# CEED/Laghos

Hardware: AMD Instinct MI355X
Metric: Mdofs×steps/s on 3D Sedov -pa (Q3/Q2) (higher is better)
Workload: dtype f64; 1 GPU; 3D Sedov -p 1 -m cube01_hex -rs 4 -ok 3 -ot 2 -pa (32^3 elements, E0/2^dim = 0.125); transport=none (one rank), elements=32768, h1_dofs=2738019, l2_dofs=884736, quad_points_per_element=216, rk_stages_executed=1300, ode=RK4, parallelism=elements1x1x1, zones_per_gpu=32x32x32

## Files before the change

### include/laghos_hip.h

```cpp
#ifndef LAGHOS_HIP_H
#define LAGHOS_HIP_H

#ifdef __cplusplus
extern "C" {
#endif

#define LGH_OK 0
#define LGH_ERR_ARG 1
#define LGH_ERR_UNSUPPORTED 2
#define LGH_ERR_HIP 3
#define LGH_ERR_COMM 4

#define LGH_SPACE_H1 0
#define LGH_SPACE_L2 1

typedef struct lgh_ctx lgh_ctx;

typedef struct lgh_config
{
   int dim, NE;
   int D1D, Q1D, L1D;
   int N;
   const int *h1_map;
   const double *B_h1;
// ... 42 lines not shown
int lgh_mass_eliminate_rhs(lgh_ctx *ctx, double *b);
int lgh_mass_mult(lgh_ctx *ctx, int space, const double *x, double *y);
int lgh_mass_mult_full(lgh_ctx *ctx, int space, const double *x, double *y);

int lgh_cg_solve(lgh_ctx *ctx, int space, const double *b, double *x, double rel_tol,
                 int max_iter, int *iters);
int lgh_l2_mass_solve_local(lgh_ctx *ctx, const double *b, double *x);

int lgh_qupdate(lgh_ctx *ctx, const double *S);
int lgh_qupdate_set_tiny_grad(lgh_ctx *ctx, double tiny_grad);
int lgh_set_fused_forces(lgh_ctx *ctx, int on);
int lgh_qupdate_store_stress(lgh_ctx *ctx, int on);
int lgh_qupdate_stores_stress(lgh_ctx *ctx, int *on);
int lgh_qupdate_form(lgh_ctx *ctx, int *form);
int lgh_reset_quadrature_data(lgh_ctx *ctx);
int lgh_fused_force_mult(lgh_ctx *ctx, double *y_h1);
int lgh_fused_force_mult_transpose(lgh_ctx *ctx, double *y_l2);
int lgh_quadrature_generation(lgh_ctx *ctx, unsigned long *gen, int *f1_valid, int *ftv_valid);
int lgh_get_fused_forces(lgh_ctx *ctx, int *f1, int *ftv);

int lgh_solve_velocity(lgh_ctx *ctx, const double *S, double *dS_dt, const double *one_l2,
                       double *rhs_h1, double *work_B, double rel_tol, int max_iter,
                       int *h1_iters);
int lgh_solve_energy(lgh_ctx *ctx, const double *S, const double *v_h1, double *dS_dt,
                     double *e_rhs, const double *e_source, double rel_tol, int max_iter,
                     int *l2_iters);
int lgh_solve_energy_begin(lgh_ctx *ctx, const double *S, const double *v_h1, double *dS_dt,
                           double *e_rhs, const double *e_source, double rel_tol, int max_iter);
int lgh_solve_energy_end(lgh_ctx *ctx, int *l2_iters);
int lgh_energy_lockstep_stats(lgh_ctx *ctx, long out[4]);

int lgh_vec_set(lgh_ctx *ctx, double *y, double a, long n);
int lgh_vec_copy(lgh_ctx *ctx, double *y, const double *x, long n);
int lgh_vec_axpby_pair(lgh_ctx *ctx, double *z1, double a1, const double *x1, double b1, double *z2, double a2, const double *x2, double b2,
                       const double *y, long n);
int lgh_vec_axpby(lgh_ctx *ctx, double *z, double a, const double *x, double b,
                  const double *y, long n);
int lgh_vec_dot(lgh_ctx *ctx, const double *x, const double *y, long n, double *result);
int lgh_vec_fingerprint(lgh_ctx *ctx, const double *x, long n, unsigned long long offset, unsigned long long out[2]);
int lgh_vec_fingerprint_shape(lgh_ctx *ctx, const double *x, long n, long out[4]);
int lgh_fingerprint_host(const void *words, long n, unsigned long long offset, unsigned long long out[2]);

int lgh_set_velocity_source(lgh_ctx *ctx, const double *accel_h1);

int lgh_tg_source_2d(lgh_ctx *ctx, const double *S, double *e_source);

int lgh_internal_energy(lgh_ctx *ctx, const double *e_l2, double *result);
int lgh_kinetic_energy(lgh_ctx *ctx, const double *v_h1, double *result);

int lgh_sedov_setup(int dim, double gamma, double rho0, double blast_energy, double omega, double par[21]);
int lgh_sedov_shock(const double par[21], double t, double shock[6]);
int lgh_sedov_eval_point(const double par[21], double t, double r, double *rho, double *v, double *P);
int lgh_sedov_eval(lgh_ctx *ctx, const double par[21], double t, long n, const double *r, double *rho, double *v,
                   double *P);
int lgh_compute_density(lgh_ctx *ctx, const double *x_h1, double *rho_l2);
int lgh_sedov_density_error(lgh_ctx *ctx, const double *x_h1, const double *rho_l2, const double par[21], double t,
                            const double origin[3], int n1d, const double *weights, const double *B_h1,
                            const double *G_h1, const double *B_l2, double *err2);

int lgh_sample_fields(lgh_ctx *ctx, const double *S, const double *rho_l2 ,
                      int R1, const double *B_h1_lat ,
                      const double *B_l2_lat ,
                      double *x_out, double *v_out, double *e_out, double *rho_out, double *p_out);

int lgh_sample_derived(lgh_ctx *ctx, const double *S, int R1, const double *B_h1_lat ,
                       const double *G_h1_lat , const double *B_l2_lat ,
// ... 82 lines not shown
```

### laghos_amd/_lib.py

```python
import ctypes
import os

_HERE = os.path.dirname(os.path.abspath(__file__))
LIB_PATH = os.path.join(_HERE, "liblaghos_hip.so")

c_dp = ctypes.c_void_p
c_int_p = ctypes.POINTER(ctypes.c_int)
c_dbl_p = ctypes.POINTER(ctypes.c_double)


class LghConfig(ctypes.Structure):
    _fields_ = [
        ("dim", ctypes.c_int), ("NE", ctypes.c_int),
        ("D1D", ctypes.c_int), ("Q1D", ctypes.c_int), ("L1D", ctypes.c_int),
        ("N", ctypes.c_int),
        ("h1_map", c_int_p),
        ("B_h1", c_dbl_p), ("G_h1", c_dbl_p), ("B_l2", c_dbl_p),
        ("weights", c_dbl_p), ("gamma", c_dbl_p),
        ("ess_count", ctypes.c_int * 3),
        ("ess", c_int_p * 3),
        ("owner", c_dbl_p),
        ("use_viscosity", ctypes.c_int), ("use_vorticity", ctypes.c_int),
        ("cfl", ctypes.c_double),
        ("order_v", ctypes.c_int),
# ... 12 lines not shown
    "lgh_last_error": (ctypes.c_char_p, []),
    "lgh_version": (ctypes.c_char_p, []),
    "lgh_create": (_I, [ctypes.POINTER(LghConfig), ctypes.POINTER(_P)]),
    "lgh_destroy": (_I, [_P]),
    "lgh_sync": (_I, [_P]),
    "lgh_stream": (_P, [_P]),
    "lgh_qdata_stressJinvT": (_P, [_P]),
    "lgh_qdata_Jac0inv": (_P, [_P]),
    "lgh_qdata_rho0DetJ0w": (_P, [_P]),
    "lgh_mass_D": (_P, [_P]),
    "lgh_mass_diag": (_P, [_P]),
    "lgh_set_h0": (_I, [_P, _D]),
    "lgh_get_h0": (_I, [_P, c_dbl_p]),
    "lgh_set_dt_est": (_I, [_P, _D]),
    "lgh_get_dt_est": (_I, [_P, c_dbl_p]),
    "lgh_setup_rho0detj0": (_I, [_P, _P, _P, _P, c_dbl_p]),
    "lgh_force_mult": (_I, [_P, _P, _P]),
    "lgh_force_mult_transpose": (_I, [_P, _P, _P]),
    "lgh_mass_set_essential_tdofs": (_I, [_P, _I]),
    "lgh_mass_eliminate_rhs": (_I, [_P, _P]),
    "lgh_mass_mult": (_I, [_P, _I, _P, _P]),
    "lgh_mass_mult_full": (_I, [_P, _I, _P, _P]),
    "lgh_cg_solve": (_I, [_P, _I, _P, _P, _D, _I, c_int_p]),
    "lgh_l2_mass_solve_local": (_I, [_P, _P, _P]),
    "lgh_qupdate": (_I, [_P, _P]),
    "lgh_solve_velocity": (_I, [_P, _P, _P, _P, _P, _P, _D, _I, c_int_p]),
    "lgh_solve_energy": (_I, [_P, _P, _P, _P, _P, _P, _D, _I, c_int_p]),
    "lgh_solve_energy_begin": (_I, [_P, _P, _P, _P, _P, _P, _D, _I]),
    "lgh_tg_source_2d": (_I, [_P, _P, _P]),
    "lgh_set_velocity_source": (_I, [_P, _P]),
    "lgh_solve_energy_end": (_I, [_P, c_int_p]),
    "lgh_vec_set": (_I, [_P, _P, _D, _L]),
    "lgh_vec_copy": (_I, [_P, _P, _P, _L]),
    "lgh_vec_axpby": (_I, [_P, _P, _D, _P, _D, _P, _L]),
    "lgh_vec_axpby_pair": (_I, [_P, _P, _D, _P, _D, _P, _D, _P, _D, _P, _L]),
    "lgh_vec_dot": (_I, [_P, _P, _P, _L, c_dbl_p]),
    "lgh_vec_fingerprint": (_I, [_P, _P, _L, ctypes.c_ulonglong, ctypes.POINTER(ctypes.c_ulonglong)]),
    "lgh_vec_fingerprint_shape": (_I, [_P, _P, _L, ctypes.POINTER(ctypes.c_long)]),
    "lgh_fingerprint_host": (_I, [_P, _L, ctypes.c_ulonglong, ctypes.POINTER(ctypes.c_ulonglong)]),
    "lgh_internal_energy": (_I, [_P, _P, c_dbl_p]),
    "lgh_kinetic_energy": (_I, [_P, _P, c_dbl_p]),
    "lgh_sedov_setup": (_I, [_I, _D, _D, _D, _D, c_dbl_p]),
    "lgh_sedov_shock": (_I, [c_dbl_p, _D, c_dbl_p]),
    "lgh_sedov_eval_point": (_I, [c_dbl_p, _D, _D, c_dbl_p, c_dbl_p, c_dbl_p]),
    "lgh_sedov_eval": (_I, [_P, c_dbl_p, _D, _L, _P, _P, _P, _P]),
    "lgh_compute_density": (_I, [_P, _P, _P]),
    "lgh_sedov_density_error": (_I, [_P, _P, _P, c_dbl_p, _D, c_dbl_p, _I, c_dbl_p, c_dbl_p, c_dbl_p, c_dbl_p, c_dbl_p]),
    "lgh_sample_fields": (_I, [_P, _P, _P, _I, c_dbl_p, c_dbl_p, _P, _P, _P, _P, _P]),
    "lgh_sample_derived": (_I, [_P, _P, _I, c_dbl_p, c_dbl_p, c_dbl_p, _P, _P, _P, _P, _P]),
    "lgh_diagnostics_zones": (_I, [_P, _P, _P]),
    "lgh_diagnostics": (_I, [_P, _P, c_dbl_p]),
    "lgh_profile": (_I, [_P, _P, ctypes.POINTER(LghProfileSpec), c_dbl_p, ctypes.POINTER(ctypes.c_long)]),
    "lgh_get_timers": (_I, [_P, c_dbl_p, ctypes.POINTER(ctypes.c_long)]),
    "lgh_reset_timers": (_I, [_P]),
    "lgh_enable_timers": (_I, [_P, _I]),
    "lgh_ktime_begin": (_I, [_P, _I, _I]),
    "lgh_ktime_end": (_I, [_P, c_int_p, c_dbl_p]),
    "lgh_table_symmetry": (_I, [_P, c_int_p, c_int_p]),
    "lgh_k1_form": (_I, [_P, c_int_p]),
    "lgh_l2_mass_form": (_I, [_P, c_int_p, c_int_p]),
    "lgh_vcg_layout_stats": (_I, [_P, ctypes.POINTER(ctypes.c_long)]),
    "lgh_energy_lockstep_stats": (_I, [_P, ctypes.POINTER(ctypes.c_long)]),
    "lgh_mesh_order": (_I, [_P, ctypes.POINTER(ctypes.c_long)]),
    "lgh_mesh_order_host": (_I, [_I, _I, _I, _I, c_int_p, c_int_p, c_int_p, ctypes.POINTER(ctypes.c_long)]),
    "lgh_mass_data_form": (_I, [_P, c_int_p]),
    "lgh_jac0inv_form": (_I, [_P, c_int_p]),
# ... 73 lines not shown
```

### laghos_amd/csrc/lgh_1d.hip

```cpp
#include <algorithm>
#include <cmath>
#include <limits>
#include <type_traits>

#include "lgh_common.hpp"

namespace lgh
{

bool kernel_id_supported_1d(int kid)
{
   switch (kid)
   {
      case 0x122: case 0x134: case 0x146: case 0x158: case 0x16A: return true;
   }
   return false;
}

template <int V> using IC = std::integral_constant<int, V>;

template <class F> static int dispatch_1d(const lgh_ctx *c, F &&f)
{
   switch (c->kid)
   {
// ... 689 lines not shown
   LGH_TRY(alloc_copy(&c->B, cfg->B_h1, (size_t)Q * D));
   LGH_TRY(alloc_copy(&c->G, cfg->G_h1, (size_t)Q * D));
   LGH_TRY(alloc_copy(&c->Bl, cfg->B_l2, (size_t)Q * L));
   LGH_TRY(alloc_copy(&c->W, cfg->weights, (size_t)Q));
   LGH_TRY(alloc_copy(&c->gamma, cfg->gamma, (size_t)NE));
   const size_t nmap = (size_t)NE * D;
   LGH_TRY(alloc_copy(&c->h1map, cfg->h1_map, nmap));
   LGH_TRY(mesh_order_build(c, cfg->h1_map));
   {
      std::vector<int> off((size_t)N + 1, 0), idx(nmap);
      for (size_t i = 0; i < nmap; i++) { off[(size_t)cfg->h1_map[i] + 1]++; }
      for (int n = 0; n < N; n++) { off[(size_t)n + 1] += off[n]; }
      std::vector<int> pos(off.begin(), off.end() - 1);
      for (size_t i = 0; i < nmap; i++) { idx[pos[cfg->h1_map[i]]++] = (int)i; }
      LGH_TRY(alloc_copy(&c->t_off, off.data(), off.size()));
      LGH_TRY(alloc_copy(&c->t_idx, idx.data(), idx.size()));
   }
   {
      c->ess_count[0] = cfg->ess_count[0];
      std::vector<uint8_t> mask((size_t)N, 0);
      for (int i = 0; i < c->ess_count[0]; i++) { mask[cfg->ess[0][i]] = 1; }
      LGH_TRY(alloc_copy(&c->essmask[0], mask.data(), mask.size()));
      LGH_TRY(alloc_copy(&c->ess[0], c->ess_count[0] ? cfg->ess[0] : nullptr, (size_t)c->ess_count[0]));
   }
   const size_t nq = (size_t)NE * Q;
   LGH_TRY(alloc_zero(&c->stressJinvT, nq));
   LGH_TRY(alloc_zero(&c->Jac0inv, nq));
   LGH_TRY(alloc_zero(&c->rho0DetJ0w, nq));
   LGH_TRY(alloc_zero(&c->massD, nq));
   LGH_TRY(alloc_zero(&c->me_fac, (size_t)NE * L * L));
   LGH_TRY(alloc_zero(&c->diagV, (size_t)N));
   LGH_TRY(alloc_zero(&c->dinvV, (size_t)N));
   LGH_TRY(alloc_zero(&c->dt_est_dev, (size_t)kDtSlotStride * (1 + kDtSlots)));
   LGH_TRY(alloc_zero(&c->dev_flags, (size_t)8));
   LGH_TRY(alloc_zero(&c->YE, std::max(nmap, (size_t)c->L2V)));
   const size_t nv = std::max<size_t>((size_t)N, (size_t)c->L2V);
   LGH_TRY(alloc_zero(&c->cg_r, nv));
   LGH_TRY(alloc_zero(&c->cg_z, nv));
   LGH_TRY(alloc_zero(&c->cg_d0, nv));
   LGH_TRY(alloc_zero(&c->cg_y, nv));
   c->part_stride = (int)std::max<size_t>(std::max<size_t>((size_t)NE, (nv + 255) / 256), 2048) + (int)kShards;
   LGH_TRY(alloc_zero(&c->partials, 4 * (size_t)c->part_stride));
   LGH_TRY(alloc_zero(&c->tickets, 4 * (size_t)kTicketSlot));
   LGH_TRY(alloc_zero(&c->cgs, 1));
   LGH_TRY(alloc_zero(&c->scal, 16));
   LGH_HIP_CHECK(hipHostMalloc((void **)&c->host_pinned, 96 * sizeof(double), hipHostMallocMapped | hipHostMallocCoherent));
   memset(c->host_pinned, 0, 96 * sizeof(double));
   LGH_HIP_CHECK(hipHostGetDevicePointer((void **)&c->host_pinned_dev, c->host_pinned, 0));
   LGH_HIP_CHECK(hipEventCreate(&c->timers.ev[0]));
   LGH_HIP_CHECK(hipEventCreate(&c->timers.ev[1]));
   {
      const std::vector<double> infs((size_t)kDtSlotStride * (1 + kDtSlots), std::numeric_limits<double>::infinity());
      LGH_HIP_CHECK(hipMemcpy(c->dt_est_dev, infs.data(), infs.size() * sizeof(double), hipMemcpyHostToDevice));
   }
#undef LGH_TRY
   return LGH_OK;
}

int mass_changed_1d(lgh_ctx *c)
{
   return dispatch_1d(c, [&](auto Dc, auto Qc) {
      constexpr int D = decltype(Dc)::value, Q = decltype(Qc)::value;
      hipLaunchKernelGGL((h1_diag_e_1d_k<D, Q>), dim3(zone_grid(c)), dim3(256), 0, c->stream, c->NE, c->B, c->massD, c->YE);
      hipLaunchKernelGGL(gather_1d_k, dim3(ceil_div(c->N, 256)), dim3(256), 0, c->stream, c->N, c->t_off, c->t_idx, c->YE,
                         (const uint8_t *)nullptr, c->diagV);
      hipLaunchKernelGGL(reciprocal_1d_k, dim3(ceil_div(c->N, 256)), dim3(256), 0, c->stream, c->N, c->diagV, c->dinvV);
      hipLaunchKernelGGL((l2_factor_1d_k<D - 1, Q>), dim3(zone_grid(c)), dim3(256), 0, c->stream, c->NE, c->Bl, c->massD,
// ... 258 lines not shown
```

### laghos_amd/csrc/lgh_api.hip

```cpp
#include <cstdarg>
#include <cstdlib>
#include <cmath>
#include <algorithm>
#include <limits>

#include "lgh_common.hpp"

#include <chrono>
#include <dlfcn.h>

namespace lgh
{

static thread_local char g_err[512] = "";
void set_error(const char *fmt, ...)
{
   va_list ap;
   va_start(ap, fmt);
   vsnprintf(g_err, sizeof(g_err), fmt, ap);
   va_end(ap);
}

__global__ void __launch_bounds__(256) vec_set_k(double *y, double a, long n)
{
// ... 5 lines not shown
   for (long i = blockIdx.x * (long)blockDim.x + threadIdx.x; i < n; i += (long)gridDim.x * blockDim.x)
   {
      z[i] = fma(a, x[i], __dmul_rn(b, y[i]));
   }
}
__global__ void __launch_bounds__(256)
vec_axpby2_k(double2 *z, double a, const double2 *x, double b, const double2 *y, long n2)
{
   const long stride = (long)gridDim.x * blockDim.x;
   long i = blockIdx.x * (long)blockDim.x + threadIdx.x;
   for (; i + stride < n2; i += 2 * stride)
   {
      const double2 x0 = x[i], y0 = y[i], x1 = x[i + stride], y1 = y[i + stride];
      z[i] = make_double2(fma(a, x0.x, __dmul_rn(b, y0.x)), fma(a, x0.y, __dmul_rn(b, y0.y)));
      z[i + stride] = make_double2(fma(a, x1.x, __dmul_rn(b, y1.x)), fma(a, x1.y, __dmul_rn(b, y1.y)));
   }
   if (i < n2)
   {
      const double2 x0 = x[i], y0 = y[i];
      z[i] = make_double2(fma(a, x0.x, __dmul_rn(b, y0.x)), fma(a, x0.y, __dmul_rn(b, y0.y)));
   }
}
__global__ void __launch_bounds__(256)
vec_axpby_pair_k(double2 *z1, double a1, const double2 *x1, double b1, double2 *z2, double a2, const double2 *x2, double b2, const double2 *y, long n2)
{
   const long stride = (long)gridDim.x * blockDim.x;
   for (long i = blockIdx.x * (long)blockDim.x + threadIdx.x; i < n2; i += stride)
   {
      const double2 y0 = y[i], p = x1[i], q = x2[i];
      z1[i] = make_double2(fma(a1, p.x, __dmul_rn(b1, y0.x)), fma(a1, p.y, __dmul_rn(b1, y0.y)));
      z2[i] = make_double2(fma(a2, q.x, __dmul_rn(b2, y0.x)), fma(a2, q.y, __dmul_rn(b2, y0.y)));
   }
}
__global__ void __launch_bounds__(256) vec_neg_k(double *y, long n)
{
   for (long i = blockIdx.x * (long)blockDim.x + threadIdx.x; i < n; i += (long)gridDim.x * blockDim.x) { y[i] = -y[i]; }
}
__global__ void __launch_bounds__(256) vec_zero_list_k(double *y, const int *list, int n)
{
   const int i = blockIdx.x * blockDim.x + threadIdx.x;
   if (i < n) { y[list[i]] = 0.0; }
}
__global__ void __launch_bounds__(256)
vec_dot_k(const double *x, const double *y, const double *w, long n, double *partials,
          unsigned int *ticket, double *out)
{
   __shared__ double red[16];
   double s = 0.0;
   for (long i = blockIdx.x * (long)blockDim.x + threadIdx.x; i < n; i += (long)gridDim.x * blockDim.x)
   {
      s += (w ? w[i] : 1.0) * x[i] * y[i];
   }
   const double bsum = block_sum(s, red);
   double total;
   if (grid_sum_last_block(bsum, partials, ticket, red, total))
   {
      if (threadIdx.x == 0) { *out = total; }
   }
}
__global__ void set_double_k(double *p, double v) { *p = v; }
__global__ void __launch_bounds__(256) dt_est_set_k(double *p, double v)
{
   if (threadIdx.x == 0) { p[0] = v; }
   for (int s = threadIdx.x; s < kDtSlots; s += blockDim.x) { p[kDtSlotStride * (1 + s)] = __builtin_inf(); }
}
__global__ void __launch_bounds__(256) dt_est_fold_k(double *p, const int *err, double *host_out, const unsigned long long token)
// ... 32 lines not shown
   if (n >= 4096 && (((uintptr_t)z | (uintptr_t)x | (uintptr_t)y) & 15u) == 0)
   {
      const long n2 = n / 2;
      hipLaunchKernelGGL(vec_axpby2_k, dim3(grid_for(n2)), dim3(256), 0, c->stream, (double2 *)z, a, (const double2 *)x, b,
                         (const double2 *)y, n2);
      if (n & 1) { hipLaunchKernelGGL(vec_axpby_k, dim3(1), dim3(64), 0, c->stream, z + 2 * n2, a, x + 2 * n2, b, y + 2 * n2, 1L); }
   }
   else { hipLaunchKernelGGL(vec_axpby_k, dim3(grid_for(n)), dim3(256), 0, c->stream, z, a, x, b, y, n); }
   LGH_HIP_CHECK(hipGetLastError());
   return LGH_OK;
}
int vec_axpby_pair(lgh_ctx *c, double *z1, double a1, const double *x1, double b1, double *z2, double a2, const double *x2, double b2,
                   const double *y, long n)
{
   if (n <= 0) { return LGH_OK; }
   if (n >= 4096 && (((uintptr_t)z1 | (uintptr_t)x1 | (uintptr_t)z2 | (uintptr_t)x2 | (uintptr_t)y) & 15u) == 0)
   {
      const long n2 = n / 2;
      hipLaunchKernelGGL(vec_axpby_pair_k, dim3(grid_for(n2)), dim3(256), 0, c->stream, (double2 *)z1, a1, (const double2 *)x1, b1, (double2 *)z2, a2,
                         (const double2 *)x2, b2, (const double2 *)y, n2);
      LGH_HIP_CHECK(hipGetLastError());
      if (n & 1)
      {
         hipLaunchKernelGGL(vec_axpby_k, dim3(1), dim3(64), 0, c->stream, z1 + 2 * n2, a1, x1 + 2 * n2, b1, y + 2 * n2, 1L);
         hipLaunchKernelGGL(vec_axpby_k, dim3(1), dim3(64), 0, c->stream, z2 + 2 * n2, a2, x2 + 2 * n2, b2, y + 2 * n2, 1L);
      }
      LGH_HIP_CHECK(hipGetLastError());
      return LGH_OK;
   }
   int rc = vec_axpby(c, z1, a1, x1, b1, y, n);
   if (rc) { return rc; }
   return vec_axpby(c, z2, a2, x2, b2, y, n);
}
int vec_neg_inplace(lgh_ctx *c, double *y, long n)
{
   if (n <= 0) { return LGH_OK; }
   hipLaunchKernelGGL(vec_neg_k, dim3(grid_for(n)), dim3(256), 0, c->stream, y, n);
   LGH_HIP_CHECK(hipGetLastError());
   return LGH_OK;
}
int vec_zero_list(lgh_ctx *c, double *y, const int *list, int n)
{
   if (n <= 0) { return LGH_OK; }
   hipLaunchKernelGGL(vec_zero_list_k, dim3(ceil_div(n, 256)), dim3(256), 0, c->stream, y, list, n);
   LGH_HIP_CHECK(hipGetLastError());
   return LGH_OK;
}
int vec_dot(lgh_ctx *c, const double *x, const double *y, const double *w, long n, double *dev_out)
{
   hipLaunchKernelGGL(vec_dot_k, dim3(grid_for(n)), dim3(256), 0, c->stream, x, y, w, n,
                      c->partials + 3 * (size_t)c->part_stride, c->tickets + 3 * kTicketSlot, dev_out);
   LGH_HIP_CHECK(hipGetLastError());
   return LGH_OK;
}

void timer_start(lgh_ctx *c)
{
   if (!c->timers.enabled) { return; }
   (void)hipEventRecord(c->timers.ev[0], c->stream);
}
void timer_stop(lgh_ctx *c, int which)
{
   if (!c->timers.enabled) { return; }
   (void)hipEventRecord(c->timers.ev[1], c->stream);
   (void)hipEventSynchronize(c->timers.ev[1]);
   float ms = 0.f;
// ... 55 lines not shown
static bool kernel_id_supported(int id)
{
   switch (id)
   {
      case 0x222: case 0x234: case 0x246: case 0x258: case 0x26A:
      case 0x322: case 0x334: case 0x346: case 0x358: case 0x36A:
         return true;
   }
   return false;
}

}

namespace lgh
{
int host_wait_token(lgh_ctx *c, volatile unsigned long long *word, const unsigned long long token)
{
   const bool spin = !(getenv("LGH_SPIN") && getenv("LGH_SPIN")[0] == '0');
   if (spin)
   {
      const auto t0 = std::chrono::steady_clock::now();
      for (long i = 0;; i++)
      {
         if (__atomic_load_n((const unsigned long long *)word, __ATOMIC_ACQUIRE) == token) { return LGH_OK; }
         __builtin_ia32_pause();
         if ((i & 1023) == 1023 && std::chrono::steady_clock::now() - t0 > std::chrono::milliseconds(50)) { break; }
      }
   }
   LGH_HIP_CHECK(hipStreamSynchronize(c->stream));
   if (__atomic_load_n((const unsigned long long *)word, __ATOMIC_ACQUIRE) != token) { set_error("host look: the finishing kernel did not report"); return LGH_ERR_HIP; }
   return LGH_OK;
}

int energy_overlap_poll(lgh_ctx *c)
{
   if (c->e_async != 1 || c->e_polled) { return LGH_OK; }
   int it = 0;
   std::swap(c->stream, c->stream2);
   c->on_stream2 = 1;
   int rc = cg_l2_end(c, &it);
   if (rc == LGH_OK) { rc = (hipEventRecord(c->ev_join, c->stream) == hipSuccess) ? LGH_OK : LGH_ERR_HIP; }
   std::swap(c->stream, c->stream2);
   c->on_stream2 = 0;
   if (rc) { return rc; }
   c->e_polled = 1;
   c->e_iters = it;
   return LGH_OK;
}

}

using namespace lgh;

extern "C"
{

const char *lgh_last_error(void) { return g_err; }
const char *lgh_version(void) { return "laghos_hip 0.1 (gfx950)"; }

static int create_impl(const lgh_config *cfg, lgh_ctx *c, const int kid);

int lgh_create(const lgh_config *cfg, lgh_ctx **out)
{
   LGH_CHECK_ARG(cfg && out);
   LGH_CHECK_ARG(cfg->dim == 1 || cfg->dim == 2 || cfg->dim == 3);
   LGH_CHECK_ARG(cfg->NE > 0 && cfg->N > 0);
   LGH_CHECK_ARG(cfg->h1_map && cfg->B_h1 && cfg->G_h1 && cfg->B_l2 && cfg->weights && cfg->gamma);
   if (cfg->L1D != cfg->D1D - 1)
   {
      set_error("L1D!=D1D-1");
      return LGH_ERR_UNSUPPORTED;
   }
   const int kid = (cfg->dim << 8) | (cfg->D1D << 4) | cfg->Q1D;
   if (!(cfg->dim == 1 ? kernel_id_supported_1d(kid) : kernel_id_supported(kid)))
// ... 32 lines not shown
   memset((void *)c, 0, sizeof(lgh_ctx));
   new (&c->timers) Timers();
   c->device = cfg->device;
   const int rc_create = (cfg->dim == 1) ? create_1d(cfg, c) : create_impl(cfg, c, kid);
   if (rc_create != LGH_OK)
   {
      lgh_destroy(c);
      return rc_create;
   }
   *out = c;
   return LGH_OK;
}

static int create_impl(const lgh_config *cfg, lgh_ctx *c, const int kid)
{
   c->dim = cfg->dim; c->NE = cfg->NE; c->D1D = cfg->D1D; c->Q1D = cfg->Q1D; c->L1D = cfg->L1D;
   const int dim = c->dim;
   c->ND = dim == 2 ? c->D1D * c->D1D : c->D1D * c->D1D * c->D1D;
   c->NQ = dim == 2 ? c->Q1D * c->Q1D : c->Q1D * c->Q1D * c->Q1D;
   c->NL = dim == 2 ? c->L1D * c->L1D : c->L1D * c->L1D * c->L1D;
   c->N = cfg->N;
   c->H1V = dim * c->N;
   c->L2V = c->NE * c->NL;
   c->kid = kid;
   c->visc = cfg->use_viscosity != 0;
   c->vort = cfg->use_vorticity != 0;
   c->cfl = cfg->cfl;
   c->h1order = (double)cfg->order_v;
   {
      const char *env = getenv("LGH_Q_TINY_GRAD");
      c->q_tiny_grad = env ? atof(env) : 1e-30;
      c->stress_store = 1;
      c->stress_current = 0;
   }
   c->h0 = 0.0;
   c->device = cfg->device;
   c->cur_ess = -1;
   c->nranks = 1;
   c->rank = 0;
   if (cfg->stream) { c->stream = (hipStream_t)cfg->stream; c->own_stream = false; }
   else { LGH_HIP_CHECK(hipStreamCreateWithFlags(&c->stream, hipStreamNonBlocking)); c->own_stream = true; }

   int rc;
#define LGH_TRY(x) do { rc = (x); if (rc) { return rc; } } while (0)
   LGH_TRY(dev_alloc_copy(&c->B, cfg->B_h1, (size_t)c->Q1D * c->D1D));
   {
      const char *env = getenv("LGH_B_SYM");
      auto mirror = [&](const double *B, const int n) {
         if (env && env[0] == '0') { return 0; }
         for (int i = 0; i < n; i++)
         {
            const double u = B[i], v = B[n - 1 - i];
            if (std::fabs(u - v) > 1e-14 * std::max(1.0, std::max(std::fabs(u), std::fabs(v)))) { return 0; }
         }
         return 1;
      };
      c->b_h1_sym = mirror(cfg->B_h1, c->Q1D * c->D1D);
      c->b_l2_sym = mirror(cfg->B_l2, c->Q1D * c->L1D);
   }
   LGH_TRY(dev_alloc_copy(&c->G, cfg->G_h1, (size_t)c->Q1D * c->D1D));
   LGH_TRY(dev_alloc_copy(&c->Bl, cfg->B_l2, (size_t)c->Q1D * c->L1D));
   LGH_TRY(dev_alloc_copy(&c->W, cfg->weights, (size_t)c->NQ));
   {
      const int Q = c->Q1D, dim = c->dim;
      std::vector<double> w1((size_t)Q);
      const double w0 = (dim == 3) ? cbrt(cfg->weights[0]) : sqrt(cfg->weights[0]);
// ... 73 lines not shown
   }
   for (int k = 0; k < 3; k++)
   {
      c->ess_count[k] = (k < dim) ? cfg->ess_count[k] : 0;
      std::vector<uint8_t> mask((size_t)c->N, 0);
      for (int i = 0; i < c->ess_count[k]; i++)
      {
         const int n = cfg->ess[k][i];
         if (n < 0 || n >= c->N) { set_error("essential dof out of range"); return LGH_ERR_ARG; }
         mask[n] = 1;
      }
      LGH_TRY(dev_alloc_copy(&c->essmask[k], mask.data(), mask.size()));
      LGH_TRY(dev_alloc_copy(&c->ess[k], c->ess_count[k] ? cfg->ess[k] : nullptr, (size_t)c->ess_count[k]));
   }
   if (cfg->owner) { LGH_TRY(dev_alloc_copy(&c->owner, cfg->owner, (size_t)c->N)); }

   const size_t nq = (size_t)c->NE * c->NQ;
   LGH_TRY(dev_alloc_zero(&c->stressJinvT, nq * dim * dim));
   LGH_TRY(dev_alloc_zero(&c->Jac0inv, nq * dim * dim));
   LGH_TRY(dev_alloc_zero(&c->Jac0inv_soa, nq * dim * dim));
   LGH_TRY(dev_alloc_zero(&c->Jac0inv_e, (size_t)cfg->NE * dim * dim));
   LGH_TRY(dev_alloc_zero(&c->rho0DetJ0w, nq));
   LGH_TRY(dev_alloc_zero(&c->massD, nq + 2048));
   LGH_TRY(dev_alloc_zero(&c->diagV, (size_t)c->N));
   LGH_TRY(dev_alloc_zero(&c->dinvV, (size_t)c->N));
   LGH_TRY(dev_alloc_zero(&c->dt_est_dev, (size_t)kDtSlotStride * (1 + kDtSlots)));
   {
      const char *env = getenv("LGH_FUSED_FTV");
      if (!(env && env[0] == '0'))
      {
         LGH_TRY(dev_alloc_zero(&c->erhs_q, (size_t)c->L2V));
         LGH_TRY(dev_alloc_zero(&c->v_snap, (size_t)c->H1V));
      }
      LGH_TRY(dev_alloc_zero(&c->dev_flags, (size_t)8));
      c->mass_rank1 = -1;
      env = getenv("LGH_FUSED_F1");
      if (c->dim == 3 && !(env && env[0] == '0')) { LGH_TRY(dev_alloc_zero(&c->force_e_q, nmap * dim + (size_t)dim * c->ND)); }
   }
   const size_t ne_nd = nmap * dim;
   LGH_TRY(dev_alloc_zero(&c->XE, std::max<size_t>(ne_nd, (size_t)c->L2V)));
   LGH_TRY(dev_alloc_zero(&c->YE, ne_nd + (size_t)dim * c->ND));
   const size_t nv = std::max<size_t>((size_t)c->N, (size_t)c->L2V);
   LGH_TRY(dev_alloc_zero(&c->cg_r, nv));
   LGH_TRY(dev_alloc_zero(&c->cg_z, nv));
   LGH_TRY(dev_alloc_zero(&c->cg_d0, nv));
   LGH_TRY(dev_alloc_zero(&c->cg_d1, nv));
   LGH_TRY(dev_alloc_zero(&c->cg_y, nv));
   c->part_stride = (int)std::max<size_t>(std::max<size_t>((size_t)c->NE, (nv + 255) / 256), 2048) + (int)kShards;
   LGH_TRY(dev_alloc_zero(&c->partials, 4 * (size_t)c->part_stride));
   LGH_TRY(dev_alloc_zero(&c->tickets, 4 * (size_t)kTicketSlot));
   LGH_TRY(dev_alloc_zero(&c->cgs, 1));
   LGH_TRY(dev_alloc_zero(&c->scal, 16));
   LGH_HIP_CHECK(hipHostMalloc((void **)&c->host_pinned, 96 * sizeof(double), hipHostMallocMapped | hipHostMallocCoherent));
   memset(c->host_pinned, 0, 96 * sizeof(double));
   LGH_HIP_CHECK(hipHostGetDevicePointer((void **)&c->host_pinned_dev, c->host_pinned, 0));
   LGH_HIP_CHECK(hipEventCreate(&c->timers.ev[0]));
   LGH_HIP_CHECK(hipEventCreate(&c->timers.ev[1]));
   {
      const std::vector<double> infs((size_t)kDtSlotStride * (1 + kDtSlots), std::numeric_limits<double>::infinity());
      LGH_HIP_CHECK(hipMemcpy(c->dt_est_dev, infs.data(), infs.size() * sizeof(double), hipMemcpyHostToDevice));
   }
#undef LGH_TRY
   return LGH_OK;
}

int lgh_destroy(lgh_ctx *c)
{
   if (!c) { return LGH_OK; }
   (void)hipSetDevice(c->device);
   (void)hipStreamSynchronize(c->stream);
   void *ptrs[] = {c->B, c->G, c->Bl, c->W, c->w1d, c->M1h, c->M1l, c->gamma, c->h1map, c->t_off, c->t_idx, c->t_ell, c->essmask[0],
                   c->essmask[1], c->essmask[2], c->ess[0], c->ess[1], c->ess[2], c->owner,
                   c->stressJinvT, c->Jac0inv, c->Jac0inv_soa, c->Jac0inv_e, c->rho0DetJ0w, c->massD, c->diagV, c->dinvV,
                   c->dt_est_dev, c->erhs_q, c->v_snap, c->dev_flags, c->ones_l2, c->massS, c->ones_ne, c->force_e_q, c->XE, c->YE, c->cg_r, c->cg_z, c->cg_d0, c->cg_d1, c->cg_y,
                   c->partials, c->tickets, c->cgs, c->scal, c->vcg_s, c->vcg_vec, c->vcg_partials,
                   c->vcg_tickets, c->me_fac, c->fp_dev, c->diag_dev, c->prof_dev};
   for (void *p : ptrs) { if (p) { (void)hipFree(p); } }
   if (c->host_pinned) { (void)hipHostFree(c->host_pinned); }
   if (c->timers.ev[0]) { (void)hipEventDestroy(c->timers.ev[0]); }
   if (c->timers.ev[1]) { (void)hipEventDestroy(c->timers.ev[1]); }
   if (c->ktime)
   {
      for (hipEvent_t e : c->ktime->ev) { (void)hipEventDestroy(e); }
      delete c->ktime;
   }
   cg_l2_free(c);
   vcg_free(c);
   mesh_order_free(c);
   if (c->q_trace_dev) { (void)hipFree(c->q_trace_dev); }
   if (c->stream2)
   {
      (void)hipStreamSynchronize(c->stream2);
      (void)hipStreamDestroy(c->stream2);
      (void)hipEventDestroy(c->ev_fork);
      (void)hipEventDestroy(c->ev_join);
   }
   for (auto &ring : c->ls_ev) { for (hipEvent_t e : ring) { if (e) { (void)hipEventDestroy(e); } } }
   extern void lgh_comm_free(lgh_ctx *);
   lgh_comm_free(c);
   if (c->own_stream) { (void)hipStreamDestroy(c->stream); }
   delete c;
   return LGH_OK;
}

int lgh_sync(lgh_ctx *c)
{
   LGH_CHECK_ARG(c);
   LGH_HIP_CHECK(hipStreamSynchronize(c->stream));
   return LGH_OK;
}
void *lgh_stream(lgh_ctx *c) { return c ? (void *)c->stream : nullptr; }

static void invalidate_fused(lgh_ctx *c)
{
   c->fused_ftv_valid = 0;
   c->fused_f1_valid = 0;
   c->qgen++;
}
double *lgh_qdata_stressJinvT(lgh_ctx *c)
{
   invalidate_fused(c);
   if (c->stress_store) { c->stress_current = 1; }
   return c->stressJinvT;
}
static int stress_on_hand(lgh_ctx *c, const char *who)
{
   if (c->stress_current) { return LGH_OK; }
   set_error("%s needs stressJinvT, which the last lgh_qupdate kept in registers (lgh_qupdate_store_stress(ctx, 0)): "
             "only F.1 and F^T v of the state's own velocity are on hand; store the stress (..., 1) and update again", who);
   return LGH_ERR_ARG;
}
static int no_1d(const lgh_ctx *c, const char *who)
{
   if (c->dim != 1) { return LGH_OK; }
   set_error("%s: not available for a 1D context (lgh_1d.hip has its own kernels)", who);
   return LGH_ERR_UNSUPPORTED;
}
int lgh_qupdate_form(lgh_ctx *c, int *form)
{
   LGH_CHECK_ARG(c && form);
   *form = qupdate_form(c);
   return LGH_OK;
}
int lgh_qupdate_stores_stress(lgh_ctx *c, int *on)
{
   LGH_CHECK_ARG(c && on);
   *on = (!c->stress_store && c->erhs_q && c->force_e_q && c->v_snap && !c->fused_forces_off && c->dim == 3) ? 0 : 1;
   return LGH_OK;
}
int lgh_qupdate_store_stress(lgh_ctx *c, int on)
{
   LGH_CHECK_ARG(c);
   if ((on != 0) != (c->stress_store != 0))
   {
      c->stress_store = on ? 1 : 0;
      invalidate_fused(c);
      c->stress_current = 0;
   }
   return LGH_OK;
}
int lgh_reset_quadrature_data(lgh_ctx *c)
{
   LGH_CHECK_ARG(c);
   invalidate_fused(c);
   return LGH_OK;
}
int lgh_fused_force_mult(lgh_ctx *c, double *y_h1)
{
   LGH_CHECK_ARG(c && y_h1);
   if (!(c->force_e_q && c->fused_f1_valid)) { set_error("lgh_fused_force_mult: no fused F.1 on hand"); return LGH_ERR_ARG; }
   int rc = h1_transpose_gather(c, c->dim, c->force_e_q, y_h1);
   if (rc == LGH_OK && c->multi != 0) { rc = halo_sum(c, y_h1, c->dim); }
   return rc;
}
int lgh_fused_force_mult_transpose(lgh_ctx *c, double *y_l2)
{
   LGH_CHECK_ARG(c && y_l2);
   if (!(c->erhs_q && c->fused_ftv_valid)) { set_error("lgh_fused_force_mult_transpose: no fused F^T v on hand"); return LGH_ERR_ARG; }
   LGH_HIP_CHECK(hipMemcpyAsync(y_l2, c->erhs_q, sizeof(double) * (size_t)c->L2V, hipMemcpyDeviceToDevice, c->stream));
   return LGH_OK;
}
int lgh_quadrature_generation(lgh_ctx *c, unsigned long *gen, int *f1_valid, int *ftv_valid)
{
   LGH_CHECK_ARG(c && gen && f1_valid && ftv_valid);
   *gen = c->qgen;
   *f1_valid = c->fused_f1_valid;
   *ftv_valid = c->fused_ftv_valid;
   return LGH_OK;
}
double *lgh_qdata_Jac0inv(lgh_ctx *c) { return c->Jac0inv; }
double *lgh_qdata_rho0DetJ0w(lgh_ctx *c) { return c->rho0DetJ0w; }
double *lgh_mass_D(lgh_ctx *c)
{
   c->mass_rank1 = -1;
   c->mass_gen++;
   return c->massD;
}
int lgh_mass_data_form(lgh_ctx *c, int *form)
{
   LGH_CHECK_ARG(c && form);
   if (c->dim == 1) { *form = 0; return LGH_OK; }
   const double *Dq, *Se;
   int dqs;
   int rc = mass_data(c, &Dq, &dqs, &Se);
   if (rc) { return rc; }
   *form = (c->mass_rank1 == 1) ? 1 : 0;
   return LGH_OK;
}
int lgh_mass_data_changed(lgh_ctx *c)
{
   LGH_CHECK_ARG(c);
   c->mass_rank1 = -1;
   c->mass_gen++;
   if (c->dim == 1) { return mass_changed_1d(c); }
   return mass_assemble_diag(c);
}
double *lgh_mass_diag(lgh_ctx *c) { return c->diagV; }
int lgh_set_h0(lgh_ctx *c, double h0) { LGH_CHECK_ARG(c); c->h0 = h0; return LGH_OK; }
int lgh_get_h0(lgh_ctx *c, double *h0) { LGH_CHECK_ARG(c && h0); *h0 = c->h0; return LGH_OK; }

int lgh_set_dt_est(lgh_ctx *c, double v)
{
   LGH_CHECK_ARG(c);
   hipLaunchKernelGGL(dt_est_set_k, dim3(1), dim3(256), 0, c->stream, c->dt_est_dev, v);
   LGH_HIP_CHECK(hipGetLastError());
   return LGH_OK;
}
int lgh_get_dt_est(lgh_ctx *c, double *v)
{
   LGH_CHECK_ARG(c && v);
   const unsigned long long token = ++c->look_token;
   hipLaunchKernelGGL(dt_est_fold_k, dim3(1), dim3(256), 0, c->stream, c->dt_est_dev, c->dev_flags + 4, c->host_pinned_dev + 8, token);
   LGH_HIP_CHECK(hipGetLastError());
   {
      const int rc = host_wait_token(c, (volatile unsigned long long *)(c->host_pinned + 10), token);
      if (rc) { return rc; }
   }
   *v = c->host_pinned[8];
   if (*(const int *)(c->host_pinned + 9) != 0)
   {
      LGH_HIP_CHECK(hipMemsetAsync(c->dev_flags + 4, 0, sizeof(int), c->stream));
      set_error("lgh_solve_energy was given a velocity other than the state's while the stress was kept in registers "
                "(lgh_qupdate_store_stress(ctx, 0)): its right-hand side is NaN");
      return LGH_ERR_ARG;
   }
   return LGH_OK;
}

int lgh_setup_rho0detj0(lgh_ctx *c, const double *x0, const double *rho0_l2, const double *rho0_q,
                        double *volume)
{
   LGH_CHECK_ARG(c && x0 && rho0_l2 && rho0_q && volume);
   invalidate_fused(c);
   c->mass_rank1 = -1;
   c->mass_gen++;
   int rc = (c->dim == 1) ? setup_1d(c, x0, rho0_l2, rho0_q, volume)
                          : setup_rho0detj0(c, x0, rho0_l2, rho0_q, volume);
   if (rc) { return rc; }
   if (c->dim != 1) { rc = mass_assemble_diag(c); }
   if (rc == LGH_OK) { c->setup_done = 1; }
   return rc;
}

int lgh_force_mult(lgh_ctx *c, const double *x_l2, double *y_h1)
{
   LGH_CHECK_ARG(c && x_l2 && y_h1);
   int rc = stress_on_hand(c, "lgh_force_mult");
   if (rc) { return rc; }
   if (c->dim == 1) { return force_mult_1d(c, x_l2, y_h1); }
   kt_begin(c, LGH_KERNEL_FORCE_MULT);
   rc = force_mult_E(c, c->stressJinvT, x_l2, c->YE);
   kt_end(c, LGH_KERNEL_FORCE_MULT);
   if (rc) { return rc; }
   rc = h1_transpose_gather(c, c->dim, c->YE, y_h1);
   if (rc) { return rc; }
   if (c->multi != 0) { rc = halo_sum(c, y_h1, c->dim); }
   return rc;
}
int lgh_force_mult_transpose(lgh_ctx *c, const double *v_h1, double *y_l2)
{
   LGH_CHECK_ARG(c && v_h1 && y_l2);
   const int rc0 = stress_on_hand(c, "lgh_force_mult_transpose");
   if (rc0) { return rc0; }
   if (c->dim == 1) { return force_mult_t_1d(c, v_h1, y_l2); }
   kt_begin(c, LGH_KERNEL_FORCE_MULT_T);
   const int rc = force_mult_t_L(c, c->stressJinvT, v_h1, y_l2);
   kt_end(c, LGH_KERNEL_FORCE_MULT_T);
   return rc;
}

int lgh_mass_set_essential_tdofs(lgh_ctx *c, int comp)
{
   LGH_CHECK_ARG(c && comp >= -1 && comp < c->dim);
   c->cur_ess = comp;
   return LGH_OK;
}
int lgh_mass_eliminate_rhs(lgh_ctx *c, double *b)
{
   LGH_CHECK_ARG(c && b);
   if (c->cur_ess < 0) { return LGH_OK; }
   return vec_zero_list(c, b, c->ess[c->cur_ess], c->ess_count[c->cur_ess]);
}
int lgh_mass_mult(lgh_ctx *c, int space, const double *x, double *y)
{
   LGH_CHECK_ARG(c && x && y && (space == LGH_SPACE_H1 || space == LGH_SPACE_L2));
   if (c->dim == 1) { return mass_apply_1d(c, space, x, y, true); }
   return space == LGH_SPACE_H1 ? mass_apply_h1(c, x, y, true) : mass_apply_l2(c, x, y);
}
int lgh_mass_mult_full(lgh_ctx *c, int space, const double *x, double *y)
{
   LGH_CHECK_ARG(c && x && y && (space == LGH_SPACE_H1 || space == LGH_SPACE_L2));
   if (c->dim == 1) { return mass_apply_1d(c, space, x, y, false); }
   return space == LGH_SPACE_H1 ? mass_apply_h1(c, x, y, false) : mass_apply_l2(c, x, y);
}

int lgh_cg_solve(lgh_ctx *c, int space, const double *b, double *x, double rel_tol, int max_iter,
                 int *iters)
{
   LGH_CHECK_ARG(c && b && x && (space == LGH_SPACE_H1 || space == LGH_SPACE_L2));
   if (c->dim == 1) { return cg_1d(c, space, b, x, rel_tol, max_iter, iters, false); }
   return cg_solve(c, space, b, x, rel_tol, max_iter, iters, false);
}

int lgh_l2_mass_solve_local(lgh_ctx *c, const double *b, double *x)
{
   LGH_CHECK_ARG(c && b && x);
   if (c->dim != 1)
   {
      set_error("lgh_l2_mass_solve_local: the zone-local energy solve belongs to the 1D (full-assembly) path; 2D/3D run the energy CG");
      return LGH_ERR_UNSUPPORTED;
   }
   return l2_solve_local_1d(c, b, x);
}

int lgh_qupdate(lgh_ctx *c, const double *S)
{
   LGH_CHECK_ARG(c && S);
   RoctxRange range("QUpdate-UpdateQuadratureData");
   timer_start(c);
   kt_begin(c, LGH_KERNEL_QUPDATE);
   int rc = (c->dim == 1) ? qupdate_1d(c, S) : qupdate(c, S);
   kt_end(c, LGH_KERNEL_QUPDATE);
   timer_stop(c, 3);
   c->timers.c[2] += c->NE;
   return rc;
}

__global__ void __launch_bounds__(256) not_all_ones_k(const double *x, const long n, int *flag)
{
   const long i = (long)blockIdx.x * blockDim.x + threadIdx.x;
   if (i < n && x[i] != 1.0) { *flag = 1; }
}
static bool is_the_one_vector(lgh_ctx *c, const double *one_l2)
{
   if (!one_l2) { return true; }
   int *flag = c->dev_flags + 1;
   if (hipMemsetAsync(flag, 0, sizeof(int), c->stream) != hipSuccess) { return false; }
   hipLaunchKernelGGL(not_all_ones_k, dim3(ceil_div(c->L2V, 256)), dim3(256), 0, c->stream, one_l2, (long)c->L2V, flag);
   int h = 1;
   if (hipMemcpyAsync(&h, flag, sizeof(int), hipMemcpyDeviceToHost, c->stream) != hipSuccess) { return false; }
   if (hipStreamSynchronize(c->stream) != hipSuccess) { return false; }
   return h == 0;
}
static int one_vector(lgh_ctx *c, const double *one_l2, const double **out)
{
   if (one_l2) { *out = one_l2; return LGH_OK; }
   if (!c->ones_l2)
   {
      LGH_HIP_CHECK(hipMalloc((void **)&c->ones_l2, sizeof(double) * (size_t)c->L2V));
      const int rc = vec_set(c, c->ones_l2, 1.0, c->L2V);
      if (rc) { return rc; }
   }
   *out = c->ones_l2;
   return LGH_OK;
}

int lgh_solve_velocity(lgh_ctx *c, const double *S, double *dS_dt, const double *one_l2,
                       double *rhs_h1, double *work_B, double rel_tol, int max_iter, int *h1_iters)
{
   LGH_CHECK_ARG(c && S && dS_dt && rhs_h1 && work_B);
   const int dim = c->dim, N = c->N;
   double *dv = dS_dt + c->H1V;
   int rc;
   if (dim == 1)
   {
      LGH_CHECK_ARG(!c->accel_src);
      const double *ones = nullptr;
      rc = one_vector(c, one_l2, &ones);
      if (rc) { return rc; }
      rc = stress_on_hand(c, "lgh_solve_velocity");
      if (rc) { return rc; }
      return solve_velocity_1d(c, ones, dv, rhs_h1, rel_tol, max_iter, h1_iters);
   }
   if (!c->timers.enabled && !c->accel_src && vcg_fused_init_ok(c))
   {
      const double *force_E = c->YE;
      if (c->force_e_q && c->fused_f1_valid && is_the_one_vector(c, one_l2)) { force_E = c->force_e_q; }
      else
      {
         const double *ones = nullptr;
         rc = one_vector(c, one_l2, &ones);
         if (rc) { return rc; }
         rc = stress_on_hand(c, "lgh_solve_velocity (F.1 of a vector other than one, or of changed quadrature data)");
         if (rc) { return rc; }
         kt_begin(c, LGH_KERNEL_FORCE_MULT);
         rc = force_mult_E(c, c->stressJinvT, ones, c->YE);
         kt_end(c, LGH_KERNEL_FORCE_MULT);
         if (rc) { return rc; }
      }
      int its[3] = {0, 0, 0};
      RoctxRange range("SolveVelocity-CGVMass");
      rc = vcg_solve(c, rhs_h1, dv, rel_tol, max_iter, its, force_E);
      if (rc) { return rc; }
// ... 31 lines not shown
      for (int cc = 0; cc < dim; cc++)
      {
         rc = mass_apply_h1(c, c->accel_src + (size_t)cc * N, work_B, false);
         if (rc) { return rc; }
         rc = vec_axpby(c, rhs_h1 + (size_t)cc * N, 1.0, rhs_h1 + (size_t)cc * N, 1.0, work_B, N);
         if (rc) { return rc; }
      }
   }
   {
      for (int cc = 0; cc < dim; cc++)
      {
         rc = vec_zero_list(c, rhs_h1 + (size_t)cc * N, c->ess[cc], c->ess_count[cc]);
         if (rc) { return rc; }
      }
      int its[3] = {0, 0, 0};
      RoctxRange range("SolveVelocity-CGVMass");
      timer_start(c);
      rc = vcg_solve(c, rhs_h1, dv, rel_tol, max_iter, its);
      if (rc == LGH_OK)
      {
         timer_stop(c, 0);
         for (int cc = 0; cc < dim; cc++)
         {
            c->timers.c[0] += its[cc];
            if (h1_iters) { *h1_iters += its[cc]; }
         }
         c->cur_ess = dim - 1;
         return LGH_OK;
      }
      if (rc != LGH_ERR_UNSUPPORTED) { return rc; }
   }
   for (int cc = 0; cc < dim; cc++)
   {
      LGH_HIP_CHECK(hipMemcpyAsync(work_B, rhs_h1 + (size_t)cc * N, sizeof(double) * N,
                                   hipMemcpyDeviceToDevice, c->stream));
      rc = lgh_mass_set_essential_tdofs(c, cc);
      if (rc) { return rc; }
      rc = lgh_mass_eliminate_rhs(c, work_B);
      if (rc) { return rc; }
      int it = 0;
      timer_start(c);
      rc = cg_solve(c, LGH_SPACE_H1, work_B, dv + (size_t)cc * N, rel_tol, max_iter, &it, true);
      timer_stop(c, 0);
      if (rc) { return rc; }
      c->timers.c[0] += it;
      if (h1_iters) { *h1_iters += it; }
   }
   return LGH_OK;
}

__global__ void __launch_bounds__(256) vec_differs_k(const double *__restrict__ a, const double *__restrict__ b, const long n, int *flag)
{
   const long stride = (long)gridDim.x * blockDim.x, t = (long)blockIdx.x * blockDim.x + threadIdx.x;
   bool diff = false;
   if (((((uintptr_t)a) | ((uintptr_t)b)) & 15u) == 0)
   {
      const longlong2 *a2 = (const longlong2 *)a, *b2 = (const longlong2 *)b;
      for (long i = t; i < n / 2; i += stride)
      {
         const longlong2 p = a2[i], q = b2[i];
         diff = diff || p.x != q.x || p.y != q.y;
      }
      if ((n & 1) && t == 0) { diff = diff || __double_as_longlong(a[n - 1]) != __double_as_longlong(b[n - 1]); }
   }
   else
   {
      for (long i = t; i < n; i += stride) { diff = diff || __double_as_longlong(a[i]) != __double_as_longlong(b[i]); }
   }
   if (diff) { *flag = 1; }
}
__global__ void __launch_bounds__(256) erhs_take_or_poison_k(double *__restrict__ y, const double *__restrict__ x, const long n, const int *__restrict__ flag, int *err)
{
   const long i = (long)blockIdx.x * blockDim.x + threadIdx.x;
   if (*flag != 0)
   {
      if (i < n) { y[i] = __builtin_nan(""); }
      if (i == 0) { *err = 1; }
      return;
   }
   if (i < n) { y[i] = x[i]; }
}
__global__ void __launch_bounds__(256) copy_unless_k(double *__restrict__ y, const double *__restrict__ x, const long n, const int *__restrict__ flag)
{
   if (*flag != 0) { return; }
   const long i = (long)blockIdx.x * blockDim.x + threadIdx.x;
   if (i < n) { y[i] = x[i]; }
}
static int energy_rhs(lgh_ctx *c, const double *v_h1, double *e_rhs)
{
   RoctxRange range("SolveEnergy-ForcePA");
   if (c->erhs_q && c->fused_ftv_valid)
   {
      int *flag = c->dev_flags + (c->on_stream2 ? 2 : 0);
      LGH_HIP_CHECK(hipMemsetAsync(flag, 0, sizeof(int), c->stream));
      hipLaunchKernelGGL(vec_differs_k, dim3(grid_for((c->H1V + 1) / 2)), dim3(256), 0, c->stream, v_h1, c->v_snap, (long)c->H1V, flag);
      LGH_HIP_CHECK(hipGetLastError());
      if (c->stress_current)
      {
         const int rc = force_mult_t_L(c, c->stressJinvT, v_h1, e_rhs, flag);
         if (rc) { return rc; }
         hipLaunchKernelGGL(copy_unless_k, dim3(ceil_div(c->L2V, 256)), dim3(256), 0, c->stream, e_rhs, c->erhs_q, (long)c->L2V, flag);
      }
      else
      {
         hipLaunchKernelGGL(erhs_take_or_poison_k, dim3(ceil_div(c->L2V, 256)), dim3(256), 0, c->stream, e_rhs, c->erhs_q, (long)c->L2V, flag, c->dev_flags + 4);
      }
      LGH_HIP_CHECK(hipGetLastError());
      return LGH_OK;
   }
   return lgh_force_mult_transpose(c, v_h1, e_rhs);
}

int lgh_solve_energy(lgh_ctx *c, const double *S, const double *v_h1, double *dS_dt, double *e_rhs,
                     const double *e_source, double rel_tol, int max_iter, int *l2_iters)
{
   LGH_CHECK_ARG(c && S && v_h1 && dS_dt && e_rhs);
   (void)S;
   double *de = dS_dt + 2 * (size_t)c->H1V;
   if (c->dim == 1)
   {
      const int rc1 = stress_on_hand(c, "lgh_solve_energy");
      if (rc1) { return rc1; }
      return solve_energy_1d(c, v_h1, de, e_rhs, e_source, l2_iters);
   }
   timer_start(c);
   int rc = energy_rhs(c, v_h1, e_rhs);
   timer_stop(c, 2);
   if (rc) { return rc; }
   if (e_source)
   {
      rc = vec_axpby(c, e_rhs, 1.0, e_rhs, 1.0, e_source, c->L2V);
      if (rc) { return rc; }
   }
   int it = 0;
   RoctxRange range("SolveEnergy-CGEMass");
   timer_start(c);
   rc = cg_solve(c, LGH_SPACE_L2, e_rhs, de, rel_tol, max_iter, &it, true);
   timer_stop(c, 1);
   if (rc) { return rc; }
   const int counted = (it == 0) ? 1 : it;
   c->timers.c[1] += counted;
   if (l2_iters) { *l2_iters += counted; }
   return LGH_OK;
}

static int create_stream2(lgh_ctx *c)
{
   const char *penv = getenv("LGH_STREAM2_PRIORITY");
   const char want = (penv && (penv[0] == 'd' || penv[0] == 'h')) ? penv[0] : 'l';
   int least = 0, greatest = 0;
   if (want != 'd' && hipDeviceGetStreamPriorityRange(&least, &greatest) == hipSuccess && least != greatest)
   {
      LGH_HIP_CHECK(hipStreamCreateWithPriority(&c->stream2, hipStreamNonBlocking, want == 'h' ? greatest : least));
   }
   else { LGH_HIP_CHECK(hipStreamCreateWithFlags(&c->stream2, hipStreamNonBlocking)); }
   LGH_HIP_CHECK(hipEventCreateWithFlags(&c->ev_fork, hipEventDisableTiming));
   LGH_HIP_CHECK(hipEventCreateWithFlags(&c->ev_join, hipEventDisableTiming));
   return LGH_OK;
}
static bool energy_overlap_ok(const lgh_ctx *c)
{
   const bool on = !(getenv("LGH_OVERLAP") && getenv("LGH_OVERLAP")[0] == '0');
   return on && (c->multi == 0 || comm_second_channel(c)) && !c->timers.enabled && !(c->ktime && c->ktime->which >= 0) && vcg_available(c);
}
int lgh_solve_energy_begin(lgh_ctx *c, const double *S, const double *v_h1, double *dS_dt, double *e_rhs,
                           const double *e_source, double rel_tol, int max_iter)
{
   LGH_CHECK_ARG(c && S && v_h1 && dS_dt && e_rhs);
   c->e_args = {S, v_h1, dS_dt, e_rhs, e_source, rel_tol, max_iter};
   c->e_lockstep = 0;
   if (c->dim == 1)
   {
      c->e_async = 2;
      return LGH_OK;
   }
   if (!energy_overlap_ok(c))
   {
      const bool ls_on = !(getenv("LGH_ENERGY_LOCKSTEP") && getenv("LGH_ENERGY_LOCKSTEP")[0] == '0');
      const bool overlap_wanted = !(getenv("LGH_OVERLAP") && getenv("LGH_OVERLAP")[0] == '0');
      if (ls_on && overlap_wanted && c->multi != 0 && !comm_second_channel(c) && !c->timers.enabled && !(c->ktime && c->ktime->which >= 0) && vcg_available(c) &&
          l2_lockstep_possible(c) && vcg_lockstep_ready(c))
      {
         int rc = energy_rhs(c, v_h1, e_rhs);
         if (rc == LGH_OK && e_source) { rc = vec_axpby(c, e_rhs, 1.0, e_rhs, 1.0, e_source, c->L2V); }
         if (rc == LGH_OK) { rc = cg_l2_begin_lockstep(c, e_rhs, dS_dt + 2 * (size_t)c->H1V, rel_tol, max_iter); }
         if (rc) { return rc; }
         c->ls_side = (getenv("LGH_LOCKSTEP_STREAM2") && getenv("LGH_LOCKSTEP_STREAM2")[0] == '1') ? 1 : 0;
         if (c->ls_side)
         {
            if (!c->stream2)
            {
               const int rc2 = create_stream2(c);
               if (rc2) { return rc2; }
            }
            for (auto &ring : c->ls_ev) { for (hipEvent_t &e : ring) { if (!e) { LGH_HIP_CHECK(hipEventCreateWithFlags(&e, hipEventDisableTiming)); } } }
         }
         c->e_async = 3;
// ... 23 lines not shown
   c->on_stream2 = 0;
   if (rc) { return rc; }
   c->e_async = 1;
   c->e_polled = 0;
   return LGH_OK;
}
int lgh_energy_lockstep_stats(lgh_ctx *c, long out[4])
{
   LGH_CHECK_ARG(c && out);
   out[0] = c->ls_stats[0]; out[1] = c->ls_stats[1]; out[2] = c->ls_stats[2];
   out[3] = (c->dim != 1 && c->multi != 0 && !comm_second_channel(c) && vcg_available(c) && l2_lockstep_possible(c) && vcg_lockstep_ready(c)) ? 1 : 0;
   return LGH_OK;
}
int lgh_solve_energy_end(lgh_ctx *c, int *l2_iters)
{
   LGH_CHECK_ARG(c && (c->e_async == 1 || c->e_async == 2 || c->e_async == 3));
   const int mode = c->e_async;
   c->e_async = 0;
   if (mode == 3)
   {
      c->e_lockstep = 0;
      int it = 0;
      const int rc = cg_l2_end_lockstep(c, &it);
      if (rc) { return rc; }
      const int counted = (it == 0) ? 1 : it;
      c->timers.c[1] += counted;
      if (l2_iters) { *l2_iters += counted; }
      return LGH_OK;
   }
   if (mode == 1 && c->e_polled)
   {
      c->e_polled = 0;
      LGH_HIP_CHECK(hipStreamWaitEvent(c->stream, c->ev_join, 0));
      const int counted = (c->e_iters == 0) ? 1 : c->e_iters;
      c->timers.c[1] += counted;
      if (l2_iters) { *l2_iters += counted; }
      return LGH_OK;
   }
   if (mode == 2)
   {
      return lgh_solve_energy(c, c->e_args.S, c->e_args.v, c->e_args.dS, c->e_args.e_rhs, c->e_args.src,
                              c->e_args.tol, c->e_args.maxit, l2_iters);
   }
   int it = 0;
   std::swap(c->stream, c->stream2);
   c->on_stream2 = 1;
   int rc = cg_l2_end(c, &it);
   if (rc == LGH_OK) { rc = (hipEventRecord(c->ev_join, c->stream) == hipSuccess) ? LGH_OK : LGH_ERR_HIP; }
   std::swap(c->stream, c->stream2);
   c->on_stream2 = 0;
   if (rc) { return rc; }
   LGH_HIP_CHECK(hipStreamWaitEvent(c->stream, c->ev_join, 0));
   const int counted = (it == 0) ? 1 : it;
   c->timers.c[1] += counted;
   if (l2_iters) { *l2_iters += counted; }
   return LGH_OK;
}

int lgh_vec_set(lgh_ctx *c, double *y, double a, long n) { LGH_CHECK_ARG(c && y); return vec_set(c, y, a, n); }
int lgh_vec_copy(lgh_ctx *c, double *y, const double *x, long n)
{
   LGH_CHECK_ARG(c && y && x);
   LGH_HIP_CHECK(hipMemcpyAsync(y, x, sizeof(double) * n, hipMemcpyDeviceToDevice, c->stream));
   return LGH_OK;
}
int lgh_vec_axpby(lgh_ctx *c, double *z, double a, const double *x, double b, const double *y, long n)
{
   LGH_CHECK_ARG(c && z && x && y);
   return vec_axpby(c, z, a, x, b, y, n);
}
int lgh_vec_axpby_pair(lgh_ctx *c, double *z1, double a1, const double *x1, double b1, double *z2, double a2, const double *x2, double b2,
                       const double *y, long n)
{
   LGH_CHECK_ARG(c && z1 && x1 && z2 && x2 && y && n >= 0);
   {
      auto overlap = [n](const double *p, const double *q) { return p < q + n && q < p + n; };
      LGH_CHECK_ARG(!overlap(z1, z2) && !overlap(z1, x2) && !overlap(z1, y));
      LGH_CHECK_ARG(!overlap(z2, y) && !overlap(z2, x1) && (z2 == x2 || !overlap(z2, x2)) && (z1 == x1 || !overlap(z1, x1)));
   }
   return vec_axpby_pair(c, z1, a1, x1, b1, z2, a2, x2, b2, y, n);
}
int lgh_vec_dot(lgh_ctx *c, const double *x, const double *y, long n, double *result)
{
   LGH_CHECK_ARG(c && x && y && result);
   int rc = vec_dot(c, x, y, nullptr, n, c->scal + 1);
   if (rc) { return rc; }
   LGH_HIP_CHECK(hipMemcpyAsync(c->host_pinned + 1, c->scal + 1, sizeof(double), hipMemcpyDeviceToHost, c->stream));
   LGH_HIP_CHECK(hipStreamSynchronize(c->stream));
   *result = c->host_pinned[1];
   return LGH_OK;
}

int lgh_set_velocity_source(lgh_ctx *c, const double *accel_h1)
{
   LGH_CHECK_ARG(c);
   if (accel_h1)
   {
      const int rc = no_1d(c, "lgh_set_velocity_source");
      if (rc) { return rc; }
   }
   c->accel_src = accel_h1;
   return LGH_OK;
}

int lgh_tg_source_2d(lgh_ctx *c, const double *S, double *e_source)
{
   LGH_CHECK_ARG(c && S && e_source);
   const int rc = no_1d(c, "lgh_tg_source_2d");
   if (rc) { return rc; }
   return tg_source_2d(c, S, e_source);
}

int lgh_internal_energy(lgh_ctx *c, const double *e_l2, double *result)
{
   LGH_CHECK_ARG(c && e_l2 && result);
   if (c->dim == 1) { return energy_1d(c, 0, e_l2, result); }
   return interp_energy(c, 0, e_l2, result);
}
int lgh_kinetic_energy(lgh_ctx *c, const double *v_h1, double *result)
{
   LGH_CHECK_ARG(c && v_h1 && result);
   if (c->dim == 1) { return energy_1d(c, 1, v_h1, result); }
   return interp_energy(c, 1, v_h1, result);
}

int lgh_get_timers(lgh_ctx *c, double t[4], long n[3])
{
   LGH_CHECK_ARG(c && t && n);
   for (int i = 0; i < 4; i++) { t[i] = c->timers.t[i]; }
   for (int i = 0; i < 3; i++) { n[i] = c->timers.c[i]; }
   return LGH_OK;
}
int lgh_reset_timers(lgh_ctx *c)
{
   LGH_CHECK_ARG(c);
   for (int i = 0; i < 4; i++) { c->timers.t[i] = 0; }
   for (int i = 0; i < 3; i++) { c->timers.c[i] = 0; }
   return LGH_OK;
}
int lgh_enable_timers(lgh_ctx *c, int on)
{
   LGH_CHECK_ARG(c);
   c->timers.enabled = on != 0;
   return LGH_OK;
}

int lgh_ktime_begin(lgh_ctx *c, int which, int max_samples)
{
   LGH_CHECK_ARG(c && which >= 0 && max_samples > 0);
   if (!c->ktime) { c->ktime = new KTime(); }
   KTime *k = c->ktime;
   while ((int)k->ev.size() < 2 * max_samples)
   {
      hipEvent_t e;
// ... 27 lines not shown
{
   LGH_CHECK_ARG(c);
   if (c->fused_forces_off == (on ? 0 : 1)) { return LGH_OK; }
   c->fused_forces_off = on ? 0 : 1;
   invalidate_fused(c);
   return LGH_OK;
}

int lgh_get_fused_forces(lgh_ctx *c, int *f1, int *ftv)
{
   LGH_CHECK_ARG(c && f1 && ftv);
   *f1 = (c->force_e_q && !c->fused_forces_off) ? 1 : 0;
   *ftv = (c->erhs_q && !c->fused_forces_off) ? 1 : 0;
   return LGH_OK;
}

int lgh_qupdate_set_tiny_grad(lgh_ctx *c, double tiny_grad)
{
   LGH_CHECK_ARG(c);
   c->q_tiny_grad = tiny_grad;
   return LGH_OK;
}

int lgh_table_symmetry(lgh_ctx *c, int *h1, int *l2)
{
   LGH_CHECK_ARG(c && h1 && l2);
   *h1 = c->b_h1_sym;
   *l2 = c->b_l2_sym;
   return LGH_OK;
}
int lgh_l2_mass_form(lgh_ctx *c, int *form, int *compact)
{
   LGH_CHECK_ARG(c && form && compact);
   if (c->dim == 1) { *form = 0; *compact = 0; return LGH_OK; }
   return l2_mass_form(c, form, compact);
}
int lgh_k1_form(lgh_ctx *c, int *form)
{
   LGH_CHECK_ARG(c && form);
   *form = (c->dim == 1) ? -1 : vcg_k1_form(c);
   return LGH_OK;
}

int lgh_test_vcg_k1(lgh_ctx *c, const double *r, const double *d_old, const double rz[3], const double rz_prev[3], int first,
                    double *y_E, double den[3])
{
   LGH_CHECK_ARG(c && r && (first || d_old) && rz && rz_prev && y_E && den);
   const int rc = no_1d(c, "lgh_test_vcg_k1");
   if (rc) { return rc; }
   return vcg_test_k1(c, r, d_old, rz, rz_prev, first, y_E, den);
}
int lgh_jac0inv_form(lgh_ctx *c, int *compact)
{
   LGH_CHECK_ARG(c && compact);
   *compact = (c->jac0_compact == 1) ? 1 : 0;
   return LGH_OK;
}
int lgh_vcg_layout_stats(lgh_ctx *c, long out[4])
{
   LGH_CHECK_ARG(c && out);
   const int rc = no_1d(c, "lgh_vcg_layout_stats");
   if (rc) { return rc; }
   return vcg_layout_stats(c, out);
}
int lgh_test_vcg_merged_faces(lgh_ctx *c, unsigned char *mask, long *n_merged)
{
   LGH_CHECK_ARG(c && mask && n_merged);
   const int rc = no_1d(c, "lgh_test_vcg_merged_faces");
   if (rc) { return rc; }
   return vcg_test_merged_faces(c, mask, n_merged);
}
int lgh_test_vcg_k2(lgh_ctx *c, int it, const double *y_E, double *r, double *d, double *x, const double den[3], const double rz[3],
                    const double rz_prev[3], const double alpha_prev[3], double rz_out[3], int *deferred_x)
{
   LGH_CHECK_ARG(c && it >= 1 && y_E && r && d && x && den && rz && rz_prev && alpha_prev && rz_out && deferred_x);
   const int rc = no_1d(c, "lgh_test_vcg_k2");
   if (rc) { return rc; }
   return vcg_test_k2(c, it, y_E, r, d, x, den, rz, rz_prev, alpha_prev, rz_out, deferred_x);
}
int lgh_test_exact_sum(lgh_ctx *c, int mode, long n, int G, int E, const double *scale, const double *v, const long long *w_in,
                       long long *w_out, double *d_out, int *i_out)
{
   LGH_CHECK_ARG(c && mode >= 0 && mode <= 4 && n >= 1 && n <= (1L << 24) && E >= -1000 && E <= 1000);
   LGH_CHECK_ARG(mode != 0 || (v && w_out && i_out));
   LGH_CHECK_ARG(mode != 1 || (w_in && d_out && !scale));
   LGH_CHECK_ARG(mode != 2 || (v && w_out && d_out && G >= 1 && G <= 1024));
   LGH_CHECK_ARG(mode != 3 || (w_in && w_out && n % 64 == 0));
   LGH_CHECK_ARG(mode != 4 || (v && i_out));
   return vcg_test_exact_sum(c, mode, n, G, E, scale, v, w_in, w_out, d_out, i_out);
}
int lgh_force_mult_E(lgh_ctx *c, const double *sJit, const double *x_E, double *y_E)
{
   LGH_CHECK_ARG(c && sJit && x_E && y_E);
   const int rc = no_1d(c, "lgh_force_mult_E");
   if (rc) { return rc; }
   return force_mult_E(c, sJit, x_E, y_E);
}
int lgh_force_mult_transpose_E(lgh_ctx *c, const double *sJit, const double *v_E, double *y_E)
{
   LGH_CHECK_ARG(c && sJit && v_E && y_E);
   const int rc = no_1d(c, "lgh_force_mult_transpose_E");
   if (rc) { return rc; }
   return force_mult_t_E(c, sJit, v_E, y_E);
}
int lgh_mass_apply_E(lgh_ctx *c, int space, const double *x_E, double *y_E)
{
   LGH_CHECK_ARG(c && x_E && y_E);
   const int rc = no_1d(c, "lgh_mass_apply_E");
   if (rc) { return rc; }
   return mass_apply_E(c, space, x_E, y_E);
}
int lgh_test_eig(lgh_ctx *c, int dim, int n, const double *A, double *lambda, double *vec)
{
   LGH_CHECK_ARG(c && A && lambda && vec && (dim == 2 || dim == 3));
   return test_eig(c, dim, n, A, lambda, vec);
}
int lgh_test_sqrt(lgh_ctx *c, int n, const double *x, double *y)
{
   LGH_CHECK_ARG(c && x && y && n >= 0);
   return test_sqrt(c, n, x, y);
}
int lgh_test_singular(lgh_ctx *c, int dim, int n, const double *A, double *sv)
{
   LGH_CHECK_ARG(c && A && sv && (dim == 2 || dim == 3));
   return test_singular(c, dim, n, A, sv);
}

}
```

### laghos_amd/csrc/lgh_comm.hip

```cpp
#include <dlfcn.h>
#include <fcntl.h>
#include <sys/mman.h>
#include <sys/stat.h>
#include <unistd.h>
#include <cstdlib>
#include <cmath>

#include <algorithm>
#include <atomic>
#include <chrono>
#include <condition_variable>
#include <map>
#include <memory>
#include <mutex>
#include <string>
#include <utility>

#include "lgh_common.hpp"

namespace lgh
{

typedef struct ncclComm *ncclComm_t;
typedef struct { char internal[128]; } ncclUniqueId;
// ... 881 lines not shown
      if (rc) { return rc; }
      if (flag < 0.0)
      {
         if (!rc_local) { set_error("lgh_comm_set_neighbors failed on another rank"); }
         return rc_local ? rc_local : LGH_ERR_COMM;
      }
      cm->allpairs = (flag > 0.5);
   }
   else if (rc_local) { return rc_local; }
   {
      LGH_HIP_CHECK(hipMalloc((void **)&cm->d_base, std::max<size_t>(n_nbr, 1) * sizeof(int)));
      LGH_HIP_CHECK(hipMalloc((void **)&cm->d_cnt, std::max<size_t>(n_nbr, 1) * sizeof(int)));
      LGH_HIP_CHECK(hipMalloc((void **)&cm->rank_src, rs.size() * sizeof(int)));
      if (n_nbr)
      {
         LGH_HIP_CHECK(hipMemcpy(cm->d_base, cm->nbr_base.data(), n_nbr * sizeof(int), hipMemcpyHostToDevice));
         LGH_HIP_CHECK(hipMemcpy(cm->d_cnt, cm->nbr_count.data(), n_nbr * sizeof(int), hipMemcpyHostToDevice));
      }
      LGH_HIP_CHECK(hipMemcpy(cm->rank_src, rs.data(), rs.size() * sizeof(int), hipMemcpyHostToDevice));
   }
   return LGH_OK;
}

int lgh_test_set_rank(lgh_ctx *c, int nranks, int rank)
{
   LGH_CHECK_ARG(c && nranks >= 1 && rank >= 0 && rank < nranks);
   c->nranks = nranks;
   c->rank = rank;
   return LGH_OK;
}
int lgh_test_word_peers(lgh_ctx *c, int nwords, long *capacity_words)
{
   LGH_CHECK_ARG(c && nwords > 0 && capacity_words);
   const long long *peers = nullptr;
   int n_peers = 0;
   const int rc = comm_word_peers(c, nwords, &peers, &n_peers);
   if (rc) { return rc; }
   const Comm *cm = c->comm;
   *capacity_words = (cm && cm->wordbuf) ? (long)cm->wordnbr * cm->wordcap : 0;
   if (peers) { LGH_HIP_CHECK(hipMemset((void *)peers, 0, (size_t)n_peers * nwords * sizeof(long long))); }
   return (cm && cm->wordbuf && cm->wordnbr == n_peers && cm->wordcap == nwords) || n_peers == 0 ? LGH_OK : LGH_ERR_COMM;
}
int lgh_test_halo_pack(lgh_ctx *c, const double *v, int ncomp, double *out)
{
   LGH_CHECK_ARG(c && v && out && c->comm && ncomp >= 1 && ncomp <= 3);
   Comm *cm = c->comm;
   if (cm->total == 0) { return LGH_OK; }
   hipLaunchKernelGGL(halo_pack_k, dim3(ceil_div((long)cm->total * ncomp, 256)), dim3(256), 0, c->stream,
                      cm->total, ncomp, c->N, cm->nodes, cm->pos, cm->cnt, v, cm->sendbuf, 0, 0, nullptr, nullptr, nullptr);
   LGH_HIP_CHECK(hipGetLastError());
   LGH_HIP_CHECK(hipMemcpyAsync(out, cm->sendbuf, (size_t)cm->bufsize * sizeof(double), hipMemcpyDeviceToDevice, c->stream));
   return LGH_OK;
}
int lgh_test_halo_combine(lgh_ctx *c, const double *in, double *v, int ncomp)
{
   LGH_CHECK_ARG(c && v && in && c->comm && ncomp >= 1 && ncomp <= 3);
   Comm *cm = c->comm;
   if (cm->total == 0) { return LGH_OK; }
   LGH_HIP_CHECK(hipMemcpyAsync(cm->recvbuf, in, (size_t)cm->bufsize * sizeof(double), hipMemcpyDeviceToDevice, c->stream));
   hipLaunchKernelGGL(halo_combine_k, dim3(ceil_div((long)cm->n_shared * ncomp, 256)), dim3(256), 0, c->stream,
                      cm->n_shared, ncomp, c->N, cm->sh_node, cm->sh_off, cm->sh_src, cm->pos, cm->cnt,
                      cm->recvbuf, v, c->nranks, 0, nullptr, nullptr, nullptr, nullptr);
   LGH_HIP_CHECK(hipGetLastError());
   return LGH_OK;
}

int lgh_test_rccl_self_sendrecv(lgh_ctx *c, int n, double *max_abs_diff)
{
   LGH_CHECK_ARG(c && c->comm && c->comm->comm && !c->comm->local && n > 0 && max_abs_diff);
   double *buf = nullptr;
   LGH_HIP_CHECK(hipMalloc((void **)&buf, 2 * (size_t)n * sizeof(double)));
   std::vector<double> h(2 * (size_t)n, 0.0);
   for (int i = 0; i < n; i++) { h[i] = 1.0 + 0.5 * i; }
   LGH_HIP_CHECK(hipMemcpy(buf, h.data(), h.size() * sizeof(double), hipMemcpyHostToDevice));
   int rc = LGH_OK;
   if (g_nccl.GroupStart() != ncclSuccess || g_nccl.Send(buf, (size_t)n, ncclFloat64, c->rank, c->comm->comm, c->stream) != ncclSuccess ||
       g_nccl.Recv(buf + n, (size_t)n, ncclFloat64, c->rank, c->comm->comm, c->stream) != ncclSuccess ||
       g_nccl.GroupEnd() != ncclSuccess)
   {
      set_error("RCCL self send/recv failed");
      rc = LGH_ERR_COMM;
   }
   if (rc == LGH_OK && hipStreamSynchronize(c->stream) != hipSuccess) { rc = LGH_ERR_HIP; }
   if (rc == LGH_OK && hipMemcpy(h.data(), buf, h.size() * sizeof(double), hipMemcpyDeviceToHost) != hipSuccess) { rc = LGH_ERR_HIP; }
   (void)hipFree(buf);
   if (rc) { return rc; }
   double d = 0.0;
   for (int i = 0; i < n; i++) { d = std::max(d, std::fabs(h[(size_t)n + i] - h[i])); }
   *max_abs_diff = d;
   return LGH_OK;
}

int lgh_groups_to_neighbors(int my_rank, int N, int n_groups, const int *group_off, const int *group_ranks,
                            const int *group_master, const int *ldof_off, const int *ldofs, double *owner,
                            int *n_nbr, int *nbr_rank, int *nbr_count, int cap_nbr, int *nbr_nodes, long cap_nodes)
{
   LGH_CHECK_ARG(my_rank >= 0 && N >= 0 && n_groups >= 0 && owner && n_nbr);
   LGH_CHECK_ARG(n_groups == 0 || (group_off && group_ranks && ldof_off && ldofs));
   for (int i = 0; i < N; i++) { owner[i] = 1.0; }
   std::vector<std::vector<int>> sets((size_t)n_groups);
   std::vector<int> order((size_t)n_groups);
   for (int g = 0; g < n_groups; g++)
// ... 21 lines not shown
   {
      if (sets[order[i]] == sets[order[i + 1]]) { set_error("lgh_groups_to_neighbors: two groups with the same rank set"); return LGH_ERR_ARG; }
   }
   std::vector<int> peers;
   for (int g = 0; g < n_groups; g++) { for (int r : sets[g]) { if (r != my_rank) { peers.push_back(r); } } }
   std::sort(peers.begin(), peers.end());
   peers.erase(std::unique(peers.begin(), peers.end()), peers.end());
   if ((int)peers.size() > cap_nbr) { set_error("lgh_groups_to_neighbors: %d peers, room for %d", (int)peers.size(), cap_nbr); return LGH_ERR_ARG; }
   LGH_CHECK_ARG(peers.empty() || (nbr_rank && nbr_count && nbr_nodes));
   long pos = 0;
   for (size_t k = 0; k < peers.size(); k++)
   {
      nbr_rank[k] = peers[k];
      int cnt = 0;
      for (int i = 0; i < n_groups; i++)
      {
         const int g = order[i];
         if (!std::binary_search(sets[g].begin(), sets[g].end(), peers[k])) { continue; }
         const int nd = ldof_off[g + 1] - ldof_off[g];
         if (pos + nd > cap_nodes) { set_error("lgh_groups_to_neighbors: node list capacity %ld too small", cap_nodes); return LGH_ERR_ARG; }
         for (int j = 0; j < nd; j++) { nbr_nodes[pos + j] = ldofs[ldof_off[g] + j]; }
         pos += nd;
         cnt += nd;
      }
      nbr_count[k] = cnt;
   }
   *n_nbr = (int)peers.size();
   return LGH_OK;
}

int lgh_halo_sum(lgh_ctx *c, double *v_h1, int ncomp)
{
   LGH_CHECK_ARG(c && v_h1 && ncomp >= 1 && ncomp <= 3);
   return halo_sum(c, v_h1, ncomp, nullptr, 0);
}

int lgh_allreduce(lgh_ctx *c, double *value, int op)
{
   LGH_CHECK_ARG(c && value);
   if (!c->multi || !c->comm) { return LGH_OK; }
   c->host_pinned[3] = *value;
   LGH_HIP_CHECK(hipMemcpyAsync(c->scal + 2, c->host_pinned + 3, sizeof(double), hipMemcpyHostToDevice, c->stream));
   int rc = allreduce_dev(c, c->scal + 2, 1, op);
   if (rc) { return rc; }
   LGH_HIP_CHECK(hipMemcpyAsync(c->host_pinned + 2, c->scal + 2, sizeof(double), hipMemcpyDeviceToHost, c->stream));
   LGH_HIP_CHECK(hipStreamSynchronize(c->stream));
   *value = c->host_pinned[2];
   return LGH_OK;
}

}
```

### laghos_amd/csrc/lgh_common.hpp

```cpp
#pragma once
#include <hip/hip_runtime.h>

#include <cstdint>
#include <cstdio>
#include <cstring>
#include <string>
#include <vector>

#include "../../include/laghos_hip.h"

namespace lgh
{

void set_error(const char *fmt, ...);

#define LGH_HIP_CHECK(expr)                                                              \
   do                                                                                    \
   {                                                                                     \
      hipError_t e_ = (expr);                                                            \
      if (e_ != hipSuccess)                                                              \
      {                                                                                  \
         lgh::set_error("HIP error %s at %s:%d: %s", hipGetErrorName(e_), __FILE__,      \
                        __LINE__, #expr);                                                \
         return LGH_ERR_HIP;                                                             \
      }                                                                                  \
   } while (0)

#define LGH_CHECK_ARG(cond)                                                              \
   do                                                                                    \
   {                                                                                     \
      if (!(cond))                                                                       \
      {                                                                                  \
         lgh::set_error("bad argument: %s (%s:%d)", #cond, __FILE__, __LINE__);          \
         return LGH_ERR_ARG;                                                             \
      }                                                                                  \
   } while (0)

constexpr int kWave = 64;

struct CgScalars
{
   double rz;
   double rz_prev;
   double den;
   double r0;
   double nom0;
   double rel_tol2;
   int done;
   int iters;
   int first;
   int pad;
};

struct Timers
{
   bool enabled = true;
   hipEvent_t ev[2] = {nullptr, nullptr};
   double t[4] = {0, 0, 0, 0};
   long c[3] = {0, 0, 0};
};

struct KTime
{
   int which = -1, max = 0, n = 0;
   std::vector<hipEvent_t> ev;
};

struct Comm;

struct MeshOrder
{
   bool structured = false, identity = true;
   int components = 0, extent[3] = {0, 0, 0};
   std::vector<int> zorder;
   std::vector<int> nnum;
   std::vector<int> ncaller;
   int *zorder_d = nullptr, *ncaller_d = nullptr, *nnum_d = nullptr;
};

}

struct lgh_ctx
{
   int dim, NE, D1D, Q1D, L1D, ND, NQ, NL, N, H1V, L2V;
   int kid;
   bool visc, vort;
   double cfl, h0, h1order;
   double q_tiny_grad;
   int device;
   hipStream_t stream;
   hipStream_t stream2;
   int on_stream2;
   hipEvent_t ev_fork, ev_join;
   void *l2run;
   const double *accel_src;
   int e_async;
   int e_lockstep;
   int ls_side = 0;
   hipEvent_t ls_ev[4][4] = {};
   long ls_stats[3] = {0, 0, 0};
   int e_polled, e_iters;
   struct { const double *S, *v; double *dS, *e_rhs; const double *src; double tol; int maxit; } e_args;
   bool own_stream;

   double *B, *G, *Bl, *W, *gamma;
   int *h1map;
   int *t_off;
   int *t_idx;
   int *t_ell;
   int t_deg;
   uint8_t *essmask[3];
   int *ess[3];
   int ess_count[3];
   double *owner;
   int cur_ess;

   double *stressJinvT, *Jac0inv, *rho0DetJ0w, *massD, *diagV, *dinvV;
   double *Jac0inv_soa;
   double *Jac0inv_e;
   int jac0_compact;
   double *massS, *ones_ne;
   double *M1h = nullptr, *M1l = nullptr;
   double *w1d = nullptr;
   int mass_rank1;
   double *dt_est_dev;
   double *erhs_q;
// ... 254 lines not shown

int force_mult_E(lgh_ctx *c, const double *sJit, const double *xE, double *yE);
int force_mult_t_L(lgh_ctx *c, const double *sJit, const double *v_h1, double *y_l2, const int *guard = nullptr);
int force_mult_t_E(lgh_ctx *c, const double *sJit, const double *vE, double *y_l2);
int h1_transpose_gather(lgh_ctx *c, int ncomp, const double *YE, double *yL);
int mass_apply_h1(lgh_ctx *c, const double *x, double *y, bool eliminate);
int mass_apply_l2(lgh_ctx *c, const double *x, double *y);
int mass_apply_E(lgh_ctx *c, int space, const double *xE, double *yE);
int mass_assemble_diag(lgh_ctx *c);
int qupdate_form(lgh_ctx *c);
int mass_data(lgh_ctx *c, const double **Dq, int *dqs, const double **Se);
int l2_mass_form(lgh_ctx *c, int *form, int *compact);
int vcg_solve(lgh_ctx *c, double *B, double *X, double rel_tol, int max_iter, int iters[3],
              const double *force_E = nullptr);
bool vcg_fused_init_ok(const lgh_ctx *c);
int partition_nodes_by_cost(lgh_ctx *c, int W, int **out, const std::vector<int> *valence = nullptr);
int make_ellz(lgh_ctx *c, unsigned **out, const int *ell = nullptr, int deg = 0);
int vcg_test_merged_faces(lgh_ctx *c, unsigned char *mask, long *n_merged);
int vcg_layout_stats(lgh_ctx *c, long out[4]);
int make_essbits(lgh_ctx *c, uint8_t **out);
void vcg_free(lgh_ctx *c);
constexpr int kDtSlots = 256, kDtSlotStride = 16;
constexpr int kYePad = 16;
bool vcg_available(const lgh_ctx *c);
int vcg_test_k1(lgh_ctx *c, const double *r, const double *d_old, const double rz[3], const double rz_prev[3], int first,
                double *YE_out, double den_out[3]);
int vcg_test_k2(lgh_ctx *c, int it, const double *YE_in, double *r, double *d, double *x, const double den[3], const double rz[3],
                const double rz_prev[3], const double alpha_prev[3], double rz_out[3], int *deferred_x);
int vcg_test_exact_sum(lgh_ctx *c, int mode, long n, int G, int E, const double *scale, const double *v, const long long *w_in,
                       long long *w_out, double *d_out, int *i_out);
int vcg_k1_form(lgh_ctx *c);
void comm_shared_nodes(const lgh_ctx *c, const uint8_t **hmask, const int **sh_node, int *n_shared);
int energy_overlap_poll(lgh_ctx *c);
int host_wait_token(lgh_ctx *c, volatile unsigned long long *word, unsigned long long token);
constexpr int kLsWord = 50;
constexpr int kLsWordsPerSet = 56;
struct LockstepWords { const long long *own; const long long *peers; int n_peers, before; };
bool l2_lockstep_possible(lgh_ctx *c);
int cg_l2_begin_lockstep(lgh_ctx *c, const double *b, double *x, double rel_tol, int max_iter);
int l2_lockstep_limit(lgh_ctx *c);
int l2_lockstep_apply(lgh_ctx *c, int it, const LockstepWords &prev, double *den_mirror);
int l2_lockstep_update(lgh_ctx *c, int it, const double *den_src, long long *word_out);
int l2_lockstep_fold(lgh_ctx *c, int it, const LockstepWords &last);
int cg_l2_end_lockstep(lgh_ctx *c, int *iters);
int comm_ranks_before(const lgh_ctx *c);
bool vcg_lockstep_ready(const lgh_ctx *c);
int cg_l2_begin(lgh_ctx *c, const double *b, double *x, double rel_tol, int max_iter);
int cg_l2_end(lgh_ctx *c, int *iters);
void cg_l2_free(lgh_ctx *c);
int cg_solve(lgh_ctx *c, int space, const double *b, double *x, double rel_tol, int max_iter,
             int *iters, bool x_is_zero);
int qupdate(lgh_ctx *c, const double *S);
int setup_rho0detj0(lgh_ctx *c, const double *x0, const double *rho0_l2, const double *rho0_q,
                    double *volume);
int interp_energy(lgh_ctx *c, int which, const double *vec, double *result);
int tg_source_2d(lgh_ctx *c, const double *S, double *out);
int test_eig(lgh_ctx *c, int dim, int n, const double *A, double *lambda, double *vec);
int test_singular(lgh_ctx *c, int dim, int n, const double *A, double *sv);
int test_sqrt(lgh_ctx *c, int n, const double *x, double *y);
int vec_set(lgh_ctx *c, double *y, double a, long n);
int vec_axpby(lgh_ctx *c, double *z, double a, const double *x, double b, const double *y, long n);
int vec_axpby_pair(lgh_ctx *c, double *z1, double a1, const double *x1, double b1, double *z2, double a2, const double *x2, double b2,
                   const double *y, long n);
int vec_neg_inplace(lgh_ctx *c, double *y, long n);
int vec_zero_list(lgh_ctx *c, double *y, const int *list, int n);
int vec_dot(lgh_ctx *c, const double *x, const double *y, const double *w, long n, double *dev_out);
// ... 71 lines not shown
```

### laghos_amd/csrc/lgh_derived.hip

```cpp
#include "lgh_common.hpp"
#include "lgh_sample.hpp"

#include <algorithm>

namespace lgh
{

struct DerivedArgs
{
   double Th[kSampleMaxTab];
   double Gh[kSampleMaxTab];
   double Tl[kSampleMaxTab];
   const double *x, *v, *e;
   double *detj, *gradv, *div, *vort, *cs;
   const int *map;
   const double *gamma;
   long N, NP;
   int NE, D, L, R1, ZPB;
   int stride;
   int need_x, need_v, need_e;
};

template <int DIM, int KMAX>
__device__ __forceinline__ void derived_component(const DerivedArgs &a, const double *__restrict__ src, const long e0, const int nz,
// ... 206 lines not shown
         }
      }
      if (a.div)
      {
         double s = Lm[0][0];
#pragma unroll
         for (int m = 1; m < DIM; m++) { s += Lm[m][m]; }
         a.div[pt] = s;
      }
      if (a.vort)
      {
         if constexpr (DIM == 2) { a.vort[pt] = Lm[1][0] - Lm[0][1]; }
         if constexpr (DIM == 3)
         {
            a.vort[pt] = Lm[2][1] - Lm[1][2];
            a.vort[NP + pt] = Lm[0][2] - Lm[2][0];
            a.vort[2 * NP + pt] = Lm[1][0] - Lm[0][1];
         }
      }
   }
}

}

using namespace lgh;

extern "C"
{

int lgh_sample_derived(lgh_ctx *c, const double *S, int R1, const double *B_h1_lat, const double *G_h1_lat, const double *B_l2_lat,
                       double *detj_out, double *gradv_out, double *div_out, double *vort_out, double *cs_out)
{
   LGH_CHECK_ARG(c && S);
   if (!B_h1_lat || !G_h1_lat || !B_l2_lat)
   {
      set_error("lgh_sample_derived: %s is NULL", !B_h1_lat ? "B_h1_lat" : (!G_h1_lat ? "G_h1_lat" : "B_l2_lat"));
      return LGH_ERR_ARG;
   }
   if (R1 < 2 || R1 > 9)
   {
      set_error("lgh_sample_derived: R1 = %d lattice points per direction is out of range (2 <= R1 <= 9)", R1);
      return LGH_ERR_ARG;
   }
   const int dim = c->dim, D = c->D1D, L = c->L1D;
   if (dim == 1 && vort_out)
   {
      set_error("lgh_sample_derived: vort_out: there is no vorticity in 1D");
      return LGH_ERR_ARG;
   }
   if (R1 * D > kSampleMaxTab || R1 * L > kSampleMaxTab)
   {
      set_error("lgh_sample_derived: lattice tables of R1 * D1D = %d entries (at most %d)", R1 * D, kSampleMaxTab);
      return LGH_ERR_UNSUPPORTED;
   }
   if (!detj_out && !gradv_out && !div_out && !vort_out && !cs_out) { return LGH_OK; }
   DerivedArgs a;
   memset(&a, 0, sizeof(a));
   std::copy(B_h1_lat, B_h1_lat + (size_t)R1 * D, a.Th);
   std::copy(G_h1_lat, G_h1_lat + (size_t)R1 * D, a.Gh);
   std::copy(B_l2_lat, B_l2_lat + (size_t)R1 * L, a.Tl);
   const int NPZ = ipow(R1, dim);
   a.x = S; a.v = S + (size_t)c->H1V; a.e = S + 2 * (size_t)c->H1V;
   a.detj = detj_out; a.gradv = gradv_out; a.div = div_out; a.vort = vort_out; a.cs = cs_out;
   a.need_v = (gradv_out || div_out || vort_out) ? 1 : 0;
   a.need_x = (a.need_v || detj_out) ? 1 : 0;
   a.need_e = cs_out ? 1 : 0;
// ... 26 lines not shown
```

### laghos_amd/csrc/lgh_diag.hip

```cpp
#include "lgh_common.hpp"
#include "lgh_diag.hpp"

#include <algorithm>
#include <climits>
#include <cmath>

namespace lgh
{

constexpr int kDiagZone = LGH_DIAG_ZONE_COUNT;
constexpr int kDiagFoldThreads = 1024;

struct DiagArgs
{
   const double *S, *B, *G, *Bl, *W, *gamma, *m;
   const int *map, *zorder;
   double *out;
   int NE, N, D, Q, L, TC;
};

__host__ __device__ constexpr int diag_kind(const int k)
{
   return (k <= 6 || k >= 14) ? 0 : ((k == 7 || k == 8 || k == 10) ? 1 : 2);
}
// ... 241 lines not shown
   const size_t S1 = (dim == 3) ? (size_t)D * D * Q : 0, S2 = (dim == 1) ? 0 : (size_t)D * (c->NQ / Q);
   const size_t fixed = (size_t)Q * (2 * D + L) + c->NQ + kDiagZone * 4 + (size_t)dim * dim * S2;
   size_t lds = 0;
   for (a.TC = dim + 1; a.TC >= 1; a.TC--)
   {
      lds = (fixed + (size_t)a.TC * (c->ND + 2 * S1)) * sizeof(double);
      if (lds <= 64 * 1024 || dim == 1) { break; }
   }
   if (a.TC < 1 || lds > 64 * 1024)
   {
      set_error("lgh_diagnostics: one zone of D1D = %d, Q1D = %d needs %zu bytes of LDS", D, Q, lds);
      return LGH_ERR_UNSUPPORTED;
   }
   const unsigned threads = (unsigned)std::min(256, 64 * ceil_div(c->NQ, 64));
   const unsigned grid = (unsigned)std::min(c->NE, 1 << 16);
   KtScope kt(c, LGH_KERNEL_DIAG);
   if (dim == 3) { hipLaunchKernelGGL(diag_zones_k<3>, dim3(grid), dim3(threads), lds, c->stream, a); }
   else if (dim == 2) { hipLaunchKernelGGL(diag_zones_k<2>, dim3(grid), dim3(threads), lds, c->stream, a); }
   else { hipLaunchKernelGGL(diag_zones_k<1>, dim3(grid), dim3(threads), lds, c->stream, a); }
   LGH_HIP_CHECK(hipGetLastError());
   return LGH_OK;
}

}

using namespace lgh;

extern "C"
{

int lgh_diagnostics_zones(lgh_ctx *c, const double *S, double *zone_out)
{
   LGH_CHECK_ARG(c && S && zone_out);
   const int rc = diag_ready(c, "lgh_diagnostics_zones");
   if (rc) { return rc; }
   return diag_zones(c, S, zone_out);
}

int lgh_diagnostics(lgh_ctx *c, const double *S, double out[LGH_DIAG_COUNT])
{
   LGH_CHECK_ARG(c && S && out);
   int rc = diag_ready(c, "lgh_diagnostics");
   if (rc) { return rc; }
   if (!c->diag_dev)
   {
      LGH_HIP_CHECK(hipMalloc((void **)&c->diag_dev, ((size_t)kDiagZone * c->NE + 32) * sizeof(double)));
   }
   double *g = c->diag_dev, *zone = g + 32;
   rc = diag_zones(c, S, zone);
   if (rc) { return rc; }
   hipLaunchKernelGGL(diag_fold_k, dim3(kDiagZone), dim3(kDiagFoldThreads), 0, c->stream, c->NE, (const double *)zone, g);
   LGH_HIP_CHECK(hipGetLastError());
   double h[18];
   LGH_HIP_CHECK(hipStreamSynchronize(c->stream));
   LGH_HIP_CHECK(hipMemcpy(h, g, sizeof(h), hipMemcpyDeviceToHost));
   double rank = (double)c->rank, zid = h[17];
   if (c->multi != 0 && c->comm)
   {
      const double own_min = h[10], own_zone = h[17];
      for (int i = 0; i < 10; i += 3)
      {
         rc = allreduce_dev(c, g + i, std::min(3, 10 - i), 0);
         if (rc) { return rc; }
      }
      rc = allreduce_dev(c, g + 10, 7, 1);
      if (rc) { return rc; }
      LGH_HIP_CHECK(hipStreamSynchronize(c->stream));
      LGH_HIP_CHECK(hipMemcpy(h, g, 17 * sizeof(double), hipMemcpyDeviceToHost));
      rank = (own_min == h[10]) ? (double)c->rank : INFINITY;
      rc = lgh_allreduce(c, &rank, 1);
      if (rc) { return rc; }
      zid = (rank == (double)c->rank) ? own_zone : INFINITY;
      rc = lgh_allreduce(c, &zid, 1);
      if (rc) { return rc; }
// ... 10 lines not shown
```

### laghos_amd/csrc/lgh_fingerprint.hip

```cpp
#include "lgh_common.hpp"

#include <algorithm>

#include "../../include/lgh_fingerprint.h"

namespace lgh
{

constexpr int kFpThreads = 256;
constexpr int kFpWaves = kFpThreads / kWave;

__device__ __forceinline__ void fp_take(const ulonglong2 w, const unsigned long long pos, unsigned long long &s, unsigned long long &x)
{
   const unsigned long long h0 = lgh_fp_word(w.x, pos), h1 = lgh_fp_word(w.y, pos + 1ULL);
   s += h0 + h1;
   x ^= h0 ^ h1;
}

__device__ __forceinline__ void fp_fold(unsigned long long &s, unsigned long long &x, unsigned long long *red)
{
   for (int d = kWave / 2; d > 0; d >>= 1)
   {
      s += __shfl_down(s, d, kWave);
      x ^= __shfl_down(x, d, kWave);
// ... 85 lines not shown
   *cap = 8L * c->ncu;
   *head = (n > 0 && ((uintptr_t)x & 15u) != 0) ? 1 : 0;
   const long np = (n - *head) >> 1;
   *blocks = std::max(1L, std::min(*cap, (np + kFpThreads - 1) / kFpThreads));
}

}

using namespace lgh;

extern "C"
{

int lgh_fingerprint_host(const void *words, long n, unsigned long long offset, unsigned long long out[2])
{
   if (!out || n < 0 || (n > 0 && !words))
   {
      set_error("lgh_fingerprint_host: bad argument (n = %ld, words %s, out %s)", n, words ? "given" : "NULL", out ? "given" : "NULL");
      return LGH_ERR_ARG;
   }
   if (((uintptr_t)words & 7u) != 0)
   {
      set_error("lgh_fingerprint_host: the words must be 8-byte aligned");
      return LGH_ERR_ARG;
   }
   out[0] = out[1] = 0ULL;
   lgh_fp_accumulate((const unsigned long long *)words, n, offset, out);
   return LGH_OK;
}

int lgh_vec_fingerprint(lgh_ctx *c, const double *x, long n, unsigned long long offset, unsigned long long out[2])
{
   LGH_CHECK_ARG(c && out && n >= 0 && (x || n == 0));
   LGH_CHECK_ARG(((uintptr_t)x & 7u) == 0);
   if (n == 0)
   {
      out[0] = out[1] = 0ULL;
      return LGH_OK;
   }
   long blocks, cap;
   int head;
   fp_shape(c, x, n, &blocks, &head, &cap);
   if (!c->fp_dev) { LGH_HIP_CHECK(hipMalloc((void **)&c->fp_dev, (2 + 2 * (size_t)cap) * sizeof(unsigned long long))); }
   {
      KtScope kt(c, LGH_KERNEL_FINGERPRINT);
      hipLaunchKernelGGL(fingerprint_k, dim3((unsigned)blocks), dim3(kFpThreads), 0, c->stream, (const unsigned long long *)x, n, head,
                         offset, c->fp_dev + 2);
      hipLaunchKernelGGL(fingerprint_fold_k, dim3(1), dim3(kFpThreads), 0, c->stream, c->fp_dev + 2, (int)blocks, c->fp_dev);
   }
   LGH_HIP_CHECK(hipGetLastError());
   unsigned long long h[2] = {0ULL, 0ULL};
   LGH_HIP_CHECK(hipMemcpyAsync(h, c->fp_dev, sizeof(h), hipMemcpyDeviceToHost, c->stream));
   LGH_HIP_CHECK(hipStreamSynchronize(c->stream));
   out[0] = h[0];
   out[1] = h[1];
   return LGH_OK;
}

int lgh_vec_fingerprint_shape(lgh_ctx *c, const double *x, long n, long out[4])
{
   LGH_CHECK_ARG(c && out && n >= 0);
   long blocks, cap;
   int head;
   fp_shape(c, x, n, &blocks, &head, &cap);
   out[0] = n > 0 ? blocks : 0;
   out[1] = kFpThreads;
   out[2] = head;
   out[3] = 2L * kFpThreads * cap;
   return LGH_OK;
}
}
```

### laghos_amd/csrc/lgh_mass.hip

```cpp
#include "lgh_common.hpp"

namespace lgh
{

struct MassArgs
{
   int NE;
   const double *B;
   const double *Dq;
   const double *Se;
   int dqs;
   const double *M1;
   const double *w1;
   const double *x;
   const int *map;
   double *y;
   double *d;
   CgScalars *cgs;
   double *partials;
   unsigned int *ticket;
   int multi;
   int iter;
   int no_y;
   double *ux, *ur;
// ... 1233 lines not shown
   s->first = 1;
   s->iters = 0;
}

static int launch_l2_update(lgh_ctx *c, const MassArgs &m, const CgVecArgs &v)
{
   MassArgs a = m;
   const int rc = mass_data(c, &a.Dq, &a.dqs, &a.Se);
   if (rc) { return rc; }
   a.M1 = c->M1l;
   a.ux = v.x;
   a.ur = v.r;
   a.partials = v.partials;
   a.ticket = v.ticket;
   a.iter = v.iter;
#define LGH_L2U(L_, NEB_) hipLaunchKernelGGL((mass_apply_l2_kron<L_, NEB_, 4>), dim3(ceil_div(c->NE, NEB_)), dim3(256), 0, c->stream, a)
   if (l2_one_round(c)) { LGH_L2U(5, 10); }
   else
   {
      switch (c->L1D)
      {
         case 1: LGH_L2U(1, 256); break;
         case 2: LGH_L2U(2, 128); break;
         case 3: LGH_L2U(3, 64); break;
         case 4: LGH_L2U(4, 32); break;
         default: LGH_L2U(5, 16); break;
      }
   }
#undef LGH_L2U
   LGH_HIP_CHECK(hipGetLastError());
   return LGH_OK;
}

int cg_solve(lgh_ctx *c, int space, const double *b, double *x, double rel_tol, int max_iter,
             int *iters, bool x_is_zero)
{
   const bool h1 = (space == LGH_SPACE_H1);
   const int n = h1 ? c->N : c->L2V;
   const bool multi = (c->multi != 0);
   int rc;
   hipLaunchKernelGGL(cg_set_tol_k, dim3(1), dim3(1), 0, c->stream, c->cgs, rel_tol * rel_tol);

   CgVecArgs v;
   memset(&v, 0, sizeof(v));
   v.n = n;
   v.b = b;
   v.x = x;
   v.r = c->cg_r;
   v.z = h1 ? c->cg_z : c->cg_r;
   v.dinv = h1 ? c->dinvV : nullptr;
   v.owner = (h1 && multi) ? c->owner : nullptr;
   v.cgs = c->cgs;
   v.partials = c->partials;
   v.ticket = c->tickets;
   v.allreduce_pending = multi ? 1 : 0;
   const uint8_t *ess = (h1 && c->cur_ess >= 0) ? c->essmask[c->cur_ess] : nullptr;
   const int nb = ceil_div(n, 256);
   const int nbu = ceil_div(n, 256 * kUpdU);

   if (!h1) { rc = vec_set(c, x, 0.0, n); if (rc) { return rc; } x_is_zero = true; }
   if (!x_is_zero)
   {
      rc = mass_apply_h1(c, x, c->cg_y, true);
      if (rc) { return rc; }
      v.yL = c->cg_y;
      hipLaunchKernelGGL(cg_init_k<true>, dim3(nb), dim3(256), 0, c->stream, v);
   }
   else { hipLaunchKernelGGL(cg_init_k<false>, dim3(nb), dim3(256), 0, c->stream, v); }
   LGH_HIP_CHECK(hipGetLastError());
   if (multi)
   {
      rc = allreduce_dev(c, &c->cgs->rz, 1, 0);
      if (rc) { return rc; }
      hipLaunchKernelGGL(cg_init_finish_k, dim3(1), dim3(1), 0, c->stream, c->cgs);
   }

   MassArgs m = base_args(c, space);
   m.x = h1 ? c->cg_z : c->cg_r;
   m.map = h1 ? c->h1map : nullptr;
   m.y = h1 ? c->YE : c->cg_y;
   m.cgs = c->cgs;
   m.partials = c->partials + c->part_stride;
   m.ticket = c->tickets + 1 * kTicketSlot;
   m.multi = multi ? 1 : 0;

   m.d = c->cg_d0;
   v.d = c->cg_d0;
   v.d_in_place = h1 ? 0 : 1;
   m.no_y = (!h1 && l2_fused_update(c)) ? 1 : 0;
   int it = 0;
   CgScalars *hs = (CgScalars *)c->host_pinned;
   int &last = c->cg_last_iters[h1 ? 0 : 1][(h1 && c->cur_ess >= 0) ? c->cur_ess : 0];
   int chunk = last > 0 ? last : 8;
   bool done = false;
   bool first_look = true;
   int looks = 0;
   while (!done)
   {
      if (multi && it > 0) { hipLaunchKernelGGL(cg_update_finish_k, dim3(1), dim3(1), 0, c->stream, c->cgs, it); }
      LGH_HIP_CHECK(hipMemcpyAsync(hs, c->cgs, sizeof(CgScalars), hipMemcpyDeviceToHost, c->stream));
      LGH_HIP_CHECK(hipStreamSynchronize(c->stream));
      if (hs->done || it >= max_iter) { break; }
      if (!first_look) { chunk = (++looks <= 2) ? 2 : std::min(64, 2 * chunk); }
      first_look = false;
      const int upto = std::min(max_iter, it + chunk);
      for (; it < upto;)
      {
         ++it;
         m.iter = it;
         kt_begin(c, h1 ? LGH_KERNEL_MASS_CG_H1 : LGH_KERNEL_MASS_CG_L2);
         rc = h1 ? launch_mass<2>(c, space, m) : launch_mass<3>(c, space, m);
         kt_end(c, h1 ? LGH_KERNEL_MASS_CG_H1 : LGH_KERNEL_MASS_CG_L2);
         if (rc) { return rc; }
         v.iter = it;
         v.ess = ess;
         if (h1 && !multi)
         {
            v.ell = c->t_ell;
            v.deg = c->t_deg;
            v.YE = c->YE;
            kt_begin(c, LGH_KERNEL_CG_UPDATE_H1);
            if (c->t_deg <= 4) { hipLaunchKernelGGL((cg_update_k<true, 4>), dim3(nbu), dim3(256), 0, c->stream, v); }
            else if (c->t_deg <= 8) { hipLaunchKernelGGL((cg_update_k<true, 8>), dim3(nbu), dim3(256), 0, c->stream, v); }
            else
            {
               hipLaunchKernelGGL(mass_gather_k, dim3(nb), dim3(256), 0, c->stream, c->N, c->t_deg,
                                  c->t_ell, c->YE, (const uint8_t *)nullptr, c->cg_y);
               v.yL = c->cg_y;
               hipLaunchKernelGGL((cg_update_k<false, 0>), dim3(nbu), dim3(256), 0, c->stream, v);
            }
            kt_end(c, LGH_KERNEL_CG_UPDATE_H1);
         }
         else
// ... 145 lines not shown
}
int l2_lockstep_fold(lgh_ctx *c, int it, const LockstepWords &last)
{
   L2Run *r = (L2Run *)c->l2run;
   if (!r || !r->active || it != r->it) { set_error("l2_lockstep_fold: iteration %d is not the last one enqueued", it); return LGH_ERR_ARG; }
   hipLaunchKernelGGL(l2_lockstep_fold_k, dim3(1), dim3(1), 0, c->stream, c->cgs, it, last);
   LGH_HIP_CHECK(hipGetLastError());
   return LGH_OK;
}
int cg_l2_end(lgh_ctx *c, int *iters);
int cg_l2_end_lockstep(lgh_ctx *c, int *iters)
{
   L2Run *r = (L2Run *)c->l2run;
   if (!r || !r->active) { return LGH_ERR_ARG; }
   r->m.ls_on = 0;
   r->m.ls_den_mirror = nullptr;
   const int inside = r->it;
   const int rc = cg_l2_end(c, iters);
   c->ls_stats[0] += 1;
   c->ls_stats[1] += inside;
   c->ls_stats[2] += r->it - inside;
   return rc;
}

int cg_l2_end(lgh_ctx *c, int *iters)
{
   L2Run *r = (L2Run *)c->l2run;
   if (!r || !r->active) { return LGH_ERR_ARG; }
   CgScalars *hs = (CgScalars *)c->host_pinned;
   int looks = 0, chunk = 2;
   while (true)
   {
      if (r->m.multi && r->it > 0) { hipLaunchKernelGGL(cg_update_finish_k, dim3(1), dim3(1), 0, c->stream, c->cgs, r->it); }
      LGH_HIP_CHECK(hipMemcpyAsync(hs, c->cgs, sizeof(CgScalars), hipMemcpyDeviceToHost, c->stream));
      LGH_HIP_CHECK(hipStreamSynchronize(c->stream));
      if (hs->done || r->it >= r->max_iter) { break; }
      chunk = (++looks <= 2) ? 2 : std::min(64, 2 * chunk);
      const int rc = l2_enqueue(c, r, std::min(r->max_iter, r->it + chunk));
      if (rc) { return rc; }
   }
   int fin = hs->iters;
   if (!hs->done && r->it >= r->max_iter) { fin = r->max_iter; }
   c->cg_last_iters[1][0] = fin;
   if (iters) { *iters = fin; }
   r->active = false;
   return LGH_OK;
}
void cg_l2_free(lgh_ctx *c)
{
   delete (L2Run *)c->l2run;
   c->l2run = nullptr;
}


}
```

### laghos_amd/csrc/lgh_profile.hip

```cpp
#include "lgh_common.hpp"
#include "lgh_diag.hpp"
#include "lgh_vcg.hpp"

#include <algorithm>
#include <cmath>
#include <cstdlib>

namespace lgh
{

constexpr int kProfSums = 7;
constexpr int kProfWords = 2 * kLimbs;
constexpr int kProfGranule = 128;
constexpr int kProfLoShift = 96;
constexpr int kProfMinE = -760;
constexpr int kProfShards = 16, kProfShardStride = 16;
constexpr int kProfPack = 2 * (kLimbs + 1);
constexpr int kProfMaxGrid = 2048;

struct ProfScratch
{
   long long *words;
   unsigned long long *flags;
   unsigned long long *count;
// ... 433 lines not shown
      c[0] += (long long)p[0] * 4294967296LL;
      c[kLimbs - 1] += (long long)p[kLimbs + 2] + (long long)p[kLimbs + 1] * 4294967296LL;
      for (int j = 1; j < kLimbs; j++) { c[kLimbs - 1 + j] = (long long)p[kLimbs + 2 + j]; }
      bool neg = false;
      for (int pass = 0; pass < 2; pass++)
      {
         for (int j = 2 * kLimbs - 2; j > 0; j--)
         {
            const long long carry = c[j] >> 32;
            c[j] -= carry * 4294967296LL;
            c[j - 1] += carry;
         }
         if (pass == 1 || c[0] >= 0) { break; }
         neg = true;
         for (int j = 0; j < 2 * kLimbs - 1; j++) { c[j] = -c[j]; }
      }
      long long top[kLimbs], bot[kLimbs];
      for (int j = 0; j < kLimbs; j++) { top[j] = c[j]; bot[j] = (j < kLimbs - 1) ? c[kLimbs + j] : 0; }
      const double val = exact_value(bot, E - 32 * kLimbs) + exact_value(top, E);
      o[1 + k] = (flags[i] != 0.0) ? __builtin_nan("") : (neg ? -val : val);
   }
   o[8] = rmin[r];
   o[9] = -rmax[r];
   if (r == 0) { s.out[(size_t)R * LGH_PROFILE_COLS] = excl[0]; }
}

}

using namespace lgh;

extern "C" int lgh_profile(lgh_ctx *c, const double *S, const lgh_profile_spec *spec, double *out, long *n_excluded)
{
   LGH_CHECK_ARG(c && S && spec && out && n_excluded);
   if (!c->setup_done)
   {
      set_error("lgh_profile: lgh_setup_rho0detj0 has not been called (rho0DetJ0w is not set)");
      return LGH_ERR_ARG;
   }
   const int dim = c->dim, D = c->D1D, Q = c->Q1D, L = c->L1D;
   LGH_CHECK_ARG(spec->axis >= 0 && spec->axis <= 3 && (spec->axis == 3 || spec->axis < dim));
   LGH_CHECK_ARG(spec->nbins >= 1 && spec->nbins <= LGH_PROFILE_MAX_BINS);
   LGH_CHECK_ARG(std::isfinite(spec->lo) && std::isfinite(spec->hi) && spec->lo < spec->hi && std::isfinite(spec->hi - spec->lo));
   if (spec->axis == 3)
   {
      for (int k = 0; k < dim; k++) { LGH_CHECK_ARG(std::isfinite(spec->origin[k])); }
   }
   const int R = spec->nbins + 2;
   if (R > c->prof_rows)
   {
      if (c->prof_dev) { LGH_HIP_CHECK(hipFree(c->prof_dev)); c->prof_dev = nullptr; c->prof_rows = 0; }
      LGH_HIP_CHECK(hipMalloc(&c->prof_dev, prof_layout(nullptr, R).bytes));
      c->prof_rows = R;
   }
   ProfArgs a;
   a.s = prof_layout(c->prof_dev, c->prof_rows);
   a.S = S; a.B = c->B; a.G = c->G; a.Bl = c->Bl; a.W = c->W; a.gamma = c->gamma; a.m = c->rho0DetJ0w;
   a.map = c->h1map;
   const MeshOrder *o = mesh_order(c);
   a.zorder = o ? o->zorder_d : nullptr;
   a.NE = c->NE; a.N = c->N; a.D = D; a.Q = Q; a.L = L;
   a.axis = spec->axis; a.nbins = spec->nbins;
   a.lo = spec->lo;
   a.inv_w = (double)spec->nbins / (spec->hi - spec->lo);
   for (int k = 0; k < 3; k++) { a.origin[k] = (spec->axis == 3 && k < dim) ? spec->origin[k] : 0.0; }
   const char *fenv = getenv("LGH_PROFILE_FOLD");
   a.fold = fenv ? std::max(0, atoi(fenv)) : 8;
// ... 59 lines not shown
```

### laghos_amd/csrc/lgh_qupdate.hip

```cpp
#include "lgh_qpoint.hpp"
#include "lgh_qrows.hpp"

namespace lgh
{

int qupdate_form(lgh_ctx *c);
int qupdate(lgh_ctx *c, const double *S)
{
   QArgs a = q_base(c);
   a.x = S;
   a.v = S + c->H1V;
   a.e = S + 2 * (size_t)c->H1V;
   a.result = c->dt_est_dev;
   a.Jac0inv_e = (c->jac0_compact == 1) ? c->Jac0inv_e : nullptr;
   const bool keep = !c->stress_store && a.erhs_q && a.force_e && c->v_snap;
   if (keep) { a.stressJinvT = nullptr; }
   const int form = qupdate_form(c);
   const int rc = (form == 1) ? launch_qrows(c, a) : launch_q<QMODE_UPDATE>(c, a);
   c->qgen++;
   c->stress_current = (rc == LGH_OK && !keep) ? 1 : 0;
   c->fused_ftv_valid = (rc == LGH_OK && a.erhs_q && c->v_snap) ? 1 : 0;
   c->fused_f1_valid = (rc == LGH_OK && a.force_e) ? 1 : 0;
   if (c->fused_ftv_valid)
   {
      LGH_HIP_CHECK(hipMemcpyAsync(c->v_snap, S + c->H1V, sizeof(double) * (size_t)c->H1V, hipMemcpyDeviceToDevice, c->stream));
   }
   return rc;
}

int qupdate_form(lgh_ctx *c)
{
   const char *fenv = getenv("LGH_Q_FORM");
   return (qrows_available(c) && !(fenv && fenv[0] == '0')) ? 1 : 0;
}

int interp_energy(lgh_ctx *c, int which, const double *vec, double *result)
{
   QArgs a = q_base(c);
   a.result = c->scal;
   int rc;
   if (which == 0)
   {
      a.e = vec;
      rc = launch_q<QMODE_IE>(c, a);
   }
   else
   {
      a.v = vec;
      rc = launch_q<QMODE_KE>(c, a);
   }
   if (rc) { return rc; }
   if (c->multi != 0)
   {
      rc = allreduce_dev(c, c->scal, 1, 0);
      if (rc) { return rc; }
   }
   LGH_HIP_CHECK(hipMemcpyAsync(c->host_pinned, c->scal, sizeof(double), hipMemcpyDeviceToHost, c->stream));
   LGH_HIP_CHECK(hipStreamSynchronize(c->stream));
// ... 112 lines not shown
```

### laghos_amd/csrc/lgh_sample.hip

```cpp
#include "lgh_common.hpp"
#include "lgh_sample.hpp"

#include <algorithm>

namespace lgh
{

struct SampleArgs
{
   double Th[kSampleMaxTab];
   double Tl[kSampleMaxTab];
   const double *h1src[6];
   double *h1out[6];
   const double *l2src[2];
   double *e_out, *rho_out, *p_out;
   const int *map;
   const double *gamma;
   int nh, nl;
   int NE, D, L, R1, ZPB;
   int strideA, strideB;
};

template <int DIM>
__global__ void __launch_bounds__(kSampleThreads) sample_fields_k(const SampleArgs a)
// ... 48 lines not shown
   for (int i = t; i < nh * npts; i += kSampleThreads)
   {
      const int f = i / npts, zp = i - f * npts, z = zp / NPZ, p = zp - z * NPZ;
      a.h1out[f][p0 + zp] = sample_last(D, R1, preH, p, Th, in + (size_t)(z * NF + f) * sin);
   }
   if (nl > 0)
   {
      for (int zp = t; zp < npts; zp += kSampleThreads)
      {
         const int z = zp / NPZ, p = zp - z * NPZ;
         const double ev = sample_last(L, R1, preH, p, Tl, in + (size_t)(z * NF + nh) * sin);
         if (a.e_out) { a.e_out[p0 + zp] = ev; }
         if (nl > 1)
         {
            const double rv = sample_last(L, R1, preH, p, Tl, in + (size_t)(z * NF + nh + 1) * sin);
            if (a.rho_out) { a.rho_out[p0 + zp] = rv; }
            if (a.p_out) { a.p_out[p0 + zp] = (a.gamma[e0 + z] - 1.0) * rv * fmax(ev, 0.0); }
         }
      }
   }
}

}

using namespace lgh;

extern "C"
{

int lgh_sample_fields(lgh_ctx *c, const double *S, const double *rho_l2, int R1, const double *B_h1_lat, const double *B_l2_lat,
                      double *x_out, double *v_out, double *e_out, double *rho_out, double *p_out)
{
   LGH_CHECK_ARG(c && S && B_h1_lat && B_l2_lat);
   if (R1 < 2 || R1 > 9)
   {
      set_error("lgh_sample_fields: R1 = %d lattice points per direction is out of range (2 <= R1 <= 9)", R1);
      return LGH_ERR_ARG;
   }
   if (!rho_l2 && (rho_out || p_out))
   {
      set_error("lgh_sample_fields: %s needs the density dofs, but rho_l2 is NULL", rho_out ? "rho_out" : "p_out");
      return LGH_ERR_ARG;
   }
   const int dim = c->dim, D = c->D1D, L = c->L1D;
   if (R1 * D > kSampleMaxTab || R1 * L > kSampleMaxTab)
   {
      set_error("lgh_sample_fields: lattice tables of R1 * D1D = %d entries (at most %d)", R1 * D, kSampleMaxTab);
      return LGH_ERR_UNSUPPORTED;
   }
   if (!x_out && !v_out && !e_out && !rho_out && !p_out) { return LGH_OK; }
   SampleArgs a;
   memset(&a, 0, sizeof(a));
   std::copy(B_h1_lat, B_h1_lat + (size_t)R1 * D, a.Th);
   std::copy(B_l2_lat, B_l2_lat + (size_t)R1 * L, a.Tl);
   const int NPZ = ipow(R1, dim);
   const size_t NP = (size_t)c->NE * NPZ;
   for (int k = 0; k < dim; k++)
   {
      if (x_out) { a.h1src[a.nh] = S + (size_t)k * c->N; a.h1out[a.nh++] = x_out + k * NP; }
   }
   for (int k = 0; k < dim; k++)
   {
      if (v_out) { a.h1src[a.nh] = S + (size_t)(dim + k) * c->N; a.h1out[a.nh++] = v_out + k * NP; }
   }
   if (e_out || rho_out || p_out)
   {
// ... 30 lines not shown
```

### laghos_amd/csrc/lgh_sedov.hip

```cpp
#include "lgh_common.hpp"

#include <algorithm>
#include <cmath>
#include <vector>

namespace lgh
{

struct SedovPar
{
   double dim, gamma, rho0, E, omega;
   double a, b, c, d, e;
   double al0, al1, al2, al3, al4, al5;
   double V0, Vv, V2, Vs;
   double alpha;
};
static_assert(sizeof(SedovPar) == 21 * sizeof(double), "SedovPar is the flat parameter block");
struct SedovShock { double r2, U, rho1, rho2, v2, p2; };


static const double kGx[5] = {1.488743389816312108848260011297200e-01, 4.333953941292471907992659431657842e-01,
                              6.794095682990244062343273651148736e-01, 8.650633666889845107320966884234930e-01,
                              9.739065285171717200779640120844521e-01};
static const double kGw[5] = {2.955242247147528701738929946513383e-01, 2.692667193099963550912269215694694e-01,
// ... 408 lines not shown
{
   LGH_CHECK_ARG(par && dim >= 1 && dim <= 3 && gamma > 1.0 && rho0 > 0.0 && blast_energy > 0.0);
   if (omega != 0.0)
   {
      set_error("lgh_sedov_setup: only omega = 0 (uniform initial density) is supported");
      return LGH_ERR_UNSUPPORTED;
   }
   SedovPar s;
   s.dim = dim; s.gamma = gamma; s.rho0 = rho0; s.E = blast_energy; s.omega = omega;
   sedov_setup(s);
   std::copy(reinterpret_cast<double *>(&s), reinterpret_cast<double *>(&s) + 21, par);
   return LGH_OK;
}

int lgh_sedov_shock(const double par[21], double t, double shock[6])
{
   LGH_CHECK_ARG(par && shock && t > 0.0);
   const SedovShock k = sedov_shock(par_from(par), t);
   shock[0] = k.r2; shock[1] = k.U; shock[2] = k.rho1; shock[3] = k.rho2; shock[4] = k.v2; shock[5] = k.p2;
   return LGH_OK;
}

int lgh_sedov_eval_point(const double par[21], double t, double r, double *rho, double *v, double *P)
{
   LGH_CHECK_ARG(par && rho && v && P && t > 0.0);
   const SedovPar s = par_from(par);
   sedov_point(s, sedov_shock(s, t), r, *rho, *v, *P);
   return LGH_OK;
}

int lgh_sedov_eval(lgh_ctx *c, const double par[21], double t, long n, const double *r, double *rho, double *v, double *P)
{
   LGH_CHECK_ARG(c && par && t > 0.0 && n >= 0 && (n == 0 || (r && rho && v && P)));
   if (n == 0) { return LGH_OK; }
   const SedovPar s = par_from(par);
   hipLaunchKernelGGL(sedov_eval_k, dim3((unsigned)((n + 255) / 256)), dim3(256), 0, c->stream, s, sedov_shock(s, t), n, r,
                      rho, v, P);
   LGH_HIP_CHECK(hipGetLastError());
   return LGH_OK;
}

int lgh_compute_density(lgh_ctx *c, const double *x_h1, double *rho_l2)
{
   LGH_CHECK_ARG(c && x_h1 && rho_l2);
   if (c->dim == 1) { return density_1d(c, x_h1, rho_l2); }
   const int grid = std::min(c->NE, 2048);
   DevBuf scratch;
   if (scratch.alloc((size_t)grid * c->NL * (c->NL + 1) * sizeof(double))) { set_error("lgh_compute_density: hipMalloc failed"); return LGH_ERR_HIP; }
   const size_t lds = ((size_t)c->dim * c->ND + c->NQ + c->NL) * sizeof(double);
   if (c->dim == 3)
   {
      hipLaunchKernelGGL(density_project_k<3>, dim3(grid), dim3(256), lds, c->stream, c->NE, c->N, c->D1D, c->Q1D, c->L1D,
                         c->h1map, c->B, c->G, c->Bl, c->W, x_h1, c->rho0DetJ0w, (double *)scratch.p, rho_l2);
   }
   else if (c->dim == 2)
   {
      hipLaunchKernelGGL(density_project_k<2>, dim3(grid), dim3(256), lds, c->stream, c->NE, c->N, c->D1D, c->Q1D, c->L1D,
                         c->h1map, c->B, c->G, c->Bl, c->W, x_h1, c->rho0DetJ0w, (double *)scratch.p, rho_l2);
   }
   LGH_HIP_CHECK(hipGetLastError());
   LGH_HIP_CHECK(hipStreamSynchronize(c->stream));
   return LGH_OK;
}

int lgh_sedov_density_error(lgh_ctx *c, const double *x_h1, const double *rho_l2, const double par[21], double t,
                            const double origin[3], int n1d, const double *weights, const double *B_h1,
                            const double *G_h1, const double *B_l2, double *err2)
{
   LGH_CHECK_ARG(c && x_h1 && rho_l2 && par && origin && weights && B_h1 && G_h1 && B_l2 && err2 && t > 0.0 &&
                 n1d >= 1 && n1d <= 64);
   if (c->dim == 1) { return sedov_density_error_1d(c, x_h1, rho_l2, par, t, origin, n1d, weights, B_h1, G_h1, B_l2, err2); }
   const int D = c->D1D, L = c->L1D;
   std::vector<double> tab;
   tab.insert(tab.end(), weights, weights + n1d);
   tab.insert(tab.end(), B_h1, B_h1 + (size_t)n1d * D);
   tab.insert(tab.end(), G_h1, G_h1 + (size_t)n1d * D);
   tab.insert(tab.end(), B_l2, B_l2 + (size_t)n1d * L);
   DevBuf dtab, part;
   if (dtab.alloc(tab.size() * sizeof(double)) || part.alloc((size_t)c->NE * sizeof(double)))
   {
      set_error("lgh_sedov_density_error: hipMalloc failed");
      return LGH_ERR_HIP;
   }
   LGH_HIP_CHECK(hipMemcpy(dtab.p, tab.data(), tab.size() * sizeof(double), hipMemcpyHostToDevice));
   const double *dw = (const double *)dtab.p, *dB = dw + n1d, *dG = dB + (size_t)n1d * D, *dBl = dG + (size_t)n1d * D;
   const SedovPar s = par_from(par);
   const SedovShock k = sedov_shock(s, t);
   const size_t lds = ((size_t)c->dim * c->ND + c->NL + 256) * sizeof(double);
   const int grid = std::min(c->NE, 1 << 16);
   if (c->dim == 3)
   {
      hipLaunchKernelGGL(sedov_density_error_k<3>, dim3(grid), dim3(256), lds, c->stream, c->NE, c->N, D, L, n1d, c->h1map,
                         dB, dG, dBl, dw, x_h1, rho_l2, s, k, origin[0], origin[1], origin[2], (double *)part.p);
   }
   else if (c->dim == 2)
   {
      hipLaunchKernelGGL(sedov_density_error_k<2>, dim3(grid), dim3(256), lds, c->stream, c->NE, c->N, D, L, n1d, c->h1map,
                         dB, dG, dBl, dw, x_h1, rho_l2, s, k, origin[0], origin[1], 0.0, (double *)part.p);
   }
   LGH_HIP_CHECK(hipGetLastError());
   hipLaunchKernelGGL(sum_ordered_k, dim3(1), dim3(1024), 0, c->stream, c->NE, (const double *)part.p, c->scal);
   LGH_HIP_CHECK(hipGetLastError());
   if (c->multi != 0)
// ... 11 lines not shown
```

### laghos_amd/csrc/lgh_vcg.hip

```cpp
#include "lgh_vcg.hpp"

namespace lgh
{
typedef unsigned v4u_ __attribute__((ext_vector_type(4)));


template <int D, int Q, int NEB>
__global__ void __launch_bounds__(Q *Q *NEB, (Q >= 8) ? 1 : 2)
vcg_apply_3d(const VcgArgs a, const int nbatch)
{
   constexpr int NQ = Q * Q * Q, ND = D * D * D;
   constexpr int SX = (ND > D * Q * Q) ? ND : D * Q * Q;
   constexpr int SA = D * D * Q;
   constexpr int SAE = (SA > D * Q * D) ? SA : D * Q * D;
   constexpr int OFF_A = kVC * SX, OFF_IN = OFF_A + kVC * SAE;
   constexpr int PER = OFF_IN + kVC * ND + 1;
   constexpr int NT = Q * Q * NEB;
   constexpr int GPT = (NEB * ND + NT - 1) / NT;
   __shared__ double smem[NEB * PER];
   __shared__ double red[48];

   if (a.s->all_done) { return; }
   const int tid = threadIdx.x;
   const int tx = tid % Q, ty = (tid / Q) % Q, eb = tid / (Q * Q);
// ... 2301 lines not shown
   else { if (u2) { LGH_K2P_LAUNCH(true, 2, 2); } else if (occ3) { LGH_K2P_LAUNCH(true, 1, 6); } else { LGH_K2P_LAUNCH(true, 1, 4); } }
#undef LGH_K2P_LAUNCH
   kt_end(c, LGH_KERNEL_CG_UPDATE_H1);
}

int vcg_solve(lgh_ctx *c, double *B, double *X, double rel_tol, int max_iter, int iters[3], const double *force_E)
{
   if (!vcg_supported(c)) { return LGH_ERR_UNSUPPORTED; }
   VcgPlan plan;
   int rc = vcg_prepare(c, B, X, rel_tol, plan, true);
   if (rc) { return rc; }
   VcgArgs &a = plan.a;
   VcgAux *aux = plan.aux;
   const bool k2p = plan.k2p;
   const bool multi = c->multi != 0;
   const size_t N = (size_t)c->N;
   VcgScalars *ds = (VcgScalars *)c->vcg_s;
   const int nb = ceil_div((long)N, 256);
   const HaloNodeAlias *alias = (aux->ord && aux->o_alias.nodes) ? &aux->o_alias : nullptr;

   a.partials = c->vcg_partials;
   a.ticket = c->vcg_tickets;
   if (force_E)
   {
      if (multi || c->t_deg > 8) { set_error("vcg_solve: fused init is single-rank, degree <= 8"); return LGH_ERR_ARG; }
      if (aux->ellf && aux->essbits)
      {
         hipLaunchKernelGGL(vcg_init_force_z_k, dim3(nb), dim3(256), 0, c->stream, a, force_E, 8u * (unsigned)c->ND, aux->ellf, B);
      }
      else { hipLaunchKernelGGL(vcg_init_force_k<8>, dim3(nb), dim3(256), 0, c->stream, a, force_E, c->ND, B, aux->o_ellc ? aux->o_ellc : c->t_ell, c->t_deg); }
   }
   else
   {
      if (aux->ord) { LGH_HIP_CHECK(hipMemsetAsync(a.x, 0, kVC * N * sizeof(double), c->stream)); }
      hipLaunchKernelGGL(vcg_init_k, dim3(nb), dim3(256), 0, c->stream, a);
   }
   LGH_HIP_CHECK(hipGetLastError());
   if (multi)
   {
      rc = allreduce_dev(c, ds->rz, kVC, 0);
      if (rc) { return rc; }
      hipLaunchKernelGGL(vcg_init_finish_k, dim3(1), dim3(1), 0, c->stream, ds);
   }

   VcgScalars *hs = (VcgScalars *)(c->host_pinned + 32);
   static_assert(sizeof(VcgScalars) <= 64 * sizeof(double), "pinned staging too small");
   int it = 0, looks = 0;
   bool energy_polled = false;
   const bool ls = c->e_lockstep == 1 && multi && a.rzl && aux->ls_ready && (a.n_shared == 0 || a.nx_den == kVC + 1);
   const int ls_limit = ls ? std::min(l2_lockstep_limit(c), max_iter) : 0;
   const int ls_before = ls ? comm_ranks_before(c) : 0;
   auto ls_words = [&](const int set_it) { return LockstepWords{a.rzl + (set_it % 3) * kLimbWords, a.rzl_peers, a.n_rz_peers, ls_before}; };
   const bool ls_side = ls && c->ls_side != 0 && c->stream2 != nullptr;
   auto side = [&](auto &&f) -> int {
      if (!ls_side) { return f(); }
      std::swap(c->stream, c->stream2);
      const int r = f();
      std::swap(c->stream, c->stream2);
      return r;
   };
   auto hand_over = [&](hipEvent_t ev, const bool from_side) -> int {
      if (!ls_side) { return LGH_OK; }
      LGH_HIP_CHECK(hipEventRecord(ev, from_side ? c->stream2 : c->stream));
      LGH_HIP_CHECK(hipStreamWaitEvent(from_side ? c->stream : c->stream2, ev, 0));
      return LGH_OK;
   };
   if (ls_side) { rc = hand_over(c->ev_fork, false); if (rc) { return rc; } }
// ... 567 lines not shown
```

### laghos_amd/host/laghos.cpp

```cpp
#include <algorithm>
#include <cerrno>
#include <chrono>
#include <cmath>
#include <cstdlib>
#include <cstring>
#include <fstream>
#include <sys/stat.h>
#include <iomanip>
#include <iostream>
#include <limits>
#include <memory>
#include <sstream>
#include <string>

#include "laghos_solver.hpp"
#include "sedov_exact.hpp"
#include "vtk_output.hpp"
#include "checkpoint.hpp"
#include "history.hpp"
#include "profile.hpp"

using namespace laghos;

namespace
// ... 876 lines not shown
      s->prof_last = h.ti;
      if (s->t >= o.t_final || (o.max_tsteps >= 0 && s->steps > o.max_tsteps)) { s->last_step = true; }
      return s.release();
   }
   s->S.FromHost(S0);
   s->S_old.SetSize(s->S.Size());
   s->ode->Init(*s->hydro);
   s->energy_init = s->hydro->InternalEnergy(s->S) + s->hydro->KineticEnergy(s->S);
   s->hydro->ResetTimeStepEstimate();
   s->t = 0.0;
   s->dt = s->hydro->GetTimeStepEstimate(s->S);
   if (o.paraview && !DumpParaview(s.get(), 0)) { return nullptr; }
   if (o.hist_steps > 0 && !(HistoryOpen(s.get(), -1) && HistoryRecord(s.get(), 0))) { return nullptr; }
   if (o.prof_steps > 0 && !ProfileRecord(s.get(), 0)) { return nullptr; }
   return s.release();
}

void laghos_sim_destroy(laghos_sim *s) { delete s; }

int laghos_sim_step(laghos_sim *s)
{
   Options &o = s->opt;
   auto &hydro = *s->hydro;
   const bool root = (o.rank == 0) && !o.quiet;
   while (true)
   {
      if (s->last_step) { return 0; }
      if (s->t + s->dt >= o.t_final)
      {
         s->dt = o.t_final - s->t;
         s->last_step = true;
      }
      if (s->steps == o.max_tsteps) { s->last_step = true; }
      hydro.Copy(s->S_old, s->S);
      s->t_old = s->t;
      hydro.ResetTimeStepEstimate();
      s->ode->Step(s->S, s->t, s->dt);
      s->steps++;
      const double dt_est = hydro.GetTimeStepEstimate(s->S);
      if (dt_est < s->dt)
      {
         s->dt *= 0.85;
         if (s->dt < std::numeric_limits<double>::epsilon())
         {
            s->error = "The time step crashed!";
            std::fprintf(stderr, "%s\n", s->error.c_str());
            return -1;
         }
         s->t = s->t_old;
         hydro.Copy(s->S, s->S_old);
         hydro.ResetQuadratureData();
         s->repeats++;
         if (root) { std::cout << "Repeating step " << s->ti << std::endl; }
         if (s->steps < o.max_tsteps) { s->last_step = false; }
         if (s->last_step && o.ckpt_steps > 0 && s->ti > 1 && !PeriodicCheckpoint(s, s->ti - 1)) { return -1; }
         if (s->last_step && o.hist_steps > 0 && s->ti - 1 > s->hist_last && !HistoryRecord(s, s->ti - 1)) { return -1; }
         if (s->last_step && o.prof_steps > 0 && s->ti - 1 > s->prof_last && !ProfileRecord(s, s->ti - 1)) { return -1; }
         continue;
      }
      else if (dt_est > 1.25 * s->dt) { s->dt *= 1.02; }

      if (s->last_step || (s->ti % o.vis_steps) == 0)
      {
         const double sqrt_norm = hydro.ENorm(s->S);
         if (root)
         {
            std::cout << std::fixed;
            std::cout << "step " << std::setw(5) << s->ti << ",\tt = " << std::setw(5) << std::setprecision(4)
                      << s->t << ",\tdt = " << std::setw(5) << std::setprecision(6) << s->dt
// ... 417 lines not shown
```

### laghos_amd/host/laghos_solver.cpp

```cpp
#include "laghos_solver.hpp"

#include <cmath>
#include <cstdlib>
#include <cstring>
#include <iomanip>
#include <iostream>
#include <limits>

namespace laghos
{
namespace hydrodynamics
{

void AbortWithLghError(const char *where)
{
   std::fprintf(stderr, "%s failed: %s\n", where, lgh_last_error());
   std::abort();
}

LagrangianHydroOperator::LagrangianHydroOperator(const Discretization &d, const std::vector<double> &S0,
                                                 const std::vector<double> &rho0_l2,
                                                 const std::vector<double> &gamma,
                                                 const std::vector<double> &rho0_q, double cfl,
                                                 double cgt, int cgiter, int device, const char *nccl_id)
// ... 64 lines not shown
   LGH_VERIFY(lgh_setup_rho0detj0(ctx, x0.Read(), r_l2.Read(), r_q.Read(), &vol));
   double ne = (double)NE;
   if (multi)
   {
      LGH_VERIFY(lgh_allreduce(ctx, &vol, 0));
      LGH_VERIFY(lgh_allreduce(ctx, &ne, 0));
   }
   volume = vol;
   qdata->h0 = std::pow(vol / ne, 1.0 / dim) / (double)d.tab.order_v;
   LGH_VERIFY(lgh_set_h0(ctx, qdata->h0));

   one.SetSize(L2Vsize);
   LGH_VERIFY(lgh_vec_set(ctx, one.Write(), 1.0, L2Vsize));
   rhs.SetSize(H1Vsize);
   e_rhs.SetSize(L2Vsize);
   source_type = d.SourceType();
   if (source_type == 1) { e_source.SetSize(L2Vsize); }
   if (source_type == 2)
   {
      std::vector<double> acc((size_t)H1Vsize, 0.0);
      for (long i = H1Vsize / dim; i < 2 * (H1Vsize / dim); i++) { acc[i] = -1.0; }
      accel_src.FromHost(acc);
      LGH_VERIFY(lgh_set_velocity_source(ctx, accel_src.Read()));
   }
   B.SetSize(d.N);
   LGH_VERIFY(lgh_sync(ctx));
}

LagrangianHydroOperator::~LagrangianHydroOperator() { lgh_destroy(ctx); }

void LagrangianHydroOperator::Mult(const Vector &S, Vector &dS_dt) const
{
   UpdateMesh(S);
   LGH_VERIFY(lgh_vec_copy(ctx, dS_dt.Write(), S.Read() + H1Vsize, H1Vsize));
   UpdateQuadratureData(S);
   if (source_type == 1) { LGH_VERIFY(lgh_tg_source_2d(ctx, S.Read(), e_source.Write())); }
   LGH_VERIFY(lgh_solve_energy_begin(ctx, S.Read(), S.Read() + H1Vsize, dS_dt.Write(), e_rhs.Write(),
                                     source_type == 1 ? e_source.Read() : nullptr, cg_rel_tol, cg_max_iter));
   SolveVelocity(S, dS_dt);
   int it = 0;
   LGH_VERIFY(lgh_solve_energy_end(ctx, &it));
   qdata_is_current = false;
}

void LagrangianHydroOperator::SolveVelocity(const Vector &S, Vector &dS_dt) const
{
   UpdateQuadratureData(S);
   int it = 0;
   LGH_VERIFY(lgh_solve_velocity(ctx, S.Read(), dS_dt.Write(), nullptr, rhs.Write(), B.Write(),
                                 cg_rel_tol, cg_max_iter, &it));
}

void LagrangianHydroOperator::SolveEnergy(const Vector &S, const Vector &v, Vector &dS_dt) const
{
   UpdateQuadratureData(S);
   int it = 0;
   if (source_type == 1) { LGH_VERIFY(lgh_tg_source_2d(ctx, S.Read(), e_source.Write())); }
   LGH_VERIFY(lgh_solve_energy(ctx, S.Read(), v.Read(), dS_dt.Write(), e_rhs.Write(),
                               source_type == 1 ? e_source.Read() : nullptr,
                               cg_rel_tol, cg_max_iter, &it));
}

void LagrangianHydroOperator::UpdateQuadratureData(const Vector &S) const
{
   unsigned long gen = 0;
   int f1 = 0, ftv = 0;
   LGH_VERIFY(lgh_quadrature_generation(ctx, &gen, &f1, &ftv));
   if (qdata_is_current && gen == qdata_gen) { return; }
// ... 111 lines not shown
                                        std::vector<double> &v, std::vector<double> &p) const
{
   const long n = (long)r.size();
   Vector dev(4 * n);
   std::vector<double> h(4 * n, 0.0);
   std::copy(r.begin(), r.end(), h.begin());
   dev.FromHost(h);
   double *d = dev.Write();
   LGH_VERIFY(lgh_sedov_eval(ctx, par, t, n, d, d + n, d + 2 * n, d + 3 * n));
   Sync();
   dev.ToHost(h);
   rho.assign(h.begin() + n, h.begin() + 2 * n);
   v.assign(h.begin() + 2 * n, h.begin() + 3 * n);
   p.assign(h.begin() + 3 * n, h.end());
}

double LagrangianHydroOperator::AllReduce(double v, int op) const
{
   if (disc.part.nranks > 1) { LGH_VERIFY(lgh_allreduce(ctx, &v, op)); }
   return v;
}
void LagrangianHydroOperator::Add(Vector &z, double a, const Vector &x, double b, const Vector &y) const
{
   LGH_VERIFY(lgh_vec_axpby(ctx, z.Write(), a, x.Read(), b, y.Read(), z.Size()));
}
void LagrangianHydroOperator::Add2(Vector &z1, double a1, const Vector &x1, double b1, Vector &z2, double a2, const Vector &x2, double b2,
                                   const Vector &y) const
{
   LGH_VERIFY(lgh_vec_axpby_pair(ctx, z1.Write(), a1, x1.Read(), b1, z2.Write(), a2, x2.Read(), b2, y.Read(), z1.Size()));
}
void LagrangianHydroOperator::Copy(Vector &y, const Vector &x) const
{
   LGH_VERIFY(lgh_vec_copy(ctx, y.Write(), x.Read(), y.Size()));
}
void LagrangianHydroOperator::Sync() const { LGH_VERIFY(lgh_sync(ctx)); }

const TimingData &LagrangianHydroOperator::Timing() const
{
   double t[4];
   long c[3];
   LGH_VERIFY(lgh_get_timers(ctx, t, c));
   timer.sw_cgH1 = t[0];
   timer.sw_cgL2 = t[1];
   timer.sw_force = t[2];
   timer.sw_qdata = t[3];
   timer.H1iter = c[0];
   timer.L2iter = c[1];
   timer.quad_tstep = c[2];
   return timer;
}
void LagrangianHydroOperator::ResetTiming() { LGH_VERIFY(lgh_reset_timers(ctx)); }
void LagrangianHydroOperator::EnableTimers(bool on) { LGH_VERIFY(lgh_enable_timers(ctx, on ? 1 : 0)); }

void LagrangianHydroOperator::PrintTimingData(bool IamRoot, int steps, bool fom) const
{
   const TimingData &tm = Timing();
   double T[5] = {tm.sw_cgH1, tm.sw_cgL2, tm.sw_force, tm.sw_qdata, 0.0};
   T[4] = T[0] + T[2] + T[3];
   for (int i = 0; i < 5; i++) { T[i] = -AllReduce(-T[i], 1); }
   double l2work = (double)tm.L2dof * (double)tm.L2iter, quads = (double)tm.quad_tstep, zones = (double)NE;
   l2work = AllReduce(l2work, 0);
   quads = AllReduce(quads, 0);
   zones = AllReduce(zones, 0);
   if (!IamRoot) { return; }
   using namespace std;
   const long H1iter = tm.H1iter / dim;
// ... 70 lines not shown
   t += dt;
}

void RK3SSPSolver::Init(hydrodynamics::LagrangianHydroOperator &op)
{
   ODESolver::Init(op);
   k.SetSize(op.Size());
   y.SetSize(op.Size());
}
void RK3SSPSolver::Step(Vector &S, double &t, double &dt)
{
   f->Mult(S, k);
   f->Add(y, 1.0, S, dt, k);
   f->Mult(y, k);
   f->Add(y, 1.0, y, dt, k);
   f->Add(y, 3. / 4, S, 1. / 4, y);
   f->Mult(y, k);
   f->Add(y, 1.0, y, dt, k);
   f->Add(S, 1. / 3, S, 2. / 3, y);
   t += dt;
}

void RK4Solver::Init(hydrodynamics::LagrangianHydroOperator &op)
{
   ODESolver::Init(op);
   k.SetSize(op.Size());
   y.SetSize(op.Size());
   z.SetSize(op.Size());
}

void RK4Solver::Step(Vector &S, double &t, double &dt)
{
   f->Mult(S, k);
   f->Add2(y, 1.0, S, dt / 2, z, 1.0, S, dt / 6, k);
   f->Mult(y, k);
   f->Add2(y, 1.0, S, dt / 2, z, 1.0, z, dt / 3, k);
   f->Mult(y, k);
   f->Add2(y, 1.0, S, dt, z, 1.0, z, dt / 3, k);
   f->Mult(y, k);
   f->Add(S, 1.0, z, dt / 6, k);
   t += dt;
}

void ExplicitRKSolver::Init(hydrodynamics::LagrangianHydroOperator &op)
{
   ODESolver::Init(op);
   y.SetSize(op.Size());
   k.resize(s);
   for (int i = 0; i < s; i++) { k[i].SetSize(op.Size()); }
}
void ExplicitRKSolver::Step(Vector &S, double &t, double &dt)
{
   f->Mult(S, k[0]);
   for (int l = 0, i = 1; i < s; i++)
   {
      f->Add(y, 1.0, S, a[l++] * dt, k[0]);
      for (int j = 1; j < i; j++) { f->Add(y, 1.0, y, a[l++] * dt, k[j]); }
      f->Mult(y, k[i]);
   }
   for (int i = 0; i < s; i++) { f->Add(S, 1.0, S, b[i] * dt, k[i]); }
   t += dt;
}
const double RK6Solver::a[] = {
   .6e-1,
   .1923996296296296296296296296296296296296e-1,
   .7669337037037037037037037037037037037037e-1,
   .35975e-1,
   0.,
   .107925,
   1.318683415233148260919747276431735612861,
   0.,
// ... 73 lines not shown
```

### laghos_amd/host/laghos_solver.hpp

```cpp
#pragma once
#include <memory>

#include "fem.hpp"
#include "laghos_assembly.hpp"

namespace laghos
{
namespace hydrodynamics
{

struct TimingData
{
   double sw_cgH1 = 0, sw_cgL2 = 0, sw_force = 0, sw_qdata = 0;
   long L2dof = 0, H1iter = 0, L2iter = 0, quad_tstep = 0;
};

class QUpdate
{
   lgh_ctx *ctx;

public:
   explicit QUpdate(lgh_ctx *c) : ctx(c) {}
   void UpdateQuadratureData(const Vector &S, QuadratureData &) { LGH_VERIFY(lgh_qupdate(ctx, S.Read())); }
};
// ... 37 lines not shown
   void UpdateMesh(const Vector &) const {}
   void UpdateQuadratureData(const Vector &S) const;
   double GetTimeStepEstimate(const Vector &S) const;
   void ResetTimeStepEstimate() const;
   void ResetQuadratureData() const { qdata_is_current = false; LGH_VERIFY(lgh_reset_quadrature_data(ctx)); }
   double InternalEnergy(const Vector &S) const;
   double KineticEnergy(const Vector &S) const;
   double ENorm(const Vector &S) const;
   void ComputeDensity(const Vector &S, Vector &rho) const;
   double SedovDensityError(const Vector &S, const Vector &rho, const double par[21], double t,
                            const double origin[3], int err_order) const;
   void SampleFields(const Vector &S, const Vector &rho, int R, Vector &out) const;
   long SamplePoints(int R) const;
   enum { DERIVED_DIV = 1, DERIVED_VORT = 2, DERIVED_GRAD = 4, DERIVED_DETJ = 8, DERIVED_CS = 16, DERIVED_ALL = 31 };
   void SampleDerived(const Vector &S, int R, unsigned mask, Vector &out, long offset = 0) const;
   long DerivedSize(int R) const;
   void Diagnostics(const Vector &S, double out[LGH_DIAG_COUNT]) const;
   void Profile(const Vector &S, const lgh_profile_spec &spec, double *rows, long *n_excluded) const;
   void SedovEval(const double par[21], double t, const std::vector<double> &r, std::vector<double> &rho, std::vector<double> &v,
                  std::vector<double> &p) const;
   void PrintTimingData(bool IamRoot, int steps, bool fom) const;
   const TimingData &Timing() const;
   void ResetTiming();
   void EnableTimers(bool on);
   lgh_ctx *Context() const { return ctx; }
   long GlobalH1Size() const { return H1GTVSize; }
   long GlobalL2Size() const { return L2GTVSize; }
   int Rank() const { return disc.part.rank; }
   int NRanks() const { return disc.part.nranks; }
   double AllReduce(double v, int op) const;
   void Add(Vector &z, double a, const Vector &x, double b, const Vector &y) const;
   void Add2(Vector &z1, double a1, const Vector &x1, double b1, Vector &z2, double a2, const Vector &x2, double b2, const Vector &y) const;
   void Copy(Vector &y, const Vector &x) const;
   void Sync() const;
};

}

class ODESolver
{
protected:
   hydrodynamics::LagrangianHydroOperator *f = nullptr;

public:
   virtual ~ODESolver() {}
   virtual void Init(hydrodynamics::LagrangianHydroOperator &op) { f = &op; }
   virtual void Step(Vector &S, double &t, double &dt) = 0;
   virtual int Stages() const = 0;
};

class ForwardEulerSolver : public ODESolver
{
   Vector k;

public:
   void Init(hydrodynamics::LagrangianHydroOperator &op) override;
   void Step(Vector &S, double &t, double &dt) override;
   int Stages() const override { return 1; }
};
class RK2Solver : public ODESolver
{
   Vector k, x1;
   double a;

public:
   explicit RK2Solver(double a_ = 0.5) : a(a_) {}
// ... 57 lines not shown
```

Before: 1612 Mdofs*steps/s.

## Defer independent vector updates onto a side stream overlapping quadrature update

```diff
diff --git a/include/laghos_hip.h b/include/laghos_hip.h
--- a/include/laghos_hip.h
+++ b/include/laghos_hip.h
@@ -98,6 +98,8 @@
 
 int lgh_vec_set(lgh_ctx *ctx, double *y, double a, long n);
 int lgh_vec_copy(lgh_ctx *ctx, double *y, const double *x, long n);
+int lgh_vec_copy_deferred(lgh_ctx *ctx, double *y, const double *x, long n);
+int lgh_vec_axpby_deferred(lgh_ctx *ctx, double *z, double a, const double *x, double b, const double *y, long n);
 int lgh_vec_axpby_pair(lgh_ctx *ctx, double *z1, double a1, const double *x1, double b1, double *z2, double a2, const double *x2, double b2,
                        const double *y, long n);
 int lgh_vec_axpby(lgh_ctx *ctx, double *z, double a, const double *x, double b,
diff --git a/laghos_amd/_lib.py b/laghos_amd/_lib.py
--- a/laghos_amd/_lib.py
+++ b/laghos_amd/_lib.py
@@ -68,6 +68,8 @@
     "lgh_solve_energy_end": (_I, [_P, c_int_p]),
     "lgh_vec_set": (_I, [_P, _P, _D, _L]),
     "lgh_vec_copy": (_I, [_P, _P, _P, _L]),
+    "lgh_vec_copy_deferred": (_I, [_P, _P, _P, _L]),
+    "lgh_vec_axpby_deferred": (_I, [_P, _P, _D, _P, _D, _P, _L]),
     "lgh_vec_axpby": (_I, [_P, _P, _D, _P, _D, _P, _L]),
     "lgh_vec_axpby_pair": (_I, [_P, _P, _D, _P, _D, _P, _D, _P, _D, _P, _L]),
     "lgh_vec_dot": (_I, [_P, _P, _P, _L, c_dbl_p]),
diff --git a/laghos_amd/csrc/lgh_1d.hip b/laghos_amd/csrc/lgh_1d.hip
--- a/laghos_amd/csrc/lgh_1d.hip
+++ b/laghos_amd/csrc/lgh_1d.hip
@@ -745,7 +745,7 @@
    LGH_TRY(alloc_zero(&c->diagV, (size_t)N));
    LGH_TRY(alloc_zero(&c->dinvV, (size_t)N));
    LGH_TRY(alloc_zero(&c->dt_est_dev, (size_t)kDtSlotStride * (1 + kDtSlots)));
-   LGH_TRY(alloc_zero(&c->dev_flags, (size_t)8));
+   LGH_TRY(alloc_zero(&c->dev_flags, (size_t)16));
    LGH_TRY(alloc_zero(&c->YE, std::max(nmap, (size_t)c->L2V)));
    const size_t nv = std::max<size_t>((size_t)N, (size_t)c->L2V);
    LGH_TRY(alloc_zero(&c->cg_r, nv));
diff --git a/laghos_amd/csrc/lgh_api.hip b/laghos_amd/csrc/lgh_api.hip
--- a/laghos_amd/csrc/lgh_api.hip
+++ b/laghos_amd/csrc/lgh_api.hip
@@ -61,6 +61,25 @@
       z2[i] = make_double2(fma(a2, q.x, __dmul_rn(b2, y0.x)), fma(a2, q.y, __dmul_rn(b2, y0.y)));
    }
 }
+__global__ void __launch_bounds__(256) vec_copy_k(double *__restrict__ y, const double *__restrict__ x, long n)
+{
+   for (long i = blockIdx.x * (long)blockDim.x + threadIdx.x; i < n; i += (long)gridDim.x * blockDim.x) { y[i] = x[i]; }
+}
+template <bool XA>
+__global__ void __launch_bounds__(256) vec_copy2_k(double2 *__restrict__ y, const double *__restrict__ x, long n2)
+{
+   const long stride = (long)gridDim.x * blockDim.x;
+   long i = blockIdx.x * (long)blockDim.x + threadIdx.x;
+   auto ld = [&](const long j) { return XA ? ((const double2 *)x)[j] : make_double2(x[2 * j], x[2 * j + 1]); };
+   for (; i + stride < n2; i += 2 * stride)
+   {
+      const double2 x0 = ld(i), x1 = ld(i + stride);
+      y[i] = x0;
+      y[i + stride] = x1;
+   }
+   if (i < n2) { y[i] = ld(i); }
+}
+__global__ void set_int_k(int *p, int v) { *p = v; }
 __global__ void __launch_bounds__(256) vec_neg_k(double *y, long n)
 {
    for (long i = blockIdx.x * (long)blockDim.x + threadIdx.x; i < n; i += (long)gridDim.x * blockDim.x) { y[i] = -y[i]; }
@@ -159,6 +178,21 @@
    if (rc) { return rc; }
    return vec_axpby(c, z2, a2, x2, b2, y, n);
 }
+int vec_copy(lgh_ctx *c, double *y, const double *x, long n)
+{
+   if (n <= 0 || y == x) { return LGH_OK; }
+   if (n >= 4096 && (((uintptr_t)y | (uintptr_t)x) & 7u) == 0)
+   {
+      const long head = ((uintptr_t)y & 15u) ? 1 : 0, n2 = (n - head) / 2, tail = n - head - 2 * n2;
+      if (head) { hipLaunchKernelGGL(vec_copy_k, dim3(1), dim3(64), 0, c->stream, y, x, 1L); }
+      if (((uintptr_t)(x + head) & 15u) == 0) { hipLaunchKernelGGL(vec_copy2_k<true>, dim3(grid_for(n2)), dim3(256), 0, c->stream, (double2 *)(y + head), x + head, n2); }
+      else { hipLaunchKernelGGL(vec_copy2_k<false>, dim3(grid_for(n2)), dim3(256), 0, c->stream, (double2 *)(y + head), x + head, n2); }
+      if (tail) { hipLaunchKernelGGL(vec_copy_k, dim3(1), dim3(64), 0, c->stream, y + n - 1, x + n - 1, 1L); }
+   }
+   else { hipLaunchKernelGGL(vec_copy_k, dim3(grid_for(n)), dim3(256), 0, c->stream, y, x, n); }
+   LGH_HIP_CHECK(hipGetLastError());
+   return LGH_OK;
+}
 int vec_neg_inplace(lgh_ctx *c, double *y, long n)
 {
    if (n <= 0) { return LGH_OK; }
@@ -280,6 +314,103 @@
    return LGH_OK;
 }
 
+static int create_stream2(lgh_ctx *c)
+{
+   const char *penv = getenv("LGH_STREAM2_PRIORITY");
+   const char want = (penv && (penv[0] == 'd' || penv[0] == 'h')) ? penv[0] : 'l';
+   int least = 0, greatest = 0;
+   if (want != 'd' && hipDeviceGetStreamPriorityRange(&least, &greatest) == hipSuccess && least != greatest)
+   {
+      LGH_HIP_CHECK(hipStreamCreateWithPriority(&c->stream2, hipStreamNonBlocking, want == 'h' ? greatest : least));
+   }
+   else { LGH_HIP_CHECK(hipStreamCreateWithFlags(&c->stream2, hipStreamNonBlocking)); }
+   LGH_HIP_CHECK(hipEventCreateWithFlags(&c->ev_fork, hipEventDisableTiming));
+   LGH_HIP_CHECK(hipEventCreateWithFlags(&c->ev_join, hipEventDisableTiming));
+   LGH_HIP_CHECK(hipEventCreateWithFlags(&c->ev_side, hipEventDisableTiming));
+   LGH_HIP_CHECK(hipEventCreateWithFlags(&c->ev_side_in, hipEventDisableTiming));
+   return LGH_OK;
+}
+static bool energy_overlap_ok(const lgh_ctx *c)
+{
+   const bool on = !(getenv("LGH_OVERLAP") && getenv("LGH_OVERLAP")[0] == '0');
+   return on && (c->multi == 0 || comm_second_channel(c)) && !c->timers.enabled && !(c->ktime && c->ktime->which >= 0) && vcg_available(c);
+}
+bool side_ok(const lgh_ctx *c)
+{
+   return c->side_on && c->dim != 1 && c->multi == 0 && c->own_stream && !c->on_stream2 && energy_overlap_ok(c);
+}
+int side_begin(lgh_ctx *c)
+{
+   if (!c->stream2)
+   {
+      const int rc = create_stream2(c);
+      if (rc) { return rc; }
+   }
+   if (!c->side_fork_valid) { LGH_HIP_CHECK(hipEventRecord(c->ev_side_in, c->stream)); }
+   c->side_fork_valid = 1;
+   LGH_HIP_CHECK(hipStreamWaitEvent(c->stream2, c->ev_side_in, 0));
+   std::swap(c->stream, c->stream2);
+   c->on_stream2 = 1;
+   return LGH_OK;
+}
+void side_dst(lgh_ctx *c, const void *dst, size_t bytes)
+{
+   const char *lo = (const char *)dst, *hi = lo + bytes;
+   if (c->side_fork_valid && c->side_q.lo && lo < c->side_q.hi && c->side_q.lo < hi) { c->side_fork_valid = 0; }
+}
+int side_fork(lgh_ctx *c)
+{
+   if (!c->stream2)
+   {
+      const int rc = create_stream2(c);
+      if (rc) { return rc; }
+   }
+   LGH_HIP_CHECK(hipEventRecord(c->ev_side_in, c->stream));
+   c->side_fork_valid = 1;
+   c->side_q = {nullptr, nullptr};
+   return LGH_OK;
+}
+int side_end(lgh_ctx *c, const void *dst, size_t bytes)
+{
+   const hipError_t e = hipEventRecord(c->ev_side, c->stream);
+   std::swap(c->stream, c->stream2);
+   c->on_stream2 = 0;
+   c->side_pending = 1;
+   c->side_seq++;
+   if (dst && bytes)
+   {
+      if (c->side_nrng < 8) { c->side_rng[c->side_nrng] = {(const char *)dst, (const char *)dst + bytes}; }
+      c->side_nrng++;
+   }
+   LGH_HIP_CHECK(e);
+   return LGH_OK;
+}
+static void side_joined(lgh_ctx *c)
+{
+   c->side_pending = 0;
+   c->side_nrng = 0;
+}
+int side_join(lgh_ctx *c)
+{
+   if (!c->side_pending) { return LGH_OK; }
+   LGH_HIP_CHECK(hipStreamWaitEvent(c->stream, c->ev_side, 0));
+   side_joined(c);
+   return LGH_OK;
+}
+bool side_writes(const lgh_ctx *c, const void *p, size_t bytes)
+{
+   if (!c->side_pending) { return false; }
+   if (c->side_nrng > 8) { return true; }
+   const char *lo = (const char *)p, *hi = lo + bytes;
+   for (int i = 0; i < c->side_nrng; i++) { if (lo < c->side_rng[i].hi && c->side_rng[i].lo < hi) { return true; } }
+   return false;
+}
+static int record_join(lgh_ctx *c)
+{
+   c->side_seq_join = c->side_seq;
+   return (hipEventRecord(c->ev_join, c->stream) == hipSuccess) ? LGH_OK : LGH_ERR_HIP;
+}
+
 int energy_overlap_poll(lgh_ctx *c)
 {
    if (c->e_async != 1 || c->e_polled) { return LGH_OK; }
@@ -287,7 +418,7 @@
    std::swap(c->stream, c->stream2);
    c->on_stream2 = 1;
    int rc = cg_l2_end(c, &it);
-   if (rc == LGH_OK) { rc = (hipEventRecord(c->ev_join, c->stream) == hipSuccess) ? LGH_OK : LGH_ERR_HIP; }
+   if (rc == LGH_OK) { rc = record_join(c); }
    std::swap(c->stream, c->stream2);
    c->on_stream2 = 0;
    if (rc) { return rc; }
@@ -386,6 +517,10 @@
       c->q_tiny_grad = env ? atof(env) : 1e-30;
       c->stress_store = 1;
       c->stress_current = 0;
+   }
+   {
+      const char *env = getenv("LGH_SIDE");
+      c->side_on = (env && env[0] == '0') ? 0 : 1;
    }
    c->h0 = 0.0;
    c->device = cfg->device;
@@ -525,7 +660,7 @@
          LGH_TRY(dev_alloc_zero(&c->erhs_q, (size_t)c->L2V));
          LGH_TRY(dev_alloc_zero(&c->v_snap, (size_t)c->H1V));
       }
-      LGH_TRY(dev_alloc_zero(&c->dev_flags, (size_t)8));
+      LGH_TRY(dev_alloc_zero(&c->dev_flags, (size_t)16));
       c->mass_rank1 = -1;
       env = getenv("LGH_FUSED_F1");
       if (c->dim == 3 && !(env && env[0] == '0')) { LGH_TRY(dev_alloc_zero(&c->force_e_q, nmap * dim + (size_t)dim * c->ND)); }
@@ -587,6 +722,8 @@
       (void)hipStreamDestroy(c->stream2);
       (void)hipEventDestroy(c->ev_fork);
       (void)hipEventDestroy(c->ev_join);
+      if (c->ev_side) { (void)hipEventDestroy(c->ev_side); }
+      if (c->ev_side_in) { (void)hipEventDestroy(c->ev_side_in); }
    }
    for (auto &ring : c->ls_ev) { for (hipEvent_t e : ring) { if (e) { (void)hipEventDestroy(e); } } }
    extern void lgh_comm_free(lgh_ctx *);
@@ -599,6 +736,11 @@
 int lgh_sync(lgh_ctx *c)
 {
    LGH_CHECK_ARG(c);
+   if (c->side_pending)
+   {
+      LGH_HIP_CHECK(hipStreamSynchronize(c->stream2));
+      side_joined(c);
+   }
    LGH_HIP_CHECK(hipStreamSynchronize(c->stream));
    return LGH_OK;
 }
@@ -661,6 +803,7 @@
 int lgh_fused_force_mult(lgh_ctx *c, double *y_h1)
 {
    LGH_CHECK_ARG(c && y_h1);
+   LGH_ENTRY(c);
    if (!(c->force_e_q && c->fused_f1_valid)) { set_error("lgh_fused_force_mult: no fused F.1 on hand"); return LGH_ERR_ARG; }
    int rc = h1_transpose_gather(c, c->dim, c->force_e_q, y_h1);
    if (rc == LGH_OK && c->multi != 0) { rc = halo_sum(c, y_h1, c->dim); }
@@ -669,9 +812,9 @@
 int lgh_fused_force_mult_transpose(lgh_ctx *c, double *y_l2)
 {
    LGH_CHECK_ARG(c && y_l2);
+   LGH_ENTRY(c);
    if (!(c->erhs_q && c->fused_ftv_valid)) { set_error("lgh_fused_force_mult_transpose: no fused F^T v on hand"); return LGH_ERR_ARG; }
-   LGH_HIP_CHECK(hipMemcpyAsync(y_l2, c->erhs_q, sizeof(double) * (size_t)c->L2V, hipMemcpyDeviceToDevice, c->stream));
-   return LGH_OK;
+   return vec_copy(c, y_l2, c->erhs_q, c->L2V);
 }
 int lgh_quadrature_generation(lgh_ctx *c, unsigned long *gen, int *f1_valid, int *ftv_valid)
 {
@@ -692,6 +835,7 @@
 int lgh_mass_data_form(lgh_ctx *c, int *form)
 {
    LGH_CHECK_ARG(c && form);
+   LGH_ENTRY(c);
    if (c->dim == 1) { *form = 0; return LGH_OK; }
    const double *Dq, *Se;
    int dqs;
@@ -703,6 +847,7 @@
 int lgh_mass_data_changed(lgh_ctx *c)
 {
    LGH_CHECK_ARG(c);
+   LGH_ENTRY(c);
    c->mass_rank1 = -1;
    c->mass_gen++;
    if (c->dim == 1) { return mass_changed_1d(c); }
@@ -715,6 +860,7 @@
 int lgh_set_dt_est(lgh_ctx *c, double v)
 {
    LGH_CHECK_ARG(c);
+   LGH_ENTRY(c);
    hipLaunchKernelGGL(dt_est_set_k, dim3(1), dim3(256), 0, c->stream, c->dt_est_dev, v);
    LGH_HIP_CHECK(hipGetLastError());
    return LGH_OK;
@@ -722,6 +868,7 @@
 int lgh_get_dt_est(lgh_ctx *c, double *v)
 {
    LGH_CHECK_ARG(c && v);
+   LGH_ENTRY(c);
    const unsigned long long token = ++c->look_token;
    hipLaunchKernelGGL(dt_est_fold_k, dim3(1), dim3(256), 0, c->stream, c->dt_est_dev, c->dev_flags + 4, c->host_pinned_dev + 8, token);
    LGH_HIP_CHECK(hipGetLastError());
@@ -732,7 +879,7 @@
    *v = c->host_pinned[8];
    if (*(const int *)(c->host_pinned + 9) != 0)
    {
-      LGH_HIP_CHECK(hipMemsetAsync(c->dev_flags + 4, 0, sizeof(int), c->stream));
+      hipLaunchKernelGGL(set_int_k, dim3(1), dim3(1), 0, c->stream, c->dev_flags + 4, 0);
       set_error("lgh_solve_energy was given a velocity other than the state's while the stress was kept in registers "
                 "(lgh_qupdate_store_stress(ctx, 0)): its right-hand side is NaN");
       return LGH_ERR_ARG;
@@ -744,6 +891,7 @@
                         double *volume)
 {
    LGH_CHECK_ARG(c && x0 && rho0_l2 && rho0_q && volume);
+   LGH_ENTRY(c);
    invalidate_fused(c);
    c->mass_rank1 = -1;
    c->mass_gen++;
@@ -758,6 +906,7 @@
 int lgh_force_mult(lgh_ctx *c, const double *x_l2, double *y_h1)
 {
    LGH_CHECK_ARG(c && x_l2 && y_h1);
+   LGH_ENTRY(c);
    int rc = stress_on_hand(c, "lgh_force_mult");
    if (rc) { return rc; }
    if (c->dim == 1) { return force_mult_1d(c, x_l2, y_h1); }
@@ -773,6 +922,7 @@
 int lgh_force_mult_transpose(lgh_ctx *c, const double *v_h1, double *y_l2)
 {
    LGH_CHECK_ARG(c && v_h1 && y_l2);
+   LGH_ENTRY(c);
    const int rc0 = stress_on_hand(c, "lgh_force_mult_transpose");
    if (rc0) { return rc0; }
    if (c->dim == 1) { return force_mult_t_1d(c, v_h1, y_l2); }
@@ -791,18 +941,21 @@
 int lgh_mass_eliminate_rhs(lgh_ctx *c, double *b)
 {
    LGH_CHECK_ARG(c && b);
+   LGH_ENTRY(c);
    if (c->cur_ess < 0) { return LGH_OK; }
    return vec_zero_list(c, b, c->ess[c->cur_ess], c->ess_count[c->cur_ess]);
 }
 int lgh_mass_mult(lgh_ctx *c, int space, const double *x, double *y)
 {
    LGH_CHECK_ARG(c && x && y && (space == LGH_SPACE_H1 || space == LGH_SPACE_L2));
+   LGH_ENTRY(c);
    if (c->dim == 1) { return mass_apply_1d(c, space, x, y, true); }
    return space == LGH_SPACE_H1 ? mass_apply_h1(c, x, y, true) : mass_apply_l2(c, x, y);
 }
 int lgh_mass_mult_full(lgh_ctx *c, int space, const double *x, double *y)
 {
    LGH_CHECK_ARG(c && x && y && (space == LGH_SPACE_H1 || space == LGH_SPACE_L2));
+   LGH_ENTRY(c);
    if (c->dim == 1) { return mass_apply_1d(c, space, x, y, false); }
    return space == LGH_SPACE_H1 ? mass_apply_h1(c, x, y, false) : mass_apply_l2(c, x, y);
 }
@@ -811,6 +964,7 @@
                  int *iters)
 {
    LGH_CHECK_ARG(c && b && x && (space == LGH_SPACE_H1 || space == LGH_SPACE_L2));
+   LGH_ENTRY(c);
    if (c->dim == 1) { return cg_1d(c, space, b, x, rel_tol, max_iter, iters, false); }
    return cg_solve(c, space, b, x, rel_tol, max_iter, iters, false);
 }
@@ -818,6 +972,7 @@
 int lgh_l2_mass_solve_local(lgh_ctx *c, const double *b, double *x)
 {
    LGH_CHECK_ARG(c && b && x);
+   LGH_ENTRY(c);
    if (c->dim != 1)
    {
       set_error("lgh_l2_mass_solve_local: the zone-local energy solve belongs to the 1D (full-assembly) path; 2D/3D run the energy CG");
@@ -829,6 +984,7 @@
 int lgh_qupdate(lgh_ctx *c, const double *S)
 {
    LGH_CHECK_ARG(c && S);
+   if (side_writes(c, S, sizeof(double) * (2 * (size_t)c->H1V + (size_t)c->L2V))) { LGH_ENTRY(c); }
    RoctxRange range("QUpdate-UpdateQuadratureData");
    timer_start(c);
    kt_begin(c, LGH_KERNEL_QUPDATE);
@@ -848,7 +1004,7 @@
 {
    if (!one_l2) { return true; }
    int *flag = c->dev_flags + 1;
-   if (hipMemsetAsync(flag, 0, sizeof(int), c->stream) != hipSuccess) { return false; }
+   hipLaunchKernelGGL(set_int_k, dim3(1), dim3(1), 0, c->stream, flag, 0);
    hipLaunchKernelGGL(not_all_ones_k, dim3(ceil_div(c->L2V, 256)), dim3(256), 0, c->stream, one_l2, (long)c->L2V, flag);
    int h = 1;
    if (hipMemcpyAsync(&h, flag, sizeof(int), hipMemcpyDeviceToHost, c->stream) != hipSuccess) { return false; }
@@ -872,6 +1028,7 @@
                        double *rhs_h1, double *work_B, double rel_tol, int max_iter, int *h1_iters)
 {
    LGH_CHECK_ARG(c && S && dS_dt && rhs_h1 && work_B);
+   LGH_ENTRY(c);
    const int dim = c->dim, N = c->N;
    double *dv = dS_dt + c->H1V;
    int rc;
@@ -969,8 +1126,8 @@
    }
    for (int cc = 0; cc < dim; cc++)
    {
-      LGH_HIP_CHECK(hipMemcpyAsync(work_B, rhs_h1 + (size_t)cc * N, sizeof(double) * N,
-                                   hipMemcpyDeviceToDevice, c->stream));
+      rc = vec_copy(c, work_B, rhs_h1 + (size_t)cc * N, N);
+      if (rc) { return rc; }
       rc = lgh_mass_set_essential_tdofs(c, cc);
       if (rc) { return rc; }
       rc = lgh_mass_eliminate_rhs(c, work_B);
@@ -986,7 +1143,7 @@
    return LGH_OK;
 }
 
-__global__ void __launch_bounds__(256) vec_differs_k(const double *__restrict__ a, const double *__restrict__ b, const long n, int *flag)
+__global__ void __launch_bounds__(256) vec_differs_k(const double *__restrict__ a, const double *__restrict__ b, const long n, int *flag, int *next)
 {
    const long stride = (long)gridDim.x * blockDim.x, t = (long)blockIdx.x * blockDim.x + threadIdx.x;
    bool diff = false;
@@ -1005,6 +1162,7 @@
       for (long i = t; i < n; i += stride) { diff = diff || __double_as_longlong(a[i]) != __double_as_longlong(b[i]); }
    }
    if (diff) { *flag = 1; }
+   if (t == 0) { *next = 0; }
 }
 __global__ void __launch_bounds__(256) erhs_take_or_poison_k(double *__restrict__ y, const double *__restrict__ x, const long n, const int *__restrict__ flag, int *err)
 {
@@ -1028,9 +1186,9 @@
    RoctxRange range("SolveEnergy-ForcePA");
    if (c->erhs_q && c->fused_ftv_valid)
    {
-      int *flag = c->dev_flags + (c->on_stream2 ? 2 : 0);
-      LGH_HIP_CHECK(hipMemsetAsync(flag, 0, sizeof(int), c->stream));
-      hipLaunchKernelGGL(vec_differs_k, dim3(grid_for((c->H1V + 1) / 2)), dim3(256), 0, c->stream, v_h1, c->v_snap, (long)c->H1V, flag);
+      const int s2 = c->on_stream2 ? 1 : 0, odd = (int)(c->differs_calls[s2]++ & 1u);
+      int *flag = c->dev_flags + (s2 ? 2 : 0) + (odd ? 8 : 0), *next = c->dev_flags + (s2 ? 2 : 0) + (odd ? 0 : 8);
+      hipLaunchKernelGGL(vec_differs_k, dim3(grid_for((c->H1V + 1) / 2)), dim3(256), 0, c->stream, v_h1, c->v_snap, (long)c->H1V, flag, next);
       LGH_HIP_CHECK(hipGetLastError());
       if (c->stress_current)
       {
@@ -1052,6 +1210,7 @@
                      const double *e_source, double rel_tol, int max_iter, int *l2_iters)
 {
    LGH_CHECK_ARG(c && S && v_h1 && dS_dt && e_rhs);
+   LGH_ENTRY(c);
    (void)S;
    double *de = dS_dt + 2 * (size_t)c->H1V;
    if (c->dim == 1)
@@ -1081,25 +1240,6 @@
    return LGH_OK;
 }
 
-static int create_stream2(lgh_ctx *c)
-{
-   const char *penv = getenv("LGH_STREAM2_PRIORITY");
-   const char want = (penv && (penv[0] == 'd' || penv[0] == 'h')) ? penv[0] : 'l';
-   int least = 0, greatest = 0;
-   if (want != 'd' && hipDeviceGetStreamPriorityRange(&least, &greatest) == hipSuccess && least != greatest)
-   {
-      LGH_HIP_CHECK(hipStreamCreateWithPriority(&c->stream2, hipStreamNonBlocking, want == 'h' ? greatest : least));
-   }
-   else { LGH_HIP_CHECK(hipStreamCreateWithFlags(&c->stream2, hipStreamNonBlocking)); }
-   LGH_HIP_CHECK(hipEventCreateWithFlags(&c->ev_fork, hipEventDisableTiming));
-   LGH_HIP_CHECK(hipEventCreateWithFlags(&c->ev_join, hipEventDisableTiming));
-   return LGH_OK;
-}
-static bool energy_overlap_ok(const lgh_ctx *c)
-{
-   const bool on = !(getenv("LGH_OVERLAP") && getenv("LGH_OVERLAP")[0] == '0');
-   return on && (c->multi == 0 || comm_second_channel(c)) && !c->timers.enabled && !(c->ktime && c->ktime->which >= 0) && vcg_available(c);
-}
 int lgh_solve_energy_begin(lgh_ctx *c, const double *S, const double *v_h1, double *dS_dt, double *e_rhs,
                            const double *e_source, double rel_tol, int max_iter)
 {
@@ -1189,6 +1329,7 @@
    {
       c->e_polled = 0;
       LGH_HIP_CHECK(hipStreamWaitEvent(c->stream, c->ev_join, 0));
+      if (c->side_seq_join == c->side_seq) { side_joined(c); }
       const int counted = (c->e_iters == 0) ? 1 : c->e_iters;
       c->timers.c[1] += counted;
       if (l2_iters) { *l2_iters += counted; }
@@ -1203,33 +1344,65 @@
    std::swap(c->stream, c->stream2);
    c->on_stream2 = 1;
    int rc = cg_l2_end(c, &it);
-   if (rc == LGH_OK) { rc = (hipEventRecord(c->ev_join, c->stream) == hipSuccess) ? LGH_OK : LGH_ERR_HIP; }
+   if (rc == LGH_OK) { rc = record_join(c); }
    std::swap(c->stream, c->stream2);
    c->on_stream2 = 0;
    if (rc) { return rc; }
    LGH_HIP_CHECK(hipStreamWaitEvent(c->stream, c->ev_join, 0));
+   if (c->side_seq_join == c->side_seq) { side_joined(c); }
    const int counted = (it == 0) ? 1 : it;
    c->timers.c[1] += counted;
    if (l2_iters) { *l2_iters += counted; }
    return LGH_OK;
 }
 
-int lgh_vec_set(lgh_ctx *c, double *y, double a, long n) { LGH_CHECK_ARG(c && y); return vec_set(c, y, a, n); }
+int lgh_vec_set(lgh_ctx *c, double *y, double a, long n)
+{
+   LGH_CHECK_ARG(c && y);
+   LGH_ENTRY(c);
+   return vec_set(c, y, a, n);
+}
 int lgh_vec_copy(lgh_ctx *c, double *y, const double *x, long n)
 {
    LGH_CHECK_ARG(c && y && x);
-   LGH_HIP_CHECK(hipMemcpyAsync(y, x, sizeof(double) * n, hipMemcpyDeviceToDevice, c->stream));
-   return LGH_OK;
+   LGH_ENTRY(c);
+   return vec_copy(c, y, x, n);
+}
+int lgh_vec_copy_deferred(lgh_ctx *c, double *y, const double *x, long n)
+{
+   LGH_CHECK_ARG(c && y && x);
+   if (n <= 0) { return LGH_OK; }
+   if (!side_ok(c)) { return lgh_vec_copy(c, y, x, n); }
+   side_dst(c, y, sizeof(double) * (size_t)n);
+   int rc = side_begin(c);
+   if (rc) { return rc; }
+   rc = vec_copy(c, y, x, n);
+   const int rc2 = side_end(c, y, sizeof(double) * (size_t)n);
+   return rc ? rc : rc2;
+}
+int lgh_vec_axpby_deferred(lgh_ctx *c, double *z, double a, const double *x, double b, const double *y, long n)
+{
+   LGH_CHECK_ARG(c && z && x && y);
+   if (n <= 0) { return LGH_OK; }
+   if (!side_ok(c)) { return lgh_vec_axpby(c, z, a, x, b, y, n); }
+   side_dst(c, z, sizeof(double) * (size_t)n);
+   int rc = side_begin(c);
+   if (rc) { return rc; }
+   rc = vec_axpby(c, z, a, x, b, y, n);
+   const int rc2 = side_end(c, z, sizeof(double) * (size_t)n);
+   return rc ? rc : rc2;
 }
 int lgh_vec_axpby(lgh_ctx *c, double *z, double a, const double *x, double b, const double *y, long n)
 {
    LGH_CHECK_ARG(c && z && x && y);
+   LGH_ENTRY(c);
    return vec_axpby(c, z, a, x, b, y, n);
 }
 int lgh_vec_axpby_pair(lgh_ctx *c, double *z1, double a1, const double *x1, double b1, double *z2, double a2, const double *x2, double b2,
                        const double *y, long n)
 {
    LGH_CHECK_ARG(c && z1 && x1 && z2 && x2 && y && n >= 0);
+   LGH_ENTRY(c);
    {
       auto overlap = [n](const double *p, const double *q) { return p < q + n && q < p + n; };
       LGH_CHECK_ARG(!overlap(z1, z2) && !overlap(z1, x2) && !overlap(z1, y));
@@ -1240,6 +1413,7 @@
 int lgh_vec_dot(lgh_ctx *c, const double *x, const double *y, long n, double *result)
 {
    LGH_CHECK_ARG(c && x && y && result);
+   LGH_ENTRY(c);
    int rc = vec_dot(c, x, y, nullptr, n, c->scal + 1);
    if (rc) { return rc; }
    LGH_HIP_CHECK(hipMemcpyAsync(c->host_pinned + 1, c->scal + 1, sizeof(double), hipMemcpyDeviceToHost, c->stream));
@@ -1263,6 +1437,7 @@
 int lgh_tg_source_2d(lgh_ctx *c, const double *S, double *e_source)
 {
    LGH_CHECK_ARG(c && S && e_source);
+   LGH_ENTRY(c);
    const int rc = no_1d(c, "lgh_tg_source_2d");
    if (rc) { return rc; }
    return tg_source_2d(c, S, e_source);
@@ -1271,12 +1446,14 @@
 int lgh_internal_energy(lgh_ctx *c, const double *e_l2, double *result)
 {
    LGH_CHECK_ARG(c && e_l2 && result);
+   LGH_ENTRY(c);
    if (c->dim == 1) { return energy_1d(c, 0, e_l2, result); }
    return interp_energy(c, 0, e_l2, result);
 }
 int lgh_kinetic_energy(lgh_ctx *c, const double *v_h1, double *result)
 {
    LGH_CHECK_ARG(c && v_h1 && result);
+   LGH_ENTRY(c);
    if (c->dim == 1) { return energy_1d(c, 1, v_h1, result); }
    return interp_energy(c, 1, v_h1, result);
 }
@@ -1370,12 +1547,14 @@
 int lgh_l2_mass_form(lgh_ctx *c, int *form, int *compact)
 {
    LGH_CHECK_ARG(c && form && compact);
+   LGH_ENTRY(c);
    if (c->dim == 1) { *form = 0; *compact = 0; return LGH_OK; }
    return l2_mass_form(c, form, compact);
 }
 int lgh_k1_form(lgh_ctx *c, int *form)
 {
    LGH_CHECK_ARG(c && form);
+   LGH_ENTRY(c);
    *form = (c->dim == 1) ? -1 : vcg_k1_form(c);
    return LGH_OK;
 }
@@ -1384,6 +1563,7 @@
                     double *y_E, double den[3])
 {
    LGH_CHECK_ARG(c && r && (first || d_old) && rz && rz_prev && y_E && den);
+   LGH_ENTRY(c);
    const int rc = no_1d(c, "lgh_test_vcg_k1");
    if (rc) { return rc; }
    return vcg_test_k1(c, r, d_old, rz, rz_prev, first, y_E, den);
@@ -1397,6 +1577,7 @@
 int lgh_vcg_layout_stats(lgh_ctx *c, long out[4])
 {
    LGH_CHECK_ARG(c && out);
+   LGH_ENTRY(c);
    const int rc = no_1d(c, "lgh_vcg_layout_stats");
    if (rc) { return rc; }
    return vcg_layout_stats(c, out);
@@ -1404,6 +1585,7 @@
 int lgh_test_vcg_merged_faces(lgh_ctx *c, unsigned char *mask, long *n_merged)
 {
    LGH_CHECK_ARG(c && mask && n_merged);
+   LGH_ENTRY(c);
    const int rc = no_1d(c, "lgh_test_vcg_merged_faces");
    if (rc) { return rc; }
    return vcg_test_merged_faces(c, mask, n_merged);
@@ -1412,6 +1594,7 @@
                     const double rz_prev[3], const double alpha_prev[3], double rz_out[3], int *deferred_x)
 {
    LGH_CHECK_ARG(c && it >= 1 && y_E && r && d && x && den && rz && rz_prev && alpha_prev && rz_out && deferred_x);
+   LGH_ENTRY(c);
    const int rc = no_1d(c, "lgh_test_vcg_k2");
    if (rc) { return rc; }
    return vcg_test_k2(c, it, y_E, r, d, x, den, rz, rz_prev, alpha_prev, rz_out, deferred_x);
@@ -1420,6 +1603,7 @@
                        long long *w_out, double *d_out, int *i_out)
 {
    LGH_CHECK_ARG(c && mode >= 0 && mode <= 4 && n >= 1 && n <= (1L << 24) && E >= -1000 && E <= 1000);
+   LGH_ENTRY(c);
    LGH_CHECK_ARG(mode != 0 || (v && w_out && i_out));
    LGH_CHECK_ARG(mode != 1 || (w_in && d_out && !scale));
    LGH_CHECK_ARG(mode != 2 || (v && w_out && d_out && G >= 1 && G <= 1024));
@@ -1430,6 +1614,7 @@
 int lgh_force_mult_E(lgh_ctx *c, const double *sJit, const double *x_E, double *y_E)
 {
    LGH_CHECK_ARG(c && sJit && x_E && y_E);
+   LGH_ENTRY(c);
    const int rc = no_1d(c, "lgh_force_mult_E");
    if (rc) { return rc; }
    return force_mult_E(c, sJit, x_E, y_E);
@@ -1437,6 +1622,7 @@
 int lgh_force_mult_transpose_E(lgh_ctx *c, const double *sJit, const double *v_E, double *y_E)
 {
    LGH_CHECK_ARG(c && sJit && v_E && y_E);
+   LGH_ENTRY(c);
    const int rc = no_1d(c, "lgh_force_mult_transpose_E");
    if (rc) { return rc; }
    return force_mult_t_E(c, sJit, v_E, y_E);
@@ -1444,6 +1630,7 @@
 int lgh_mass_apply_E(lgh_ctx *c, int space, const double *x_E, double *y_E)
 {
    LGH_CHECK_ARG(c && x_E && y_E);
+   LGH_ENTRY(c);
    const int rc = no_1d(c, "lgh_mass_apply_E");
    if (rc) { return rc; }
    return mass_apply_E(c, space, x_E, y_E);
@@ -1451,16 +1638,19 @@
 int lgh_test_eig(lgh_ctx *c, int dim, int n, const double *A, double *lambda, double *vec)
 {
    LGH_CHECK_ARG(c && A && lambda && vec && (dim == 2 || dim == 3));
+   LGH_ENTRY(c);
    return test_eig(c, dim, n, A, lambda, vec);
 }
 int lgh_test_sqrt(lgh_ctx *c, int n, const double *x, double *y)
 {
    LGH_CHECK_ARG(c && x && y && n >= 0);
+   LGH_ENTRY(c);
    return test_sqrt(c, n, x, y);
 }
 int lgh_test_singular(lgh_ctx *c, int dim, int n, const double *A, double *sv)
 {
    LGH_CHECK_ARG(c && A && sv && (dim == 2 || dim == 3));
+   LGH_ENTRY(c);
    return test_singular(c, dim, n, A, sv);
 }
 
diff --git a/laghos_amd/csrc/lgh_comm.hip b/laghos_amd/csrc/lgh_comm.hip
--- a/laghos_amd/csrc/lgh_comm.hip
+++ b/laghos_amd/csrc/lgh_comm.hip
@@ -937,6 +937,7 @@
 int lgh_test_word_peers(lgh_ctx *c, int nwords, long *capacity_words)
 {
    LGH_CHECK_ARG(c && nwords > 0 && capacity_words);
+   LGH_ENTRY(c);
    const long long *peers = nullptr;
    int n_peers = 0;
    const int rc = comm_word_peers(c, nwords, &peers, &n_peers);
@@ -949,6 +950,7 @@
 int lgh_test_halo_pack(lgh_ctx *c, const double *v, int ncomp, double *out)
 {
    LGH_CHECK_ARG(c && v && out && c->comm && ncomp >= 1 && ncomp <= 3);
+   LGH_ENTRY(c);
    Comm *cm = c->comm;
    if (cm->total == 0) { return LGH_OK; }
    hipLaunchKernelGGL(halo_pack_k, dim3(ceil_div((long)cm->total * ncomp, 256)), dim3(256), 0, c->stream,
@@ -960,6 +962,7 @@
 int lgh_test_halo_combine(lgh_ctx *c, const double *in, double *v, int ncomp)
 {
    LGH_CHECK_ARG(c && v && in && c->comm && ncomp >= 1 && ncomp <= 3);
+   LGH_ENTRY(c);
    Comm *cm = c->comm;
    if (cm->total == 0) { return LGH_OK; }
    LGH_HIP_CHECK(hipMemcpyAsync(cm->recvbuf, in, (size_t)cm->bufsize * sizeof(double), hipMemcpyDeviceToDevice, c->stream));
@@ -973,6 +976,7 @@
 int lgh_test_rccl_self_sendrecv(lgh_ctx *c, int n, double *max_abs_diff)
 {
    LGH_CHECK_ARG(c && c->comm && c->comm->comm && !c->comm->local && n > 0 && max_abs_diff);
+   LGH_ENTRY(c);
    double *buf = nullptr;
    LGH_HIP_CHECK(hipMalloc((void **)&buf, 2 * (size_t)n * sizeof(double)));
    std::vector<double> h(2 * (size_t)n, 0.0);
@@ -1060,12 +1064,14 @@
 int lgh_halo_sum(lgh_ctx *c, double *v_h1, int ncomp)
 {
    LGH_CHECK_ARG(c && v_h1 && ncomp >= 1 && ncomp <= 3);
+   LGH_ENTRY(c);
    return halo_sum(c, v_h1, ncomp, nullptr, 0);
 }
 
 int lgh_allreduce(lgh_ctx *c, double *value, int op)
 {
    LGH_CHECK_ARG(c && value);
+   LGH_ENTRY(c);
    if (!c->multi || !c->comm) { return LGH_OK; }
    c->host_pinned[3] = *value;
    LGH_HIP_CHECK(hipMemcpyAsync(c->scal + 2, c->host_pinned + 3, sizeof(double), hipMemcpyHostToDevice, c->stream));
diff --git a/laghos_amd/csrc/lgh_common.hpp b/laghos_amd/csrc/lgh_common.hpp
--- a/laghos_amd/csrc/lgh_common.hpp
+++ b/laghos_amd/csrc/lgh_common.hpp
@@ -36,6 +36,17 @@
       }                                                                                  \
    } while (0)
 
+#define LGH_ENTRY(c)                                                                     \
+   do                                                                                    \
+   {                                                                                     \
+      (c)->side_fork_valid = 0;                                                          \
+      if ((c)->side_pending)                                                             \
+      {                                                                                  \
+         const int rc_side_ = lgh::side_join(c);                                         \
+         if (rc_side_) { return rc_side_; }                                              \
+      }                                                                                  \
+   } while (0)
+
 constexpr int kWave = 64;
 
 struct CgScalars
@@ -92,6 +103,14 @@
    hipStream_t stream2;
    int on_stream2;
    hipEvent_t ev_fork, ev_join;
+   hipEvent_t ev_side, ev_side_in;
+   int side_on;
+   int side_pending, side_nrng;
+   int side_fork_valid;
+   unsigned differs_calls[2];
+   unsigned long side_seq, side_seq_join;
+   struct { const char *lo, *hi; } side_rng[8];
+   struct { const char *lo, *hi; } side_q;
    void *l2run;
    const double *accel_src;
    int e_async;
@@ -412,6 +431,14 @@
 int vcg_k1_form(lgh_ctx *c);
 void comm_shared_nodes(const lgh_ctx *c, const uint8_t **hmask, const int **sh_node, int *n_shared);
 int energy_overlap_poll(lgh_ctx *c);
+bool side_ok(const lgh_ctx *c);
+int side_begin(lgh_ctx *c);
+void side_dst(lgh_ctx *c, const void *dst, size_t bytes);
+int side_fork(lgh_ctx *c);
+int side_end(lgh_ctx *c, const void *dst, size_t bytes);
+int side_join(lgh_ctx *c);
+bool side_writes(const lgh_ctx *c, const void *p, size_t bytes);
+int vec_copy(lgh_ctx *c, double *y, const double *x, long n);
 int host_wait_token(lgh_ctx *c, volatile unsigned long long *word, unsigned long long token);
 constexpr int kLsWord = 50;
 constexpr int kLsWordsPerSet = 56;
diff --git a/laghos_amd/csrc/lgh_derived.hip b/laghos_amd/csrc/lgh_derived.hip
--- a/laghos_amd/csrc/lgh_derived.hip
+++ b/laghos_amd/csrc/lgh_derived.hip
@@ -262,6 +262,7 @@
                        double *detj_out, double *gradv_out, double *div_out, double *vort_out, double *cs_out)
 {
    LGH_CHECK_ARG(c && S);
+   LGH_ENTRY(c);
    if (!B_h1_lat || !G_h1_lat || !B_l2_lat)
    {
       set_error("lgh_sample_derived: %s is NULL", !B_h1_lat ? "B_h1_lat" : (!G_h1_lat ? "G_h1_lat" : "B_l2_lat"));
diff --git a/laghos_amd/csrc/lgh_diag.hip b/laghos_amd/csrc/lgh_diag.hip
--- a/laghos_amd/csrc/lgh_diag.hip
+++ b/laghos_amd/csrc/lgh_diag.hip
@@ -297,6 +297,7 @@
 int lgh_diagnostics_zones(lgh_ctx *c, const double *S, double *zone_out)
 {
    LGH_CHECK_ARG(c && S && zone_out);
+   LGH_ENTRY(c);
    const int rc = diag_ready(c, "lgh_diagnostics_zones");
    if (rc) { return rc; }
    return diag_zones(c, S, zone_out);
@@ -305,6 +306,7 @@
 int lgh_diagnostics(lgh_ctx *c, const double *S, double out[LGH_DIAG_COUNT])
 {
    LGH_CHECK_ARG(c && S && out);
+   LGH_ENTRY(c);
    int rc = diag_ready(c, "lgh_diagnostics");
    if (rc) { return rc; }
    if (!c->diag_dev)
diff --git a/laghos_amd/csrc/lgh_fingerprint.hip b/laghos_amd/csrc/lgh_fingerprint.hip
--- a/laghos_amd/csrc/lgh_fingerprint.hip
+++ b/laghos_amd/csrc/lgh_fingerprint.hip
@@ -141,6 +141,7 @@
 int lgh_vec_fingerprint(lgh_ctx *c, const double *x, long n, unsigned long long offset, unsigned long long out[2])
 {
    LGH_CHECK_ARG(c && out && n >= 0 && (x || n == 0));
+   LGH_ENTRY(c);
    LGH_CHECK_ARG(((uintptr_t)x & 7u) == 0);
    if (n == 0)
    {
@@ -169,6 +170,7 @@
 int lgh_vec_fingerprint_shape(lgh_ctx *c, const double *x, long n, long out[4])
 {
    LGH_CHECK_ARG(c && out && n >= 0);
+   LGH_ENTRY(c);
    long blocks, cap;
    int head;
    fp_shape(c, x, n, &blocks, &head, &cap);
diff --git a/laghos_amd/csrc/lgh_mass.hip b/laghos_amd/csrc/lgh_mass.hip
--- a/laghos_amd/csrc/lgh_mass.hip
+++ b/laghos_amd/csrc/lgh_mass.hip
@@ -1289,6 +1289,11 @@
    return LGH_OK;
 }
 
+__global__ void cg_scalars_to_host_k(const CgScalars *__restrict__ s, CgScalars *__restrict__ host)
+{
+   *host = *s;
+   __threadfence_system();
+}
 int cg_solve(lgh_ctx *c, int space, const double *b, double *x, double rel_tol, int max_iter,
              int *iters, bool x_is_zero)
 {
@@ -1355,7 +1360,7 @@
    while (!done)
    {
       if (multi && it > 0) { hipLaunchKernelGGL(cg_update_finish_k, dim3(1), dim3(1), 0, c->stream, c->cgs, it); }
-      LGH_HIP_CHECK(hipMemcpyAsync(hs, c->cgs, sizeof(CgScalars), hipMemcpyDeviceToHost, c->stream));
+      hipLaunchKernelGGL(cg_scalars_to_host_k, dim3(1), dim3(1), 0, c->stream, c->cgs, (CgScalars *)c->host_pinned_dev);
       LGH_HIP_CHECK(hipStreamSynchronize(c->stream));
       if (hs->done || it >= max_iter) { break; }
       if (!first_look) { chunk = (++looks <= 2) ? 2 : std::min(64, 2 * chunk); }
@@ -1567,7 +1572,7 @@
    while (true)
    {
       if (r->m.multi && r->it > 0) { hipLaunchKernelGGL(cg_update_finish_k, dim3(1), dim3(1), 0, c->stream, c->cgs, r->it); }
-      LGH_HIP_CHECK(hipMemcpyAsync(hs, c->cgs, sizeof(CgScalars), hipMemcpyDeviceToHost, c->stream));
+      hipLaunchKernelGGL(cg_scalars_to_host_k, dim3(1), dim3(1), 0, c->stream, c->cgs, (CgScalars *)c->host_pinned_dev);
       LGH_HIP_CHECK(hipStreamSynchronize(c->stream));
       if (hs->done || r->it >= r->max_iter) { break; }
       chunk = (++looks <= 2) ? 2 : std::min(64, 2 * chunk);
diff --git a/laghos_amd/csrc/lgh_profile.hip b/laghos_amd/csrc/lgh_profile.hip
--- a/laghos_amd/csrc/lgh_profile.hip
+++ b/laghos_amd/csrc/lgh_profile.hip
@@ -489,6 +489,7 @@
 extern "C" int lgh_profile(lgh_ctx *c, const double *S, const lgh_profile_spec *spec, double *out, long *n_excluded)
 {
    LGH_CHECK_ARG(c && S && spec && out && n_excluded);
+   LGH_ENTRY(c);
    if (!c->setup_done)
    {
       set_error("lgh_profile: lgh_setup_rho0detj0 has not been called (rho0DetJ0w is not set)");
diff --git a/laghos_amd/csrc/lgh_qupdate.hip b/laghos_amd/csrc/lgh_qupdate.hip
--- a/laghos_amd/csrc/lgh_qupdate.hip
+++ b/laghos_amd/csrc/lgh_qupdate.hip
@@ -16,6 +16,13 @@
    const bool keep = !c->stress_store && a.erhs_q && a.force_e && c->v_snap;
    if (keep) { a.stressJinvT = nullptr; }
    const int form = qupdate_form(c);
+   const bool side = side_ok(c);
+   if (side)
+   {
+      const int rs = side_fork(c);
+      if (rs) { return rs; }
+      c->side_q = {(const char *)S, (const char *)(S + 2 * (size_t)c->H1V + (size_t)c->L2V)};
+   }
    const int rc = (form == 1) ? launch_qrows(c, a) : launch_q<QMODE_UPDATE>(c, a);
    c->qgen++;
    c->stress_current = (rc == LGH_OK && !keep) ? 1 : 0;
@@ -23,7 +30,19 @@
    c->fused_f1_valid = (rc == LGH_OK && a.force_e) ? 1 : 0;
    if (c->fused_ftv_valid)
    {
-      LGH_HIP_CHECK(hipMemcpyAsync(c->v_snap, S + c->H1V, sizeof(double) * (size_t)c->H1V, hipMemcpyDeviceToDevice, c->stream));
+      if (side)
+      {
+         int rs = side_begin(c);
+         if (rs) { return rs; }
+         rs = vec_copy(c, c->v_snap, S + c->H1V, c->H1V);
+         const int rs2 = side_end(c, nullptr, 0);
+         if (rs || rs2) { return rs ? rs : rs2; }
+      }
+      else
+      {
+         const int rs = vec_copy(c, c->v_snap, S + c->H1V, c->H1V);
+         if (rs) { return rs; }
+      }
    }
    return rc;
 }
diff --git a/laghos_amd/csrc/lgh_sample.hip b/laghos_amd/csrc/lgh_sample.hip
--- a/laghos_amd/csrc/lgh_sample.hip
+++ b/laghos_amd/csrc/lgh_sample.hip
@@ -104,6 +104,7 @@
                       double *x_out, double *v_out, double *e_out, double *rho_out, double *p_out)
 {
    LGH_CHECK_ARG(c && S && B_h1_lat && B_l2_lat);
+   LGH_ENTRY(c);
    if (R1 < 2 || R1 > 9)
    {
       set_error("lgh_sample_fields: R1 = %d lattice points per direction is out of range (2 <= R1 <= 9)", R1);
diff --git a/laghos_amd/csrc/lgh_sedov.hip b/laghos_amd/csrc/lgh_sedov.hip
--- a/laghos_amd/csrc/lgh_sedov.hip
+++ b/laghos_amd/csrc/lgh_sedov.hip
@@ -464,6 +464,7 @@
 int lgh_sedov_eval(lgh_ctx *c, const double par[21], double t, long n, const double *r, double *rho, double *v, double *P)
 {
    LGH_CHECK_ARG(c && par && t > 0.0 && n >= 0 && (n == 0 || (r && rho && v && P)));
+   LGH_ENTRY(c);
    if (n == 0) { return LGH_OK; }
    const SedovPar s = par_from(par);
    hipLaunchKernelGGL(sedov_eval_k, dim3((unsigned)((n + 255) / 256)), dim3(256), 0, c->stream, s, sedov_shock(s, t), n, r,
@@ -475,6 +476,7 @@
 int lgh_compute_density(lgh_ctx *c, const double *x_h1, double *rho_l2)
 {
    LGH_CHECK_ARG(c && x_h1 && rho_l2);
+   LGH_ENTRY(c);
    if (c->dim == 1) { return density_1d(c, x_h1, rho_l2); }
    const int grid = std::min(c->NE, 2048);
    DevBuf scratch;
@@ -501,6 +503,7 @@
 {
    LGH_CHECK_ARG(c && x_h1 && rho_l2 && par && origin && weights && B_h1 && G_h1 && B_l2 && err2 && t > 0.0 &&
                  n1d >= 1 && n1d <= 64);
+   LGH_ENTRY(c);
    if (c->dim == 1) { return sedov_density_error_1d(c, x_h1, rho_l2, par, t, origin, n1d, weights, B_h1, G_h1, B_l2, err2); }
    const int D = c->D1D, L = c->L1D;
    std::vector<double> tab;
diff --git a/laghos_amd/csrc/lgh_vcg.hip b/laghos_amd/csrc/lgh_vcg.hip
--- a/laghos_amd/csrc/lgh_vcg.hip
+++ b/laghos_amd/csrc/lgh_vcg.hip
@@ -2357,7 +2357,7 @@
    }
    else
    {
-      if (aux->ord) { LGH_HIP_CHECK(hipMemsetAsync(a.x, 0, kVC * N * sizeof(double), c->stream)); }
+      if (aux->ord) { rc = vec_set(c, a.x, 0.0, (long)(kVC * N)); if (rc) { return rc; } }
       hipLaunchKernelGGL(vcg_init_k, dim3(nb), dim3(256), 0, c->stream, a);
    }
    LGH_HIP_CHECK(hipGetLastError());
diff --git a/laghos_amd/host/laghos.cpp b/laghos_amd/host/laghos.cpp
--- a/laghos_amd/host/laghos.cpp
+++ b/laghos_amd/host/laghos.cpp
@@ -932,9 +932,9 @@
          s->last_step = true;
       }
       if (s->steps == o.max_tsteps) { s->last_step = true; }
-      hydro.Copy(s->S_old, s->S);
+      hydro.ResetTimeStepEstimate();
+      hydro.CopyDeferred(s->S_old, s->S);
       s->t_old = s->t;
-      hydro.ResetTimeStepEstimate();
       s->ode->Step(s->S, s->t, s->dt);
       s->steps++;
       const double dt_est = hydro.GetTimeStepEstimate(s->S);
diff --git a/laghos_amd/host/laghos_solver.cpp b/laghos_amd/host/laghos_solver.cpp
--- a/laghos_amd/host/laghos_solver.cpp
+++ b/laghos_amd/host/laghos_solver.cpp
@@ -120,8 +120,8 @@
 void LagrangianHydroOperator::Mult(const Vector &S, Vector &dS_dt) const
 {
    UpdateMesh(S);
-   LGH_VERIFY(lgh_vec_copy(ctx, dS_dt.Write(), S.Read() + H1Vsize, H1Vsize));
    UpdateQuadratureData(S);
+   LGH_VERIFY(lgh_vec_copy_deferred(ctx, dS_dt.Write(), S.Read() + H1Vsize, H1Vsize));
    if (source_type == 1) { LGH_VERIFY(lgh_tg_source_2d(ctx, S.Read(), e_source.Write())); }
    LGH_VERIFY(lgh_solve_energy_begin(ctx, S.Read(), S.Read() + H1Vsize, dS_dt.Write(), e_rhs.Write(),
                                      source_type == 1 ? e_source.Read() : nullptr, cg_rel_tol, cg_max_iter));
@@ -299,6 +299,14 @@
 void LagrangianHydroOperator::Copy(Vector &y, const Vector &x) const
 {
    LGH_VERIFY(lgh_vec_copy(ctx, y.Write(), x.Read(), y.Size()));
+}
+void LagrangianHydroOperator::CopyDeferred(Vector &y, const Vector &x) const
+{
+   LGH_VERIFY(lgh_vec_copy_deferred(ctx, y.Write(), x.Read(), y.Size()));
+}
+void LagrangianHydroOperator::AddDeferred(Vector &z, double a, const Vector &x, double b, const Vector &y) const
+{
+   LGH_VERIFY(lgh_vec_axpby_deferred(ctx, z.Write(), a, x.Read(), b, y.Read(), z.Size()));
 }
 void LagrangianHydroOperator::Sync() const { LGH_VERIFY(lgh_sync(ctx)); }
 
@@ -435,11 +443,17 @@
 void RK4Solver::Step(Vector &S, double &t, double &dt)
 {
    f->Mult(S, k);
-   f->Add2(y, 1.0, S, dt / 2, z, 1.0, S, dt / 6, k);
+   f->Add(y, 1.0, S, dt / 2, k);
+   f->UpdateQuadratureData(y);
+   f->AddDeferred(z, 1.0, S, dt / 6, k);
    f->Mult(y, k);
-   f->Add2(y, 1.0, S, dt / 2, z, 1.0, z, dt / 3, k);
+   f->Add(y, 1.0, S, dt / 2, k);
+   f->UpdateQuadratureData(y);
+   f->AddDeferred(z, 1.0, z, dt / 3, k);
    f->Mult(y, k);
-   f->Add2(y, 1.0, S, dt, z, 1.0, z, dt / 3, k);
+   f->Add(y, 1.0, S, dt, k);
+   f->UpdateQuadratureData(y);
+   f->AddDeferred(z, 1.0, z, dt / 3, k);
    f->Mult(y, k);
    f->Add(S, 1.0, z, dt / 6, k);
    t += dt;
diff --git a/laghos_amd/host/laghos_solver.hpp b/laghos_amd/host/laghos_solver.hpp
--- a/laghos_amd/host/laghos_solver.hpp
+++ b/laghos_amd/host/laghos_solver.hpp
@@ -93,6 +93,8 @@
    void Add(Vector &z, double a, const Vector &x, double b, const Vector &y) const;
    void Add2(Vector &z1, double a1, const Vector &x1, double b1, Vector &z2, double a2, const Vector &x2, double b2, const Vector &y) const;
    void Copy(Vector &y, const Vector &x) const;
+   void CopyDeferred(Vector &y, const Vector &x) const;
+   void AddDeferred(Vector &z, double a, const Vector &x, double b, const Vector &y) const;
    void Sync() const;
 };
 
```

Result: no change. 1610 Mdofs*steps/s (-0.2%).
